# antonilo/unsupervised_detection

Measured on AMD Instinct MI355X. Metric: frame-pairs/sec per adversarial step, DAVIS 480p batch4, 1/2/4/8 GPU, higher is better.
Workload: dtype f32

## Files before the change

include/udet.h:

```cpp
#ifndef UDET_H
#define UDET_H
#include <stddef.h>
#ifdef __cplusplus
extern "C" {
#endif

#define UDET_OK 0
#define UDET_ERR_SHAPE (-1)
#define UDET_ERR_ALIGN (-2)
#define UDET_ERR_HIP (-3)
#define UDET_ERR_UNSUPPORTED (-4)
#define UDET_ERR_ARG (-5)
#define UDET_ERR_OVERFLOW (-6)

#define UDET_ACT_NONE 0
#define UDET_ACT_LEAKY 1
#define UDET_ACT_ELU 2

int udet_version(void);
const char* udet_last_error(void);


int udet_warp(const float* image, const float* flow, float flow_scale, float* out, int n, int h, int w, int c,
              void* stream);
// ... 58 lines not shown
typedef struct {
  int batch;
  int in_h, in_w;
  int img_h, img_w;
  float flow_normalizer;
  float cbn;
  float epsilon;
  float lr, beta1, beta2, adam_eps;
  float clip;
  unsigned long long noise_seed;
  int conv_fp16;
} udet_config;

int udet_plan_create(const udet_config* cfg, udet_plan** out);
void udet_plan_destroy(udet_plan* plan);
size_t udet_workspace_bytes(const udet_plan* plan);
int udet_plan_init(udet_plan* plan, void* workspace, void* stream);

int udet_param_count(int net);
size_t udet_param_total(int net);
int udet_param_info(int net, int index, const char** name, int* rank, int* shape4, size_t* offset_floats);
int udet_buffer_count(const udet_plan* plan);
int udet_buffer_info(const udet_plan* plan, int index, const char** name, size_t* offset_bytes, int* dims_nhw_ld);

int udet_pack_pwc(udet_plan* plan, const float* w_pwc, void* workspace, void* stream);
int udet_pack_trainable(udet_plan* plan, const float* w_gen, const float* w_rec, void* workspace, void* stream);

int udet_pwc_forward(udet_plan* plan, const float* img1, const float* img2, void* workspace, void* stream);
int udet_forward(udet_plan* plan, const float* img1, const float* img2, int ncalls, void* workspace, void* stream);
int udet_prefetch_flow(udet_plan* plan, const float* img1, const float* img2, void* workspace, void* stream);
int udet_forward_prefetched(udet_plan* plan, int ncalls, void* workspace, void* stream);
int udet_prefetch_consume(udet_plan* plan, void* workspace, void* stream);
int udet_forward_from_flow(udet_plan* plan, int ncalls, void* workspace, void* stream);
int udet_generator_forward(udet_plan* plan, void* workspace, void* stream);
int udet_generator_layers(udet_plan* plan, void* workspace, void* stream);
int udet_recover_forward(udet_plan* plan, int n, void* workspace, void* stream);
int udet_backward(udet_plan* plan, int which, const float* w_gen, const float* w_rec, float* g_gen, float* g_rec,
                  void* workspace, void* stream);
int udet_stream_wait_grads(udet_plan* plan, int net, void* stream);
int udet_generator_backward(udet_plan* plan, const float* w_gen, float* g_gen, void* workspace, void* stream);
int udet_recover_backward(udet_plan* plan, const float* w_rec, float* g_rec, void* workspace, void* stream);
int udet_grad_absmean(udet_plan* plan, int net, const float* g, float* out2, void* workspace, void* stream);
int udet_apply(udet_plan* plan, int net, float* w, float* g, float* m, float* v, void* workspace, void* stream);
long udet_fp16_overflow_count(udet_plan* plan);
long udet_get_adam_step(const udet_plan* plan);
void udet_set_adam_step(udet_plan* plan, long t);
int udet_train_step(udet_plan* plan, int which, const float* img1, const float* img2, float* w_gen, float* w_rec,
                    float* g_gen, float* g_rec, float* m_gen, float* v_gen, float* m_rec, float* v_rec, void* workspace,
                    void* stream);

int udet_autotune(udet_plan* plan, const float* w_gen, const float* w_rec, float* g_gen, float* g_rec, void* workspace,
                  void* stream);
int udet_tuned_shapes(void);
int udet_tune_save(const char* path);
int udet_tune_load(const char* path);
int udet_tune_rejected(void);
int udet_profile_begin(udet_plan* plan);
int udet_profile_end(udet_plan* plan, double* out, int ncat, void* stream);

int udet_plan_set_concurrent(udet_plan* plan, int on);

int udet_plan_lane_queues(udet_plan* plan, void* stream, int* queue);
int udet_plan_pin_lanes(udet_plan* plan, void* stream, void* const* side_streams, int n);

#ifdef __cplusplus
}
// ... 3 lines not shown
```

include/udet_debug.h:

```cpp
#ifndef UDET_DEBUG_H
#define UDET_DEBUG_H
#ifdef __cplusplus
extern "C" {
#endif
void udet_debug_force_conv(int bm, int bn, int ks);
void udet_debug_conv_fp16(int on);
void udet_debug_force_wgrad(int nsplit, int dma);
int udet_debug_last_wgrad(void);
void udet_debug_upb_min_pixels(long v);
void udet_debug_set_tuning(int on);
void udet_debug_force_pair(int on);
int udet_debug_last_pair(void);
#include <stddef.h>
int udet_debug_conv2d_pair(const float* xa, const float* xb, const float* wa, const float* wb, const float* ba, const float* bb, float* ya, float* yb,
                           int na, int nb, int h, int w, int cin, int cout, int k, int stride, int dilation, int act, float alpha, void* workspace,
                           size_t workspace_bytes, void* stream);
int udet_debug_last_conv(void);
#ifdef __cplusplus
}
#endif
#endif
```

unsupervised_detection_amd/_devel.py:

```python
from __future__ import annotations

import ctypes
import os

from ._ffi import lib as _lib

_PATH = os.path.join(os.path.dirname(os.path.abspath(__file__)), "libudet_debug.so")
if not os.path.exists(_PATH):
    raise RuntimeError(f"{_PATH} is missing: build it with `make -C unsupervised_detection_amd/csrc`")
dbg = ctypes.CDLL(_PATH, mode=ctypes.RTLD_GLOBAL)
dbg.udet_debug_force_conv.restype = None
dbg.udet_debug_force_conv.argtypes = [ctypes.c_int, ctypes.c_int, ctypes.c_int]
dbg.udet_debug_last_conv.restype = ctypes.c_int
dbg.udet_debug_last_conv.argtypes = []
dbg.udet_debug_conv_fp16.restype = None
dbg.udet_debug_conv_fp16.argtypes = [ctypes.c_int]
dbg.udet_debug_force_wgrad.restype = None
dbg.udet_debug_force_wgrad.argtypes = [ctypes.c_int, ctypes.c_int]
dbg.udet_debug_upb_min_pixels.restype = None
dbg.udet_debug_upb_min_pixels.argtypes = [ctypes.c_long]
dbg.udet_debug_set_tuning.restype = None
dbg.udet_debug_set_tuning.argtypes = [ctypes.c_int]
dbg.udet_debug_last_wgrad.restype = ctypes.c_int
dbg.udet_debug_last_wgrad.argtypes = []
dbg.udet_debug_force_pair.restype = None
dbg.udet_debug_force_pair.argtypes = [ctypes.c_int]
dbg.udet_debug_last_pair.restype = ctypes.c_int
dbg.udet_debug_last_pair.argtypes = []
dbg.udet_debug_conv2d_pair.restype = ctypes.c_int
dbg.udet_debug_conv2d_pair.argtypes = [ctypes.c_void_p] * 8 + [ctypes.c_int] * 10 + [ctypes.c_float, ctypes.c_void_p, ctypes.c_size_t, ctypes.c_void_p]
```

unsupervised_detection_amd/csrc/api_plan.hip:

```cpp
#include <stdlib.h>
#include <string.h>

#include "conv_host.h"
#include "elementwise.h"
#include "plan.h"

using namespace udet;

struct udet_plan {
  Plan* p;
};

extern "C" {

int udet_plan_create(const udet_config* c, udet_plan** out) {
  if (!c || !out) { set_error("plan_create: null argument"); return UDET_ERR_ARG; }
  Config k;
  k.batch = c->batch; k.in_h = c->in_h; k.in_w = c->in_w; k.img_h = c->img_h; k.img_w = c->img_w;
  k.flow_normalizer = c->flow_normalizer; k.cbn = c->cbn; k.epsilon = c->epsilon;
  k.lr = c->lr; k.beta1 = c->beta1; k.beta2 = c->beta2; k.adam_eps = c->adam_eps; k.clip = c->clip;
  k.noise_seed = c->noise_seed;
  k.conv_fp16 = c->conv_fp16 ? 1 : 0;
  Plan* P = plan_build(k);
  if (!P) return UDET_ERR_SHAPE;
// ... 35 lines not shown
  return plan_lane_queues(h->p, (hipStream_t)stream, queue);
}
int udet_plan_pin_lanes(udet_plan* h, void* stream, void* const* side_streams, int n) {
  if (!h || (n > 0 && !side_streams)) { set_error("plan_pin_lanes: null argument"); return UDET_ERR_ARG; }
  return plan_pin_lanes(h->p, (hipStream_t)stream, reinterpret_cast<hipStream_t const*>(side_streams), n);
}
long udet_fp16_overflow_count(udet_plan* h) {
  if (!h) return 0;
  (void)plan_check_overflow(h->p, true);
  return h->p->ovf_skipped;
}
long udet_get_adam_step(const udet_plan* h) {
  plan_settle_adam_step(h->p);
  return h->p->adam_t;
}
void udet_set_adam_step(udet_plan* h, long t) {
  plan_settle_adam_step(h->p);
  h->p->adam_t = t;
}

int udet_pack_pwc(udet_plan* h, const float* w_pwc, void* ws, void* stream) {
  return plan_pack_pwc(h->p, w_pwc, (float*)ws, (hipStream_t)stream);
}
int udet_pack_trainable(udet_plan* h, const float* w_gen, const float* w_rec, void* ws, void* stream) {
  return plan_pack_trainable(h->p, w_gen, w_rec, (float*)ws, (hipStream_t)stream);
}
int udet_pwc_forward(udet_plan* h, const float* img1, const float* img2, void* ws, void* stream) {
  return plan_pwc_forward(h->p, img1, img2, (float*)ws, (hipStream_t)stream);
}
int udet_forward_from_flow(udet_plan* h, int ncalls, void* ws, void* stream) {
  UDET_TRY(plan_check_overflow(h->p, false));
  if (ncalls < 0 || ncalls > 3) { set_error("forward: ncalls must be 0..3"); return UDET_ERR_ARG; }
  return plan_forward(h->p, nullptr, nullptr, ncalls, (float*)ws, (hipStream_t)stream);
}
int udet_generator_forward(udet_plan* h, void* ws, void* stream) {
  UDET_TRY(plan_generator_forward(h->p, (float*)ws, (hipStream_t)stream));
  return plan_recover_forward(h->p, 0, (float*)ws, (hipStream_t)stream);
}
int udet_generator_layers(udet_plan* h, void* ws, void* stream) {
  h->p->ev_next = 0;
  UDET_TRY(plan_generator_layers(h->p, (float*)ws, (hipStream_t)stream));
  return plan_recover_forward(h->p, 0, (float*)ws, (hipStream_t)stream);
}
int udet_recover_forward(udet_plan* h, int n, void* ws, void* stream) {
  if (n < 1 || n > 3) { set_error("recover_forward: n must be 1..3 (multiples of the plan batch)"); return UDET_ERR_ARG; }
  return plan_recover_forward(h->p, n, (float*)ws, (hipStream_t)stream, true);
}
int udet_forward(udet_plan* h, const float* img1, const float* img2, int ncalls, void* ws, void* stream) {
  UDET_TRY(plan_check_overflow(h->p, false));
  if (ncalls < 0 || ncalls > 3) { set_error("forward: ncalls must be 0..3"); return UDET_ERR_ARG; }
  if (!img1 || !img2) { set_error("forward: null image pointer"); return UDET_ERR_ARG; }
  return plan_forward(h->p, img1, img2, ncalls, (float*)ws, (hipStream_t)stream);
}
int udet_prefetch_flow(udet_plan* h, const float* img1, const float* img2, void* ws, void* stream) {
  if (!img1 || !img2) { set_error("prefetch_flow: null image pointer"); return UDET_ERR_ARG; }
  return plan_prefetch(h->p, img1, img2, (float*)ws, (hipStream_t)stream);
}
int udet_prefetch_consume(udet_plan* h, void* ws, void* stream) {
  return plan_prefetch_consume(h->p, (float*)ws, (hipStream_t)stream);
}
int udet_forward_prefetched(udet_plan* h, int ncalls, void* ws, void* stream) {
  UDET_TRY(plan_check_overflow(h->p, false));
  if (ncalls < 0 || ncalls > 3) { set_error("forward: ncalls must be 0..3"); return UDET_ERR_ARG; }
  return plan_forward(h->p, nullptr, nullptr, ncalls, (float*)ws, (hipStream_t)stream, true);
}
int udet_backward(udet_plan* h, int which, const float* w_gen, const float* w_rec, float* g_gen, float* g_rec, void* ws,
// ... 149 lines not shown
```

unsupervised_detection_amd/csrc/common.h:

```cpp
#pragma once
#include <hip/hip_runtime.h>
#include <hip/hip_ext.h>
#include <stdint.h>
#include <stdio.h>
#include <string>

#include "../../include/udet.h"

namespace udet {

void set_error(const char* fmt, ...);
int hip_fail(hipError_t e, const char* what);
#define UDET_HIP(x)                                   \
  do {                                                \
    hipError_t _e = (x);                              \
    if (_e != hipSuccess) return udet::hip_fail(_e, #x); \
  } while (0)
#define UDET_TRY(x)            \
  do {                         \
    int _s = (x);              \
    if (_s != 0) return _s;    \
  } while (0)

struct LaunchSink {
// ... 93 lines not shown
  const float* res;
  int ldres, res_coff;
  float* y2;
  int ldy2, y2_coff;
  int accumulate;
  float* uo;
  int ldu, u_coff;
  const float* ua;
  int ldua, ua_coff, uact;
  float ualpha;
  int u_c0, u_c1;
  int ksplit;
  float* partial;
  size_t partial_cap;
  int ldp;
  int fold;
  int* tickets;
  int tail_full, tail_ks, tail_prow0;
  int f16;
  float f16_xscale;
  const float* wino_u;
  int wino_np;
  int kreal;
};
#define UDET_MAX_TICKETS 4096

int launch_conv(ConvParams& p, hipStream_t stream);
int launch_conv_pair(ConvParams& a, ConvParams& b, hipStream_t stream);
int launch_tap_gather(const ConvParams& g, const float* z, int ldz, hipStream_t stream);

struct PackJob {
  long src_off, dst_off, gamma_off, beta_off;
  long total;
  int T, R, C, Kc, ldw, k_split, k_gap, mode;
};

struct WgradParams {
  const float* x;
  int ldx, x_coff;
  int N, H, W, up_shift;
  int Cin;
  const float* dy;
  const float* ya;
  int ldy, y_coff, Cout;
  int yact;
  float yalpha;
  int OH, OW, isy, isx;
  int ycls, OHf, OWf;
  int ntaps;
  ConvTap taps[UDET_MAX_TAPS];
  float* dw;
  float* db;
  float* partial;
  size_t partial_floats;
  const float* zero16;
  int swapped, oCin, oCout, bias_m;
  int Cin4, Mpad;
  float* pbias;
  FastDiv fd_ohw, fd_ow;
  const float* w;
  const float* b;
  const float* gamma;
  float* dgamma;
  float* dbeta;
  float bn_c;
  int f16;
  float f16_yscale;
};
int launch_wgrad_T(WgradParams& p, int T, hipStream_t stream);
int launch_bn_finalize(float* dw, int T, int Cin, int Cout, const float* w, const float* b, const float* gamma, float bn_c, float* pd,
                       float* db, float* dgamma, float* dbeta, hipStream_t stream);
int launch_wgrad_up_combine(const float* deff, float* dw, int Cin, int Cout, hipStream_t stream);
size_t wgrad_partial_floats_needed(int T, int Cin, int Cout);

}
```

unsupervised_detection_amd/csrc/conv_host.h:

```cpp
#pragma once
#include "common.h"
namespace udet {
void same_pad(int in, int k, int s, int d, int* before, int* out);
void conv_setup_fwd(ConvParams& p, int N, int H, int W, int kh, int kw, int s, int d);
int conv_dgrad_classes(int s, int H, int W);
void conv_force_config(int bm, int bn, int ks);
bool conv_thin_n_ok(const ConvParams& p);
bool conv_thin_k_ok(const ConvParams& p);
int launch_conv_thin_n(const ConvParams& p, hipStream_t stream);
int launch_conv_thin_k(const ConvParams& p, hipStream_t stream);
bool conv_wino_geometry(const ConvParams& p, int* dil, int widx_at[9]);
bool conv_wino_ok(const ConvParams& p);
bool conv_wino_variant_ok(const ConvParams& p, int variant);
int conv_wino_np(int cout);
size_t conv_wino_floats(int Kc, int cout);
long conv_wino_workgroups(const ConvParams& p, int variant);
int conv_wino_max_ksplit(const ConvParams& p, int variant);
int launch_conv_wino(ConvParams& p, int variant, int ks, hipStream_t stream);
int launch_splitk_second_pass(const ConvParams& p, hipStream_t stream);
int launch_wino_pack(const float* src, float* dst, int R, int C, int Kc, int np, int k_split, int k_gap, int transposed, hipStream_t stream);
int launch_wino_from_packed(const ConvParams& p, float* dst, int np, hipStream_t stream);
void conv_debug_f16(int on);
int conv_debug_f16_on();
int conv_last_config();
void conv_set_tuning(int on);
int conv_tuned_shapes();
void conv_clear_tuning();
int conv_tune_rejected();
void conv_tune_note_reject();
float* tune_scratch(size_t floats, int which);
bool tune_compare(const float* a, const float* b, size_t n, hipStream_t stream, float* diff_out, float* scale_out);
void wgrad_set_tuning(int on);
bool wgrad_wino_ok(const WgradParams& p);
int wgrad_wino_slices(const WgradParams& p, int wanted);
int launch_wgrad_wino(const WgradParams& q, int slices, int ldn, hipStream_t stream);
int wgrad_last_config();
void wgrad_force(int nsplit, int dma);
int wgrad_tuned_shapes();
void conv_tune_dump(FILE* f);
void conv_tune_put(unsigned long long key, int bm, int bn, int ks, int ws, int fold, int tail);
void wgrad_tune_dump(FILE* f);
void conv_pair_tune_dump(FILE* f);
void conv_pair_tune_put(unsigned long long key, int bm, int bn, int ks, int ws);
int conv_pair_tuned_shapes();
void conv_pair_clear_tuning();
void conv_force_pair(int on);
int conv_last_pair();
#define UDET_TUNE_ABI 6
void wgrad_tune_put(unsigned long long key, int cfg);
bool conv_setup_dgrad(ConvParams& p, int cls, int N, int H, int W, int kh, int kw, int s, int d);
int launch_pack_weights(const float* src, float* dst, int T, int R, int C, int Kc, int ldw, int k_split, int k_gap,
                        int mode, const float* scale, hipStream_t stream);
int launch_pack_taps_into_n(const float* src, float* dst, int T, int R, int C, int Kc, int ldz, int k_split, int k_gap,
                            int transposed, hipStream_t stream);
int launch_pack_jobs(const PackJob* jobs_dev, int njobs, const float* wsrc, float* ws, float bn_c, hipStream_t stream);
int launch_fold_bn(const float* b, const float* gamma, const float* beta, float c, float* scale, float* bias_f, int n,
                   hipStream_t stream);
int launch_copy_channels(const float* src, int lds, int s_coff, float* dst, int ldd, int d_coff, long P, int C, float mul,
                         float add, hipStream_t stream);
int launch_warp(const float* img, const float* flow, int ldf, int f_coff, float flow_scale, float* out, int N, int H,
                int W, int C, int* dbg_idx, float* dbg_alpha, hipStream_t stream);
int launch_cost_volume(const float* c1, const float* wr, float* out, int ldo, int o_coff, int N, int H, int W, int C,
                       hipStream_t stream);
int launch_warp_cost_volume(const float* c1, const float* c2, const float* flow, int ldf, int f_coff, float flow_scale, float* out,
                            int ldo, int corr_coff, int c1_coff, float* warped_dbg, int N, int H, int W, int C, hipStream_t stream);
inline int round_up(int v, int m) { return (v + m - 1) / m * m; }
}
```

unsupervised_detection_amd/csrc/conv_host.hip:

```cpp
#include <string.h>

#include <stdint.h>

#include "common.h"
#include "conv_host.h"
#include "wino_pack.h"

namespace udet {

void same_pad(int in, int k, int s, int d, int* before, int* out) {
  const int o = (in + s - 1) / s;
  int total = (o - 1) * s + (k - 1) * d + 1 - in;
  if (total < 0) total = 0;
  *before = total / 2;
  *out = o;
}

static inline int floordiv2(int v) { return v >= 0 ? v / 2 : -((-v + 1) / 2); }

static void push_tap(ConvParams& p, int dy, int dx, int widx) {
  const int ymax = (p.OHq - 1) * p.isy + dy, xmax = (p.OWq - 1) * p.isx + dx;
  if (dy >= p.H || ymax < 0 || dx >= p.W || xmax < 0) return;
  p.taps[p.ntaps].dy = dy;
  p.taps[p.ntaps].dx = dx;
// ... 72 lines not shown
    const int k = (int)((e / ldw) % Kc);
    const int t = (int)(e / ((long)ldw * Kc));
    float v = 0.f;
    int ks = k;
    if (k >= k_split) ks = (k < k_split + k_gap) ? -1 : k - k_gap;
    const int r = mode == 0 ? ks : n, c = mode == 0 ? n : ks;
    if (r >= 0 && r < R && c >= 0 && c < C) {
      v = src[((long)t * R + r) * C + c];
      if (scale) v *= scale[c];
    }
    dst[e] = v;
  }
}

int launch_pack_weights(const float* src, float* dst, int T, int R, int C, int Kc, int ldw, int k_split, int k_gap,
                        int mode, const float* scale, hipStream_t stream) {
  const long total = (long)T * Kc * ldw;
  int nb = (int)((total + 255) / 256);
  if (nb > 2048) nb = 2048;
  UDET_LAUNCH(pack_weights_kernel, dim3(nb), dim3(256), 0, stream, src, dst, T, R, C, Kc, ldw, k_split, k_gap,
                     mode, scale);
  UDET_HIP(hipGetLastError());
  return UDET_OK;
}

__constant__ float UPB_MERGE[2][3][3][4] = {
    {{{.5f, 0.f, 0.f, 0.f}, {.5f, 1.f, .5f, 0.f}, {0.f, 0.f, .5f, 1.f}},
     {{.5f, 0.f, 0.f, 0.f}, {.5f, 1.f, 1.f, 0.f}, {0.f, 0.f, 0.f, 0.f}},
     {{0.f, 0.f, 0.f, 0.f}, {0.f, 0.f, .5f, 0.f}, {0.f, 0.f, -.5f, -1.f}}},
    {{{1.f, .5f, 0.f, 0.f}, {0.f, .5f, 1.f, .5f}, {0.f, 0.f, 0.f, .5f}},
     {{1.f, 1.f, 0.f, 0.f}, {0.f, 0.f, 0.f, 0.f}, {0.f, 0.f, 0.f, 0.f}},
     {{0.f, .5f, 0.f, 0.f}, {0.f, -.5f, -1.f, -.5f}, {0.f, 0.f, 0.f, -.5f}}}};

__global__ __launch_bounds__(256) void pack_jobs_kernel(const PackJob* __restrict__ jobs, const float* __restrict__ wsrc,
                                                        float* __restrict__ ws, float bn_c) {
  const PackJob j = jobs[blockIdx.y];
  const float* src = wsrc + j.src_off;
  float* dst = ws + j.dst_off;
  const float* gamma = j.gamma_off >= 0 ? wsrc + j.gamma_off : nullptr;
  if (j.mode == 2) {
    for (long e = (long)blockIdx.x * 256 + threadIdx.x; e < j.total; e += (long)gridDim.x * 256)
      dst[e] = gamma ? src[e] * (gamma[e] * bn_c) + wsrc[j.beta_off + e] : src[e];
    return;
  }
  if (j.mode == 9 || j.mode == 10) {
    const int rv = (int)(j.beta_off / 3), cv = (int)(j.beta_off % 3);
    for (long e = (long)blockIdx.x * 256 + threadIdx.x; e < j.total; e += (long)gridDim.x * 256) {
      const int n = (int)(e % j.ldw), k = (int)(e / j.ldw);
      int ks = k;
      if (k >= j.k_split) ks = (k < j.k_split + j.k_gap) ? -1 : k - j.k_gap;
      const int ci = j.mode == 9 ? ks : n, co = j.mode == 9 ? n : ks;
      const bool real = ci >= 0 && ci < j.R && co >= 0 && co < j.C;
      float w[4][4];
#pragma unroll
      for (int kk = 0; kk < 4; ++kk)
#pragma unroll
        for (int ll = 0; ll < 4; ++ll) w[kk][ll] = real ? src[((long)(kk * 4 + ll) * j.R + ci) * j.C + co] : 0.f;
      const long plane = (long)j.Kc * j.ldw;
#pragma unroll
      for (int py = 0; py < 2; ++py) {
        float t1[3][4];
#pragma unroll
        for (int a = 0; a < 3; ++a)
#pragma unroll
          for (int ll = 0; ll < 4; ++ll) {
            float v = 0.f;
#pragma unroll
            for (int kk = 0; kk < 4; ++kk) v += UPB_MERGE[py][rv][a][kk] * w[kk][ll];
            t1[a][ll] = v;
          }
#pragma unroll
        for (int px = 0; px < 2; ++px)
#pragma unroll
          for (int a = 0; a < 3; ++a)
#pragma unroll
            for (int bb = 0; bb < 3; ++bb) {
              float v = 0.f;
#pragma unroll
              for (int ll = 0; ll < 4; ++ll) v += UPB_MERGE[px][cv][bb][ll] * t1[a][ll];
              dst[(long)((py * 2 + px) * 9 + a * 3 + bb) * plane + e] = v;
            }
      }
    }
    return;
  }
  if (j.mode == 7 || j.mode == 8) {
    for (long e = (long)blockIdx.x * 256 + threadIdx.x; e < j.total; e += (long)gridDim.x * 256) wino_pack_item(j, src, gamma, bn_c, dst, e);
    return;
  }
  for (long e = (long)blockIdx.x * 256 + threadIdx.x; e < j.total; e += (long)gridDim.x * 256) {
    const int n = (int)(e % j.ldw);
    const int k = (int)((e / j.ldw) % j.Kc);
    int t = (int)(e / ((long)j.ldw * j.Kc));
    float v = 0.f;
    int ks = k;
    if (k >= j.k_split) ks = (k < j.k_split + j.k_gap) ? -1 : k - j.k_gap;
    int r = j.mode == 0 ? ks : n, c = j.mode == 0 ? n : ks;
    if (j.mode == 3 || j.mode == 4) {
      t = n / j.C;
      c = n - t * j.C;
      r = ks;
      if (t >= j.T) r = -1;
    }
    if (j.mode >= 5) {
      const int cls = t >> 2, ty = (t >> 1) & 1, tx = t & 1, py = cls >> 1, px = cls & 1;
      const int y0 = py == 0 ? (ty == 0 ? 0 : 1) : (ty == 0 ? 0 : 2), y1 = py == 0 ? (ty == 0 ? 0 : 2) : (ty == 0 ? 1 : 2);
      const int x0 = px == 0 ? (tx == 0 ? 0 : 1) : (tx == 0 ? 0 : 2), x1 = px == 0 ? (tx == 0 ? 0 : 2) : (tx == 0 ? 1 : 2);
      const int ci = j.mode == 5 ? ks : n, co = j.mode == 5 ? n : ks;
      if (ci >= 0 && ci < j.R && co >= 0 && co < j.C) {
        for (int ky = y0; ky <= y1; ++ky)
          for (int kx = x0; kx <= x1; ++kx) v += src[((long)(ky * 3 + kx) * j.R + ci) * j.C + co];
        if (gamma) v *= gamma[co] * bn_c;
      }
      dst[e] = v;
      continue;
    }
    if (r >= 0 && r < j.R && c >= 0 && c < j.C) {
      v = j.mode == 4 ? src[((long)t * j.C + c) * j.R + r] : src[((long)t * j.R + r) * j.C + c];
      if (gamma) v *= gamma[c] * bn_c;
    }
    dst[e] = v;
  }
}
int launch_pack_jobs(const PackJob* jobs_dev, int njobs, const float* wsrc, float* ws, float bn_c, hipStream_t stream) {
  if (njobs < 1) return UDET_OK;
  UDET_LAUNCH(pack_jobs_kernel, dim3(48, njobs), dim3(256), 0, stream, jobs_dev, wsrc, ws, bn_c);
  UDET_HIP(hipGetLastError());
  return UDET_OK;
}

__global__ __launch_bounds__(256) void pack_job_kernel(const PackJob j, const float* __restrict__ wsrc, float* __restrict__ ws) {
  const float* src = wsrc + j.src_off;
  float* dst = ws + j.dst_off;
  for (long e = (long)blockIdx.x * 256 + threadIdx.x; e < j.total; e += (long)gridDim.x * 256) {
    const int n = (int)(e % j.ldw);
    const int k = (int)((e / j.ldw) % j.Kc);
    int ks = k;
    if (k >= j.k_split) ks = (k < j.k_split + j.k_gap) ? -1 : k - j.k_gap;
    const int t = n / j.C, c = n - t * j.C;
    float v = 0.f;
    if (ks >= 0 && ks < j.R && t < j.T) v = j.mode == 4 ? src[((long)t * j.C + c) * j.R + ks] : src[((long)t * j.R + ks) * j.C + c];
    dst[e] = v;
  }
}
int launch_pack_taps_into_n(const float* src, float* dst, int T, int R, int C, int Kc, int ldz, int k_split, int k_gap,
                            int transposed, hipStream_t stream) {
  PackJob j;
  memset(&j, 0, sizeof(j));
  j.T = T; j.R = R; j.C = C; j.Kc = Kc; j.ldw = ldz; j.k_split = k_split; j.k_gap = k_gap;
  j.mode = transposed ? 4 : 3; j.total = (long)Kc * ldz; j.gamma_off = -1;
  int nb = (int)((j.total + 255) / 256);
  if (nb > 1024) nb = 1024;
  UDET_LAUNCH(pack_job_kernel, dim3(nb), dim3(256), 0, stream, j, src, dst);
  UDET_HIP(hipGetLastError());
  return UDET_OK;
}

__global__ __launch_bounds__(256) void tap_gather_kernel(const ConvParams g, const float* __restrict__ z, int ldz) {
  const long total = (long)g.N * g.OH * g.OW * g.Cout;
// ... 117 lines not shown
```

unsupervised_detection_amd/csrc/conv_wgrad.hip:

```cpp
#include <stdlib.h>

#include <mutex>
#include <unordered_map>

#include "common.h"
#include <algorithm>
#include <vector>
#include "conv_host.h"
#include "plan.h"

namespace udet {

typedef float floatx16 __attribute__((ext_vector_type(16)));
typedef _Float16 halfx4 __attribute__((ext_vector_type(4)));

template <int BM, int BN, int WAVES_M, int WAVES_N>
__global__ __launch_bounds__(256) void conv_wgrad_kernel(const WgradParams p, int co_tiles, int nsplit) {
  constexpr int BKP = 32;
  constexpr int WTM = BM / WAVES_M, WTN = BN / WAVES_N;
  constexpr int TM = WTM / 32, TN = WTN / 32;
  static_assert(WAVES_M * WAVES_N == 4 && TM * 32 == WTM && TN * 32 == WTN, "tile");
  constexpr int A_F4_ROW = BM / 4, B_F4_ROW = BN / 4;
  constexpr int A_PIX = 256 / A_F4_ROW, B_PIX = 256 / B_F4_ROW;
  constexpr int A_LD = BKP / A_PIX, B_LD = BKP / B_PIX;
// ... 439 lines not shown
      for (; k + 7 * SL < nsplit; k += 8 * SL) {
        float a[8];
#pragma unroll
        for (int u = 0; u < 8; ++u) a[u] = src[(size_t)(k + u * SL) * slab];
#pragma unroll
        for (int u = 0; u < 8; ++u) s += a[u];
      }
      for (; k < nsplit; k += SL) s += src[(size_t)k * slab];
    }
    if (SL > 1) {
      part[t] = s;
      __syncthreads();
      if (sl == 0) {
#pragma unroll
        for (int u = 1; u < SL; ++u) s += part[t + u * CW];
      }
      __syncthreads();
    }
    if (on && sl == 0) {
      const size_t e = ((size_t)p.taps[tap].widx * p.Cin + ci) * p.Cout + co;
      dot = fmaf(p.w[e], s, dot);
      p.dw[e] = s * gs;
    }
  }
  red[t] = dot;
  __syncthreads();
  if (rg == 0 && co < p.Cout) {
    float d = red[co];
#pragma unroll
    for (int g = 1; g < RG; ++g) d += red[g * CW + co];
    pd[(size_t)blockIdx.x * p.Cout + co] = d;
  }
}
__global__ __launch_bounds__(256) void wgrad_bn_finish2_kernel(const WgradParams p, int ldn, int nsplit, int nb, const float* __restrict__ pd) {
  __shared__ float red[256];
  __shared__ float redS[256];
  const int t = threadIdx.x, cl = t & 31, rg = t >> 5, co = blockIdx.x * 32 + cl;
  const int per = (nb + 7) / 8, b0 = rg * per, b1 = b0 + per < nb ? b0 + per : nb;
  const int pers = (nsplit + 7) / 8, k0 = rg * pers, k1 = k0 + pers < nsplit ? k0 + pers : nsplit;
  float d = 0.f, S = 0.f;
  if (co < p.Cout) {
    int b = b0;
    for (; b + 11 < b1; b += 12) {
      float a[12];
#pragma unroll
      for (int u = 0; u < 12; ++u) a[u] = pd[(size_t)(b + u) * p.Cout + co];
#pragma unroll
      for (int u = 0; u < 12; ++u) d += a[u];
    }
    for (; b < b1; ++b) d += pd[(size_t)b * p.Cout + co];
    int k = k0;
    for (; k + 7 < k1; k += 8) {
      float a[8];
#pragma unroll
      for (int u = 0; u < 8; ++u) a[u] = p.pbias[(size_t)(k + u) * ldn + co];
#pragma unroll
      for (int u = 0; u < 8; ++u) S += a[u];
    }
    for (; k < k1; ++k) S += p.pbias[(size_t)k * ldn + co];
  }
  red[t] = d;
  redS[t] = S;
  __syncthreads();
  if (rg == 0 && co < p.Cout) {
    float dsum = red[cl], Ssum = redS[cl];
#pragma unroll
    for (int g = 1; g < 8; ++g) { dsum += red[g * 32 + cl]; Ssum += redS[g * 32 + cl]; }
    p.dgamma[co] = p.bn_c * (dsum + p.b[co] * Ssum);
    p.dbeta[co] = Ssum;
    p.db[co] = p.gamma[co] * p.bn_c * Ssum;
  }
}
__global__ __launch_bounds__(256) void bn_dot_kernel(const float* __restrict__ w, const float* __restrict__ g, int R, int C,
                                                     float* __restrict__ pd) {
  __shared__ float red[256];
  const int t = threadIdx.x, cx = t & 63, ry = t >> 6;
  const int c = blockIdx.x * 64 + cx;
  const int r_begin = (int)((long)R * blockIdx.y / BND_SPLIT), r_end = (int)((long)R * (blockIdx.y + 1) / BND_SPLIT);
  float s = 0.f;
  if (c < C)
    for (int r = r_begin + ry; r < r_end; r += 4) s = fmaf(w[(size_t)r * C + c], g[(size_t)r * C + c], s);
  red[t] = s;
  __syncthreads();
  if (ry == 0 && c < C) pd[(size_t)blockIdx.y * C + c] = red[cx] + red[64 + cx] + red[128 + cx] + red[192 + cx];
}
__global__ __launch_bounds__(256) void bn_finish_kernel(float* __restrict__ dw, long n, int C, const float* __restrict__ gamma,
                                                        const float* __restrict__ b, float bn_c, const float* __restrict__ pd,
                                                        float* __restrict__ db, float* __restrict__ dgamma,
                                                        float* __restrict__ dbeta) {
  for (long e = (long)blockIdx.x * 256 + threadIdx.x; e < n; e += (long)gridDim.x * 256) {
    const int c = (int)(e % C);
    dw[e] *= gamma[c] * bn_c;
  }
  if (blockIdx.x == 0) {
    for (int c = threadIdx.x; c < C; c += 256) {
      float dot = 0.f;
      for (int j = 0; j < BND_SPLIT; ++j) dot += pd[(size_t)j * C + c];
      const float S = db[c];
      dgamma[c] = bn_c * (dot + b[c] * S);
      dbeta[c] = S;
      db[c] = gamma[c] * bn_c * S;
    }
  }
}
// ... 29 lines not shown
}
size_t wgrad_partial_floats_needed(int T, int Cin, int Cout) {
  const size_t cin4 = (size_t)((Cin + 3) & ~3), mpad = (T * cin4 + 127) / 128 * 128, ldn = (size_t)(Cout + 127) / 128 * 128;
  return (size_t)BNR_MAXBLK * Cout + ldn + mpad * ldn + 64;
}

static int g_force_wsplit = 0, g_force_wdma = -1;
static int g_wlast = 0;
int wgrad_last_config() { return g_wlast; }
void wgrad_force(int nsplit, int dma) { g_force_wsplit = nsplit > 0 ? nsplit : 0; g_force_wdma = dma; }
static std::unordered_map<uint64_t, int> g_wcache;
static std::mutex g_wcache_mu;
static int g_wtuning = 0;
void wgrad_set_tuning(int on) { g_wtuning = on; }
int wgrad_tuned_shapes() { std::lock_guard<std::mutex> l(g_wcache_mu); return (int)g_wcache.size(); }
void wgrad_tune_dump(FILE* f) {
  std::lock_guard<std::mutex> l(g_wcache_mu);
  for (auto& kv : g_wcache) fprintf(f, "w %llu %d\n", (unsigned long long)kv.first, kv.second);
}
void wgrad_tune_put(unsigned long long key, int cfg) {
  std::lock_guard<std::mutex> l(g_wcache_mu);
  g_wcache[(uint64_t)key] = cfg;
}

template <int BM, int BN, int WM_, int WN_>
static void wgrad_launch(const WgradParams& p, int m_tiles, int co_tiles, int nsplit, int dma, hipStream_t stream) {
  dim3 grid(m_tiles * co_tiles, nsplit);
  if (dma && p.f16) UDET_LAUNCH((conv_wgrad_dma_kernel<BM, BN, WM_, WN_, 2, true>), grid, dim3(512), 0, stream, p, co_tiles, nsplit);
  else if (dma == 2) UDET_LAUNCH((conv_wgrad_dma_kernel<BM, BN, WM_, WN_, 3>), grid, dim3(512), 0, stream, p, co_tiles, nsplit);
  else if (dma) UDET_LAUNCH((conv_wgrad_dma_kernel<BM, BN, WM_, WN_, 2>), grid, dim3(512), 0, stream, p, co_tiles, nsplit);
  else UDET_LAUNCH((conv_wgrad_kernel<BM, BN, WM_, WN_>), grid, dim3(256), 0, stream, p, co_tiles, nsplit);
}

int launch_wgrad_T(WgradParams& p, int T, hipStream_t stream) {
  if (conv_debug_f16_on()) p.f16 = 1;
  if (p.f16 && !(p.f16_yscale > 0.f)) p.f16_yscale = 1.f;
  if (p.f16 && g_wtuning) p.f16_yscale = 1.f;
  if (p.ldx % 4 || p.x_coff % 4 || p.ldy % 4 || p.y_coff % 4) {
    set_error("wgrad: ldx=%d x_coff=%d ldy=%d y_coff=%d must be multiples of 4", p.ldx, p.x_coff, p.ldy, p.y_coff);
    return UDET_ERR_ALIGN;
  }
  WgradParams g = p;
  g.swapped = 0; g.bias_m = -1; g.oCin = p.Cin; g.oCout = p.Cout;
  {
    int centre = -1;
    for (int t = 0; t < p.ntaps; ++t)
      if (p.taps[t].dy == 0 && p.taps[t].dx == 0) centre = t;
    auto tile_cost = [](long rows, int cols) {
      const int bn_ = cols > 64 ? 128 : (cols > 32 ? 64 : 32);
      return ((rows + 127) / 128 * 128) * (long)((cols + bn_ - 1) / bn_ * bn_);
    };
    const int co4 = (p.Cout + 3) & ~3, ci4 = (p.Cin + 3) & ~3;
    const bool cheaper = tile_cost((long)p.ntaps * co4, p.Cin) < tile_cost((long)p.ntaps * ci4, p.Cout);
    const bool narrow = p.Cout <= 4 ? p.Cin >= 16 : (p.Cout <= 16 && 128 % co4 == 0 && cheaper);
    const bool swap = narrow && p.isy == 1 && p.isx == 1 && p.up_shift == 0 && p.H == p.OH && p.W == p.OW &&
                      p.ya == nullptr && centre >= 0;
    if (swap) {
      g.x = p.dy; g.ldx = p.ldy; g.x_coff = p.y_coff; g.Cin = p.Cout;
      g.dy = p.x; g.ldy = p.ldx; g.y_coff = p.x_coff; g.Cout = p.Cin;
      for (int t = 0; t < p.ntaps; ++t) { g.taps[t].dy = -p.taps[t].dy; g.taps[t].dx = -p.taps[t].dx; }
      g.swapped = 1;
      g.bias_m = centre * co4;
    }
  }
  const int BM = 128;
  const int bn = g.Cout > 64 ? 128 : (g.Cout > 32 ? 64 : 32);
  g.Cin4 = (g.Cin + 3) & ~3;
// ... 10 lines not shown
  g.fd_ohw = make_fastdiv((unsigned)(g.OH * g.OW));
  g.fd_ow = make_fastdiv((unsigned)g.OW);
  float* pd = p.partial;
  float* base = pd + (size_t)BNR_MAXBLK * p.Cout;
  base += (16 - ((uintptr_t)base / sizeof(float)) % 16) % 16;
  const size_t fixed = (size_t)(base - p.partial);
  const size_t bgroups = p.ycls ? 4 : 1;
  const size_t per_split = bgroups * (size_t)ldn + (size_t)g.Mpad * ldn;
  if (p.partial_floats < fixed + per_split) {
    set_error("wgrad: workspace too small (%zu < %zu floats)", p.partial_floats, fixed + per_split);
    return UDET_ERR_ARG;
  }
  const long tiles = (long)m_tiles * co_tiles;
  const size_t maxs = (p.partial_floats - fixed) / per_split;
  int cap = nchunks / 2 > 0 ? nchunks / 2 : 1;
  if ((size_t)cap > maxs) cap = (int)maxs;
  int nsplit = (int)((768 + tiles - 1) / tiles);
  if (nsplit > cap) nsplit = cap;
  if (nsplit < 1) nsplit = 1;
  if (p.f16 && p.ya == nullptr && p.zero16 != nullptr && !(reinterpret_cast<uintptr_t>(p.zero16) & 15)) nsplit |= 1 << 20;
  const size_t wsz = (size_t)T * p.Cin * p.Cout;
  if (p.ntaps < T) UDET_HIP(hipMemsetAsync(p.dw, 0, wsz * sizeof(float), stream));
  const long total = (long)(Mreal + 1) * g.Cout;
  const bool dma_ok = p.ya == nullptr && p.zero16 != nullptr && !(reinterpret_cast<uintptr_t>(p.zero16) & 15);
  const bool fused_bn = p.gamma && !g.swapped && !p.ycls && p.ntaps == T && p.Cout <= 128 && p.db && p.dgamma && p.dbeta && p.w && p.b;
  const bool wino_ok = !g.swapped && !p.ycls && !plan_knob(UDET_KNOB_NO_WGRAD_WINO) && wgrad_wino_ok(g);
  auto run = [&](int cfg) -> int {
    int ns = cfg & 0xfffff;
    int dma = cfg >> 20;
    if (dma == 3 && !wino_ok) dma = 1;
    if (dma != 3 && !dma_ok) dma = 0;
    if (dma == 3) ns = wgrad_wino_slices(g, ns > (int)maxs ? (int)maxs : ns);
    WgradParams q = g;
    q.pbias = base;
    q.partial = base + (size_t)ns * bgroups * ldn;
    if (dma == 3 && launch_wgrad_wino(q, ns, ldn, stream) != UDET_OK) {
      dma = dma_ok ? 1 : 0;
      ns = nsplit & 0xfffff;
      if (ns > cap) ns = cap;
      if (ns < 1) ns = 1;
      q.partial = base + (size_t)ns * bgroups * ldn;
    }
    if (dma == 3) {}
    else if (bn == 128) wgrad_launch<128, 128, 2, 2>(q, m_tiles, co_tiles, ns, dma, stream);
    else if (bn == 64) wgrad_launch<128, 64, 2, 2>(q, m_tiles, co_tiles, ns, dma, stream);
    else wgrad_launch<128, 32, 4, 1>(q, m_tiles, co_tiles, ns, dma, stream);
    if (fused_bn) {
      const int cw = g.Cout > 64 ? 128 : (g.Cout > 32 ? 64 : (g.Cout > 16 ? 32 : 16));
      const int rg = 256 / cw;
      int sl = ns >= 64 ? 8 : (ns >= 32 ? 4 : (ns >= 12 ? 2 : 1));
      if (sl > rg) sl = rg;
      while (sl > 1 && (long)((Mreal + rg - 1) / rg) * sl > 512) sl >>= 1;
      int rb = rg / sl;
      while ((Mreal + rb - 1) / rb > BNR_MAXBLK) rb *= 2;
      const int nb = (Mreal + rb - 1) / rb;
#define UDET_RBN(CW_, SL_) UDET_LAUNCH((wgrad_reduce_bn_kernel<CW_, SL_>), dim3(nb), dim3(256), 0, stream, q, ldn, ns, rb, pd)
      if (cw == 128) { if (sl == 2) UDET_RBN(128, 2); else UDET_RBN(128, 1); }
      else if (cw == 64) { if (sl == 4) UDET_RBN(64, 4); else if (sl == 2) UDET_RBN(64, 2); else UDET_RBN(64, 1); }
      else if (cw == 32) { if (sl == 8) UDET_RBN(32, 8); else if (sl == 4) UDET_RBN(32, 4); else if (sl == 2) UDET_RBN(32, 2); else UDET_RBN(32, 1); }
      else { if (sl == 8) UDET_RBN(16, 8); else if (sl == 4) UDET_RBN(16, 4); else if (sl == 2) UDET_RBN(16, 2); else UDET_RBN(16, 1); }
#undef UDET_RBN
      UDET_LAUNCH(wgrad_bn_finish2_kernel, dim3((g.Cout + 31) / 32), dim3(256), 0, stream, q, ldn, ns, nb, pd);
      return UDET_OK;
    }
    const int sl = (ns >= 64 && total * 64 <= 262144) ? 64 : ((ns >= 8 && total * 8 <= 262144) ? 8 : 1);
    const long nbl = (total * sl + 255) / 256;
    const int nb = (int)(nbl > 4096 ? 4096 : nbl);
    if (sl == 64) UDET_LAUNCH(wgrad_reduce_kernel<64>, dim3(nb), dim3(256), 0, stream, q, ldn, ns);
    else if (sl == 8) UDET_LAUNCH(wgrad_reduce_kernel<8>, dim3(nb), dim3(256), 0, stream, q, ldn, ns);
    else UDET_LAUNCH(wgrad_reduce_kernel<1>, dim3(nb), dim3(256), 0, stream, q, ldn, ns);
    return UDET_OK;
  };
  {
    const int f[] = {p.N, p.H, p.W, p.up_shift, p.Cin, p.Cout, p.ntaps, p.OH, p.OW, p.isy, p.ya ? 1 : 0, p.ldx, p.ldy, cap, dma_ok ? 1 : 0, g.swapped, p.ycls, p.f16 ? 1 : 0,
                     p.ntaps > 0 ? p.taps[0].dy : 0, p.ntaps > 0 ? p.taps[0].dx : 0};
    uint64_t key = 1469598103934665603ull;
    for (int v : f) { key ^= (uint64_t)(uint32_t)v; key *= 1099511628211ull; }
    bool have = false;
    {
      std::lock_guard<std::mutex> l(g_wcache_mu);
      auto it = g_wcache.find(key);
      if (it != g_wcache.end()) {
        const int hv = nsplit, v = it->second >> 20, ns = it->second & 0xfffff;
        if (v < 0 || v > 3 || ns < 1) nsplit = hv;
        else nsplit = (v != 3 && ns > cap ? cap : ns) | (v << 20);
        have = true;
      }
    }
    if (!have && g_wtuning) {
      static hipEvent_t e0 = nullptr, e1 = nullptr;
      if (!e0) { (void)hipEventCreate(&e0); (void)hipEventCreate(&e1); }
      const int h = nsplit;
      float best_ms = 1e30f;
      int best = h;
      const int hc = h & 0xfffff;
// ... 41 lines not shown
        float diff = 0.f, scale = 0.f;
        if (r0) {
          run(h);
          (void)hipMemcpyAsync(r0, p.dw, wsz * sizeof(float), hipMemcpyDeviceToDevice, stream);
          if (p.db) (void)hipMemcpyAsync(r0 + wsz, p.db, (size_t)p.Cout * sizeof(float), hipMemcpyDeviceToDevice, stream);
          run(best);
          ok = tune_compare(r0, p.dw, wsz, stream, &diff, &scale);
          if (ok && p.db) ok = tune_compare(r0 + wsz, p.db, (size_t)p.Cout, stream, &diff, &scale);
        }
        if (!ok) {
          fprintf(stderr, "[udet tune] REJECTED wgrad N=%d %dx%d Cin=%d Cout=%d taps=%d: nsplit=%d dma=%d differs from the heuristic "
                  "configuration (max|diff| %.3e, scale %.3e)\n", p.N, p.OH, p.OW, p.Cin, p.Cout, p.ntaps, best & 0xfffff, best >> 20, diff, scale);
          conv_tune_note_reject();
          nsplit = h;
        }
      }
      if (getenv("UDET_TUNE_LOG"))
        fprintf(stderr, "[udet tune] wgrad N=%d %dx%d Cin=%d Cout=%d taps=%d -> nsplit=%d dma=%d (heuristic %d) %.1f us\n", p.N, p.OH,
                p.OW, p.Cin, p.Cout, p.ntaps, nsplit & 0xfffff, nsplit >> 20, h & 0xfffff, best_ms / 3 * 1e3f);
      std::lock_guard<std::mutex> l(g_wcache_mu);
      g_wcache[key] = nsplit;
    }
  }
  if (g_force_wsplit > 0) {
    const int ns = g_force_wsplit > cap ? cap : g_force_wsplit;
    int v = g_force_wdma >= 0 ? g_force_wdma : (nsplit >> 20);
    if (v == 3 && !wino_ok) v = dma_ok ? 1 : 0;
    if (v != 3 && !dma_ok) v = 0;
    nsplit = ns | (v << 20);
  }
  if ((nsplit >> 20) == 3 && !wino_ok) nsplit = (nsplit & 0xfffff) | ((dma_ok ? 1 : 0) << 20);
  if ((nsplit >> 20) == 3) nsplit = wgrad_wino_slices(g, (nsplit & 0xfffff) > (int)maxs ? (int)maxs : (nsplit & 0xfffff)) | (3 << 20);
  g_wlast = nsplit;
  UDET_TRY(run(nsplit));
  UDET_HIP(hipGetLastError());
  int nbw = (int)((wsz + 255) / 256);
  if (nbw > 2048) nbw = 2048;
  if (p.gamma && !fused_bn) {
    if (!p.db || !p.dgamma || !p.dbeta || !p.w || !p.b) {
      set_error("wgrad: BN finalisation needs db, dgamma, dbeta, w and b");
      return UDET_ERR_ARG;
    }
    UDET_LAUNCH(bn_dot_kernel, dim3((p.Cout + 63) / 64, BND_SPLIT), dim3(256), 0, stream, p.w, p.dw, T * p.Cin,
                       p.Cout, pd);
    UDET_LAUNCH(bn_finish_kernel, dim3(nbw), dim3(256), 0, stream, p.dw, (long)wsz, p.Cout, p.gamma, p.b, p.bn_c, pd,
                       p.db, p.dgamma, p.dbeta);
    UDET_HIP(hipGetLastError());
  }
  return UDET_OK;
}

}
```

unsupervised_detection_amd/csrc/devel/api_debug.hip:

```cpp
#include <string.h>

#include "../../../include/udet_debug.h"
#include "../conv_host.h"
#include "../plan.h"

using namespace udet;

extern "C" {
int udet_debug_last_conv(void) { return conv_last_config(); }
void udet_debug_force_conv(int bm, int bn, int ks) { conv_force_config(bm, bn, ks); }
void udet_debug_conv_fp16(int on) { conv_debug_f16(on); }
void udet_debug_force_wgrad(int nsplit, int dma) { wgrad_force(nsplit, dma); }
int udet_debug_last_wgrad(void) { return wgrad_last_config(); }
void udet_debug_upb_min_pixels(long v) { plan_debug_upb_min_pixels(v); }
void udet_debug_force_pair(int on) { conv_force_pair(on); }
int udet_debug_last_pair(void) { return conv_last_pair(); }
int udet_debug_conv2d_pair(const float* xa, const float* xb, const float* wa, const float* wb, const float* ba, const float* bb, float* ya, float* yb,
                           int na, int nb, int h, int w, int cin, int cout, int k, int stride, int dilation, int act, float alpha, void* workspace,
                           size_t workspace_bytes, void* stream_) {
  hipStream_t stream = (hipStream_t)stream_;
  if (cin % 8 != 0 || k * k > UDET_MAX_TAPS) { set_error("debug_conv2d_pair: cin must be a multiple of 8"); return UDET_ERR_SHAPE; }
  const int kc = cin, ldw = round_up(cout, 4);
  const size_t wfl = ((size_t)k * k * kc * ldw + 63) & ~(size_t)63, part_fl = (size_t)4 << 20, zero_fl = 64 + UDET_MAX_TICKETS;
  if (workspace_bytes < (2 * wfl + part_fl + zero_fl) * sizeof(float)) { set_error("debug_conv2d_pair: workspace too small"); return UDET_ERR_ARG; }
  float* wpa = reinterpret_cast<float*>(workspace);
  float* wpb = wpa + wfl;
  float* part = wpb + wfl;
  float* zero = part + part_fl;
  UDET_HIP(hipMemsetAsync(zero, 0, zero_fl * sizeof(float), stream));
  UDET_TRY(launch_pack_weights(wa, wpa, k * k, cin, cout, kc, ldw, kc, 0, 0, nullptr, stream));
  UDET_TRY(launch_pack_weights(wb, wpb, k * k, cin, cout, kc, ldw, kc, 0, 0, nullptr, stream));
  ConvParams p[2];
  for (int i = 0; i < 2; ++i) {
    memset(&p[i], 0, sizeof(ConvParams));
    conv_setup_fwd(p[i], i ? nb : na, h, w, k, k, stride, dilation);
    p[i].x = i ? xb : xa; p[i].ldx = cin; p[i].wp = i ? wpb : wpa; p[i].Kc = kc; p[i].ldw = ldw; p[i].bias = i ? bb : ba;
    p[i].y = i ? yb : ya; p[i].ldy = cout; p[i].Cout = cout; p[i].act = act; p[i].alpha = alpha;
    p[i].partial = part; p[i].partial_cap = part_fl; p[i].zero16 = zero; p[i].tickets = reinterpret_cast<int*>(zero + 64);
  }
  return launch_conv_pair(p[0], p[1], stream);
}
void udet_debug_set_tuning(int on) {
  conv_set_tuning(on);
  wgrad_set_tuning(on);
}
}
```

unsupervised_detection_amd/csrc/elementwise.h:

```cpp
#pragma once
#include "common.h"
namespace udet {
int launch_resize_bilinear_fwd(const float* x, int ldx, int x_coff, int N, int H, int W, float* y, int ldy, int y_coff,
                               int OH, int OW, int C, float mul, float div, hipStream_t s);
int launch_resize_bilinear_bwd(const float* dy, int ldy, int y_coff, int N, int OH, int OW, float* dx, int ldx, int x_coff,
                               int H, int W, int C, int accumulate, hipStream_t s);
int launch_upb_ring(const float* x, int ld, int N, int H, int W, float* xh, hipStream_t s);
int launch_upb_ring_fold(const float* dxh, int ld, int N, int H, int W, float* dx, hipStream_t s);
int launch_share_samples(float* buf, long P, int ld, int coff, int C, int copies, hipStream_t s);
int launch_fold_samples(float* buf, long P, int ld, int coff, int C, int copies, hipStream_t s);
int launch_emit_du(const float* d, const float* a, float* u, long P, int ld, int coff, int C, int act, float alpha, hipStream_t s);
int launch_pool2x2_sum(const float* du, float* dx, int N, int H, int W, int C, hipStream_t s);
int launch_pack_pwc_input(const float* i1, const float* i2, float* x8, long P, hipStream_t s);
int launch_gen_input(const float* img, const float* f, double* part, float* gin, int B, long HW, hipStream_t s);
size_t flow_stats_doubles(int B);
int launch_mask_rec_inputs(const float* logits, const float* f, float* mask, float* fin, long P, int ncalls, hipStream_t s);
int launch_pack_imgin(const float* img, float* imgin, long P, int ncalls, hipStream_t s);
int launch_losses(const float* f, const float* mask, const float* pred, long HW, int B, float cbn, float eps,
                  float num_pixels, float* part, float* losses, float* coef, float* sums, hipStream_t s);
size_t loss_part_floats(int B);
int launch_rec_loss_bwd(const float* f, const float* mask, const float* pred, float* dpred, long BHW, float cbn,
                        float inv_np, hipStream_t s);
int launch_gen_loss_bwd(const float* f, const float* mask, const float* pred, const float* coef, float* dpred,
                        float* dmask, long HW, int B, float cbn, hipStream_t s);
int launch_mask_bwd(const float* dmask, const float* dfin, const float* f, const float* mask, float* dlogits, long P,
                    hipStream_t s);
int launch_grad_absmean(const float* g, const long* seg_off, const long* seg_len, int nvars, float* vmean, float thresh,
                        float* out, hipStream_t s);
int launch_adam(float* w, float* g, float* m, float* v, long n, float lr_t, float b1, float b2, float eps, float clip,
                const float* flag, uint64_t seed, uint64_t step, hipStream_t s, int mode = 0, const int* skip = nullptr);
int launch_nonfinite_count(const float* g, long n, int* out, hipStream_t s);
int launch_flow_normalize(const float* f, double* part, float* out, int B, long HW, hipStream_t s);
int launch_charbonnier(const float* gt, const float* pred, const float* mask, int mc, int B, long HW, float cbn, float* part,
                       float* out, hipStream_t s);
int launch_crop_flip_resize(const void* src, int src_u8, int nearest, int N, int H, int W, int C, const int* prm, float* dst, int OH,
                            int OW, float div, float add, hipStream_t s);
int launch_crop_flip_resize_ragged(const void* src, int src_u8, int nearest, int N, int C, const long long* offsets, const int* hw,
                                   const int* prm, float* dst, int OH, int OW, float div, float add, hipStream_t s);
int launch_mask_stats(const float* pred, const float* gt, int N, int H, int W, float threshold, float gt_threshold, double* out,
                      hipStream_t s);
int launch_fill_uniform(float* x, long n, uint64_t seed, float lo, float hi, hipStream_t s);
int launch_axpy(const float* x, float* y, long n, float a, int accumulate, hipStream_t s);
}
```

unsupervised_detection_amd/csrc/elementwise.hip:

```cpp
#include "common.h"
#include "elementwise.h"

namespace udet {

static inline int grid_for(long total, int cap = 4096) {
  long nb = (total + 255) / 256;
  if (nb > cap) nb = cap;
  if (nb < 1) nb = 1;
  return (int)nb;
}

template <typename T>
__device__ __forceinline__ T wave_sum(T v) {
#pragma unroll
  for (int o = 32; o > 0; o >>= 1) v += __shfl_down(v, o, 64);
  return v;
}
template <typename T>
__device__ __forceinline__ T block_sum(T v, T* sm ) {
  v = wave_sum(v);
  __syncthreads();
  if ((threadIdx.x & 63) == 0) sm[threadIdx.x >> 6] = v;
  __syncthreads();
  return sm[0] + sm[1] + sm[2] + sm[3];
// ... 314 lines not shown
        float4* q = reinterpret_cast<float4*>(buf + o + (long)k * P * ld);
        if (FOLD) {
          const float4 w = *q;
          v.x += w.x; v.y += w.y; v.z += w.z; v.w += w.w;
        } else {
          *q = v;
        }
      }
      if (FOLD) *reinterpret_cast<float4*>(buf + o) = v;
    } else {
      float v = buf[o];
      for (int k = 1; k < copies; ++k) {
        if (FOLD) v += buf[o + (long)k * P * ld];
        else buf[o + (long)k * P * ld] = v;
      }
      if (FOLD) buf[o] = v;
    }
  }
}
static int launch_share_fold(float* buf, long P, int ld, int coff, int C, int copies, bool fold, hipStream_t s) {
  if (copies < 2 || C < 1) return UDET_OK;
  const bool v4 = (ld % 4 == 0) && (coff % 4 == 0) && (C % 4 == 0);
  const long n = P * (v4 ? C / 4 : C);
  if (v4) {
    if (fold) hipLaunchKernelGGL((share_fold_kernel<4, true>), dim3(grid_for(n)), dim3(256), 0, s, buf, P, ld, coff, C, copies);
    else hipLaunchKernelGGL((share_fold_kernel<4, false>), dim3(grid_for(n)), dim3(256), 0, s, buf, P, ld, coff, C, copies);
  } else {
    if (fold) hipLaunchKernelGGL((share_fold_kernel<1, true>), dim3(grid_for(n)), dim3(256), 0, s, buf, P, ld, coff, C, copies);
    else hipLaunchKernelGGL((share_fold_kernel<1, false>), dim3(grid_for(n)), dim3(256), 0, s, buf, P, ld, coff, C, copies);
  }
  UDET_HIP(hipGetLastError());
  return UDET_OK;
}
int launch_share_samples(float* buf, long P, int ld, int coff, int C, int copies, hipStream_t s) {
  return launch_share_fold(buf, P, ld, coff, C, copies, false, s);
}
int launch_fold_samples(float* buf, long P, int ld, int coff, int C, int copies, hipStream_t s) {
  return launch_share_fold(buf, P, ld, coff, C, copies, true, s);
}

__global__ __launch_bounds__(256) void pack_pwc_input_kernel(const float* __restrict__ i1, const float* __restrict__ i2,
                                                             float* __restrict__ x8, long P) {
  for (long e = (long)blockIdx.x * 256 + threadIdx.x; e < 2 * P; e += (long)gridDim.x * 256) {
    const float* s = e < P ? i1 + e * 3 : i2 + (e - P) * 3;
    float4 a = make_float4(s[0] + 0.5f, s[1] + 0.5f, s[2] + 0.5f, 0.f);
    *reinterpret_cast<float4*>(x8 + e * 4) = a;
  }
}
int launch_pack_pwc_input(const float* i1, const float* i2, float* x8, long P, hipStream_t s) {
  hipLaunchKernelGGL(pack_pwc_input_kernel, dim3(grid_for(2 * P)), dim3(256), 0, s, i1, i2, x8, P);
  UDET_HIP(hipGetLastError());
  return UDET_OK;
}

#define FS_BLOCKS 32
__global__ __launch_bounds__(256) void flow_stats_kernel(const float* __restrict__ f, long HW, double* __restrict__ part) {
  __shared__ double sm[4];
  const int n = blockIdx.y;
  double s0 = 0, s1 = 0, q0 = 0, q1 = 0;
  for (long p = (long)blockIdx.x * 256 + threadIdx.x; p < HW; p += (long)gridDim.x * 256) {
    const float2 v = *reinterpret_cast<const float2*>(f + ((long)n * HW + p) * 2);
    s0 += v.x; s1 += v.y;
    q0 += (double)v.x * v.x; q1 += (double)v.y * v.y;
  }
  s0 = block_sum(s0, sm); s1 = block_sum(s1, sm); q0 = block_sum(q0, sm); q1 = block_sum(q1, sm);
  if (threadIdx.x == 0) {
// ... 2 lines not shown
  }
}
__global__ __launch_bounds__(256) void pack_gen_input_kernel(const float* __restrict__ img, const float* __restrict__ f,
                                                             const double* __restrict__ part, float* __restrict__ gin,
                                                             long HW) {
  __shared__ float st[4];
  const int n = blockIdx.y;
  if (threadIdx.x < 2) {
    double s = 0, q = 0;
    for (int b = 0; b < FS_BLOCKS; ++b) {
      s += part[((long)n * FS_BLOCKS + b) * 4 + threadIdx.x];
      q += part[((long)n * FS_BLOCKS + b) * 4 + 2 + threadIdx.x];
    }
    const double mean = s / (double)HW, var = q / (double)HW - mean * mean;
    st[threadIdx.x] = (float)mean;
    st[2 + threadIdx.x] = sqrtf((float)var);
  }
  __syncthreads();
  const float m0 = st[0], m1 = st[1], d0 = st[2], d1 = st[3];
  for (long p = (long)blockIdx.x * 256 + threadIdx.x; p < HW; p += (long)gridDim.x * 256) {
    const long q = (long)n * HW + p;
    const float2 v = *reinterpret_cast<const float2*>(f + q * 2);
    *reinterpret_cast<float4*>(gin + q * 8) = make_float4(img[q * 3], img[q * 3 + 1], img[q * 3 + 2], (v.x - m0) / d0);
    *reinterpret_cast<float4*>(gin + q * 8 + 4) = make_float4((v.y - m1) / d1, 0.f, 0.f, 0.f);
  }
}
int launch_gen_input(const float* img, const float* f, double* part, float* gin, int B, long HW, hipStream_t s) {
  hipLaunchKernelGGL(flow_stats_kernel, dim3(FS_BLOCKS, B), dim3(256), 0, s, f, HW, part);
  hipLaunchKernelGGL(pack_gen_input_kernel, dim3(grid_for(HW, 256), B), dim3(256), 0, s, img, f, part, gin, HW);
  UDET_HIP(hipGetLastError());
  return UDET_OK;
}
size_t flow_stats_doubles(int B) { return (size_t)B * FS_BLOCKS * 4; }
__global__ __launch_bounds__(256) void flow_normalize_kernel(const float* __restrict__ f, const double* __restrict__ part,
                                                             float* __restrict__ out, long HW) {
  __shared__ float st[4];
  const int n = blockIdx.y;
  if (threadIdx.x < 2) {
    double s = 0, q = 0;
    for (int b = 0; b < FS_BLOCKS; ++b) {
      s += part[((long)n * FS_BLOCKS + b) * 4 + threadIdx.x];
      q += part[((long)n * FS_BLOCKS + b) * 4 + 2 + threadIdx.x];
    }
    const double mean = s / (double)HW, var = q / (double)HW - mean * mean;
    st[threadIdx.x] = (float)mean;
    st[2 + threadIdx.x] = sqrtf((float)var);
  }
  __syncthreads();
  const float m0 = st[0], m1 = st[1], d0 = st[2], d1 = st[3];
  for (long p = (long)blockIdx.x * 256 + threadIdx.x; p < HW; p += (long)gridDim.x * 256) {
    const long q = (long)n * HW + p;
    const float2 v = *reinterpret_cast<const float2*>(f + q * 2);
    *reinterpret_cast<float2*>(out + q * 2) = make_float2((v.x - m0) / d0, (v.y - m1) / d1);
  }
}
int launch_flow_normalize(const float* f, double* part, float* out, int B, long HW, hipStream_t s) {
  hipLaunchKernelGGL(flow_stats_kernel, dim3(FS_BLOCKS, B), dim3(256), 0, s, f, HW, part);
  hipLaunchKernelGGL(flow_normalize_kernel, dim3(grid_for(HW, 256), B), dim3(256), 0, s, f, part, out, HW);
  UDET_HIP(hipGetLastError());
  return UDET_OK;
}

__global__ __launch_bounds__(256) void mask_rec_inputs_kernel(const float* __restrict__ logits ,
                                                              const float* __restrict__ f, float* __restrict__ mask,
                                                              float* __restrict__ fin, long P, int ncalls) {
  for (long q = (long)blockIdx.x * 256 + threadIdx.x; q < P; q += (long)gridDim.x * 256) {
// ... 37 lines not shown
__device__ __forceinline__ float charb(float e, float cbn) {
  const float s = e * e + 0.001f * 0.001f;
  return cbn == 0.5f ? sqrtf(s) : powf(s, cbn);
}
__device__ __forceinline__ float charb_d(float e, float cbn) {
  const float s = e * e + 0.001f * 0.001f;
  return cbn == 0.5f ? e / sqrtf(s) : cbn * powf(s, cbn - 1.f) * 2.f * e;
}
#define LS_BLOCKS 64
__global__ __launch_bounds__(256) void loss_sums_kernel(const float* __restrict__ f, const float* __restrict__ mask,
                                                        const float* __restrict__ pred , long HW, int B,
                                                        float cbn, float* __restrict__ part ) {
  __shared__ float sm[4];
  const int n = blockIdx.y;
  float R = 0, Rc = 0, Pp = 0, Dr = 0, Dc = 0;
  for (long p = (long)blockIdx.x * 256 + threadIdx.x; p < HW; p += (long)gridDim.x * 256) {
    const long q = (long)n * HW + p;
    const float2 fl = *reinterpret_cast<const float2*>(f + q * 2);
    const float2 a = *reinterpret_cast<const float2*>(pred + q * 2);
    const float2 b = *reinterpret_cast<const float2*>(pred + ((long)B * HW + q) * 2);
    const float2 c = *reinterpret_cast<const float2*>(pred + ((long)2 * B * HW + q) * 2);
    const float m = mask[q], cm = 1.f - m;
    const float pa = charb(fl.x - a.x, cbn) + charb(fl.y - a.y, cbn);
    const float pb = charb(fl.x - b.x, cbn) + charb(fl.y - b.y, cbn);
    const float pc = charb(fl.x - c.x, cbn) + charb(fl.y - c.y, cbn);
    R += pa * m; Rc += pb * cm; Pp += pc; Dr += pc * m; Dc += pc * cm;
  }
  R = block_sum(R, sm); Rc = block_sum(Rc, sm); Pp = block_sum(Pp, sm); Dr = block_sum(Dr, sm); Dc = block_sum(Dc, sm);
  if (threadIdx.x == 0) {
    float* o = part + ((long)n * LS_BLOCKS + blockIdx.x) * 5;
    o[0] = R; o[1] = Rc; o[2] = Pp; o[3] = Dr; o[4] = Dc;
  }
}
__global__ void loss_finish_kernel(const float* __restrict__ part, int B, float eps, float num_pixels,
                                   float* __restrict__ losses, float* __restrict__ coef, float* __restrict__ sums) {
  if (threadIdx.x != 0 || blockIdx.x != 0) return;
  float red = 0.f, redc = 0.f, rs = 0.f;
  for (int b = 0; b < B; ++b) {
    float v[5] = {0, 0, 0, 0, 0};
    for (int k = 0; k < LS_BLOCKS; ++k)
      for (int j = 0; j < 5; ++j) v[j] += part[((long)b * LS_BLOCKS + k) * 5 + j];
    const float D = v[3] + eps, Dc = v[4] + eps;
    red += 1.f - v[0] / D;
    redc += 1.f - v[1] / Dc;
    rs += v[0] + v[1] + v[2];
    coef[b * 4 + 0] = -1.f / (B * D);
    coef[b * 4 + 1] = v[0] / (B * D * D);
    coef[b * 4 + 2] = -1.f / (B * Dc);
    coef[b * 4 + 3] = v[1] / (B * Dc * Dc);
    for (int j = 0; j < 5; ++j) sums[b * 5 + j] = v[j];
    if (b == 0) { losses[4] = v[0]; losses[5] = v[1]; losses[6] = D; losses[7] = Dc; }
  }
  red /= B; redc /= B;
  losses[0] = red + redc;
  losses[1] = rs / num_pixels;
  losses[2] = red;
  losses[3] = redc;
}
int launch_losses(const float* f, const float* mask, const float* pred, long HW, int B, float cbn, float eps,
                  float num_pixels, float* part, float* losses, float* coef, float* sums, hipStream_t s) {
  hipLaunchKernelGGL(loss_sums_kernel, dim3(LS_BLOCKS, B), dim3(256), 0, s, f, mask, pred, HW, B, cbn, part);
  hipLaunchKernelGGL(loss_finish_kernel, dim3(1), dim3(64), 0, s, part, B, eps, num_pixels, losses, coef, sums);
  UDET_HIP(hipGetLastError());
  return UDET_OK;
}
size_t loss_part_floats(int B) { return (size_t)B * LS_BLOCKS * 5; }

__global__ __launch_bounds__(256) void charbonnier_sum_kernel(const float* __restrict__ gt, const float* __restrict__ pred,
                                                              const float* __restrict__ mask, int mc, long HW, float cbn,
                                                              float* __restrict__ part ) {
  __shared__ float sm[4];
  const int n = blockIdx.y;
  float acc = 0.f;
  for (long p = (long)blockIdx.x * 256 + threadIdx.x; p < HW; p += (long)gridDim.x * 256) {
    const long q = (long)n * HW + p;
    const float2 a = *reinterpret_cast<const float2*>(gt + q * 2);
    const float2 b = *reinterpret_cast<const float2*>(pred + q * 2);
    const float m0 = mask ? mask[q * mc] : 1.f, m1 = mask ? mask[q * mc + (mc - 1)] : 1.f;
    acc += charb(a.x - b.x, cbn) * m0 + charb(a.y - b.y, cbn) * m1;
  }
  acc = block_sum(acc, sm);
  if (threadIdx.x == 0) part[(long)n * LS_BLOCKS + blockIdx.x] = acc;
}
__global__ void charbonnier_finish_kernel(const float* __restrict__ part, int B, float* __restrict__ out) {
  const int b = blockIdx.x * blockDim.x + threadIdx.x;
  if (b >= B) return;
  float v = 0.f;
  for (int k = 0; k < LS_BLOCKS; ++k) v += part[(long)b * LS_BLOCKS + k];
  out[b] = v;
}
int launch_charbonnier(const float* gt, const float* pred, const float* mask, int mc, int B, long HW, float cbn, float* part,
                       float* out, hipStream_t s) {
  hipLaunchKernelGGL(charbonnier_sum_kernel, dim3(LS_BLOCKS, B), dim3(256), 0, s, gt, pred, mask, mc, HW, cbn, part);
  hipLaunchKernelGGL(charbonnier_finish_kernel, dim3((B + 63) / 64), dim3(64), 0, s, part, B, out);
  UDET_HIP(hipGetLastError());
// ... 61 lines not shown
    dm -= g0.x * fl.x + g0.y * fl.y + g0.w;
    dm += g1.x * fl.x + g1.y * fl.y + g1.w;
    const float m = mask[q];
    const float d0 = dm * m * (1.f - m) / 10.f;
    dlogits[q * 8] = d0;
    dlogits[q * 8 + 1] = -d0;
  }
}
int launch_mask_bwd(const float* dmask, const float* dfin, const float* f, const float* mask, float* dlogits, long P,
                    hipStream_t s) {
  hipLaunchKernelGGL(mask_bwd_kernel, dim3(grid_for(P)), dim3(256), 0, s, dmask, dfin, f, mask, dlogits, P);
  UDET_HIP(hipGetLastError());
  return UDET_OK;
}

#define GA_SPLIT 8
__global__ __launch_bounds__(256) void grad_absmean_kernel(const float* __restrict__ g, const long* __restrict__ seg_off,
                                                           const long* __restrict__ seg_len, float* __restrict__ vpart) {
  __shared__ float sm[4];
  const long off = seg_off[blockIdx.x], len = seg_len[blockIdx.x];
  const long b = len * blockIdx.y / GA_SPLIT, e = len * (blockIdx.y + 1) / GA_SPLIT;
  float s0 = 0.f, s1 = 0.f, s2 = 0.f, s3 = 0.f;
  long i = b + threadIdx.x;
  for (; i + 768 < e; i += 1024) {
    s0 += fabsf(g[off + i]);
    s1 += fabsf(g[off + i + 256]);
    s2 += fabsf(g[off + i + 512]);
    s3 += fabsf(g[off + i + 768]);
  }
  for (; i < e; i += 256) s0 += fabsf(g[off + i]);
  const float s = block_sum((s0 + s1) + (s2 + s3), sm);
  if (threadIdx.x == 0) vpart[blockIdx.x * GA_SPLIT + blockIdx.y] = s;
}
__global__ void grad_flag_kernel(const float* __restrict__ vpart, const long* __restrict__ seg_len, int nvars, float thresh,
                                 float* __restrict__ out ) {
  if (threadIdx.x == 0 && blockIdx.x == 0) {
    float s = 0.f;
    for (int i = 0; i < nvars; ++i) {
      float v = 0.f;
      for (int j = 0; j < GA_SPLIT; ++j) v += vpart[i * GA_SPLIT + j];
      s += v / (float)seg_len[i];
    }
    s /= (float)nvars;
    out[0] = s;
    out[1] = s < thresh ? 1.f : 0.f;
  }
}
int launch_grad_absmean(const float* g, const long* seg_off, const long* seg_len, int nvars, float* vmean, float thresh,
                        float* out, hipStream_t s) {
  hipLaunchKernelGGL(grad_absmean_kernel, dim3(nvars, GA_SPLIT), dim3(256), 0, s, g, seg_off, seg_len, vmean);
  hipLaunchKernelGGL(grad_flag_kernel, dim3(1), dim3(64), 0, s, vmean, seg_len, nvars, thresh, out);
  UDET_HIP(hipGetLastError());
  return UDET_OK;
}

__device__ __host__ __forceinline__ float udet_uniform01(uint64_t seed, uint64_t step, uint64_t idx) {
  uint64_t z = seed * 0x9E3779B97F4A7C15ull + step * 0xBF58476D1CE4E5B9ull + idx + 0x94D049BB133111EBull;
  z = (z ^ (z >> 30)) * 0xBF58476D1CE4E5B9ull;
  z = (z ^ (z >> 27)) * 0x94D049BB133111EBull;
  z = z ^ (z >> 31);
  return (float)(z >> 40) * (1.0f / 16777216.0f);
}

__global__ __launch_bounds__(256) void adam_kernel(float* __restrict__ w, float* __restrict__ g, float* __restrict__ m,
                                                   float* __restrict__ v, long n, float lr_t, float b1, float b2, float eps,
                                                   float clip, const float* __restrict__ flag, uint64_t seed,
                                                   uint64_t step, int mode, const int* __restrict__ skip) {
  if (skip && *skip != 0) return;
  const bool noise = flag && flag[1] != 0.f;
  for (long i = (long)blockIdx.x * 256 + threadIdx.x; i < n; i += (long)gridDim.x * 256) {
    float gi = g[i];
    if (mode != 2) {
      if (noise) gi = fabsf((udet_uniform01(seed, step, (uint64_t)i) * 2.f - 1.f) * clip);
      else gi = fminf(fmaxf(gi, -clip), clip);
      g[i] = gi;
      if (mode == 1) continue;
    }
    const float mi = m[i] + (gi - m[i]) * (1.f - b1);
    const float vi = v[i] + (gi * gi - v[i]) * (1.f - b2);
    m[i] = mi;
    v[i] = vi;
    w[i] = w[i] - lr_t * mi / (sqrtf(vi) + eps);
  }
}
// ... 136 lines not shown
```

unsupervised_detection_amd/csrc/plan.h:

```cpp
#pragma once
#include <map>
#include <string>
#include <vector>

#include "common.h"

namespace udet {

struct ParamDesc {
  std::string name;
  int rank;
  int shape[4];
  size_t offset, count;
};
struct NetParams {
  std::vector<ParamDesc> p;
  size_t total = 0;
  int add(const std::string& name, int a, int b = 0, int c = 0, int d = 0);
  int find(const std::string& name) const;
};
enum { NET_PWC = 0, NET_GEN = 1, NET_REC = 2 };
const NetParams& net_params(int net);

struct Buf {
  std::string name;
  size_t off;
  int n, h, w, ld;
  size_t floats() const { return (size_t)n * h * w * ld; }
};

struct Layer {
  std::string name;
  int net;
  int kh, kw, cin, cout, stride, dil;
  bool transposed = false;
  bool up = false;
  int act = ACT_NONE;
  float alpha = 0.f;
  int w_idx = -1, b_idx = -1, g_idx = -1, be_idx = -1;
  int Kc = 0, ldw = 0, k_split = 0, k_gap = 0;
  size_t wp_off = 0;
  int KcT = 0, ldwT = 0;
  size_t wpT_off = 0;
  size_t bias_f_off = 0, scale_off = 0;
  size_t wu_off = 0, wuT_off = 0;
  size_t wino_off = 0, winoT_off = 0;
  int wino_np = 0, winoT_np = 0;
  bool upb = false;
  bool upb_bwd = false;
  bool upb_split = false;
  int xhat = -1, src = -1;
  size_t wupb_off = 0, wupbT_off = 0;
  struct SegLaunch {
    int nseg = 0;
    ConvSeg seg[UDET_MAX_SEGS];
    int seg_tap[UDET_MAX_SEGS + 1];
    std::vector<ConvTap> taps;
    size_t tab_off = 0;
  } upb_f, upb_b;
  int x = -1, x_coff = 0, y = -1, y_coff = 0;
  int res = -1, res_coff = 0, y2 = -1;
  int H = 0, W = 0;
  bool col2im = false;
  int ldz = 0, zbuf = -1;
  size_t wz_off = 0;
};

struct Config {
  int batch, in_h, in_w, img_h, img_w;
  float flow_normalizer, cbn, epsilon;
  float lr, beta1, beta2, adam_eps, clip;
  unsigned long long noise_seed;
  int conv_fp16 = 0;
};

struct Plan {
  Config cfg;
  std::vector<Buf> bufs;
  std::map<std::string, int> buf_by_name;
  std::vector<Layer> pwc, gen, rec;
  size_t packed_floats = 0;
  size_t arena_floats = 0;
  enum { NLANE = 6, NCAND = 8, MAXCAND = 32 };
  std::vector<hipStream_t> cand;
  struct Placement {
    hipStream_t main = nullptr;
    hipStream_t lane[NLANE] = {};
    int queue[NLANE] = {};
    int nqueues = 1;
  };
  std::vector<Placement> placements;
  int placed = -1;
  hipEvent_t prefetch_ev = nullptr;
  hipEvent_t grad_ev[3] = {nullptr, nullptr, nullptr};
  bool prefetch_pending = false;
  std::vector<hipEvent_t> ev_pool, ev_pool_prefetch;
  size_t ev_next = 0, ev_next_prefetch = 0;
  bool in_prefetch = false;
  bool concurrent = true;
  bool enc_a_shared = false;
  size_t scratch_off[NLANE] = {}, scratch_floats = 0;
  size_t wgrad_off[NLANE] = {}, wgrad_floats = 0;
  ~Plan();
  size_t small_off = 0;
  size_t ticket_off = 0;
  size_t seg_off[3] = {0, 0, 0};
  size_t jobs_off[3] = {0, 0, 0};
  int njobs[3] = {0, 0, 0};
  struct ProfRec {
    int cat; double flops, bytes; hipEvent_t a, b; std::string name;
    double mfma_scale = 1.0;
    enum { MAXK = 16 };
    hipEvent_t kev[2 * MAXK];
    LaunchSink sink;
  };
  bool profiling = false;
  std::vector<ProfRec*> prof;
  long adam_t = 0;
  int* ovf_host = nullptr;
  hipEvent_t ovf_ev[3] = {nullptr, nullptr, nullptr};
  bool ovf_pending[3] = {false, false, false};
  long ovf_skipped = 0;
  int ovf_report_values = 0, ovf_report_nets = 0;
  bool pwc_packed = false;
  int add_buf(const std::string& name, int n, int h, int w, int ld);
  const Buf& buf(int id) const { return bufs[id]; }
  int bid(const std::string& name) const;
};

#define UDET_PACKJOB_CAP(layers) (8 * (layers) + 32)
#define UDET_SMALL_NOISE 256
#define UDET_SMALL_OVF 300
#define UDET_SMALL_SUMS 1024
Plan* plan_build(const Config& cfg);
void plan_debug_upb_min_pixels(long v);
enum { UDET_KNOB_ENC_A_LANE = 0, UDET_KNOB_REC_DEC_WGRAD_LANE = 1, UDET_KNOB_REC_ENC_WGRAD_LANE = 2, UDET_KNOB_GEN_WGRAD_LATE = 3, UDET_KNOB_NO_WGRAD_WINO = 6, UDET_KNOB_SKIP = 7, UDET_KNOB_NO_PAIRS = 8, UDET_KNOB_COUNT = 12 };
#ifdef UDET_EXPERIMENT
void plan_debug_knob(int id, long v);
long plan_knob(int id);
#else
constexpr long plan_knob(int) { return 0; }
#endif

int plan_init_workspace(Plan* P, float* ws, hipStream_t s);
int plan_pack_pwc(Plan* P, const float* w_pwc, float* ws, hipStream_t s);
int plan_pack_trainable(Plan* P, const float* w_gen, const float* w_rec, float* ws, hipStream_t s);
int plan_pwc_forward(Plan* P, const float* img1, const float* img2, float* ws, hipStream_t s);
int plan_forward(Plan* P, const float* img1, const float* img2, int ncalls, float* ws, hipStream_t s, bool prefetched = false);
int plan_prefetch(Plan* P, const float* img1, const float* img2, float* ws, hipStream_t s);
int plan_prefetch_consume(Plan* P, float* ws, hipStream_t s);
int plan_generator_forward(Plan* P, float* ws, hipStream_t s);
int plan_generator_layers(Plan* P, float* ws, hipStream_t s);
int plan_recover_forward(Plan* P, int ncalls, float* ws, hipStream_t s, bool inputs_prepacked = false, bool skip_enc_a = false, bool enc_a_input_packed = false);
int plan_losses(Plan* P, float* ws, hipStream_t s);
int plan_backward(Plan* P, int which, const float* w_gen, const float* w_rec, float* g_gen, float* g_rec, float* ws, hipStream_t s);
int plan_apply(Plan* P, int net, float* w, float* g, float* m, float* v, float* ws, hipStream_t s);
int plan_check_overflow(Plan* P, bool wait);
void plan_settle_adam_step(Plan* P);
int plan_lane_queues(Plan* P, hipStream_t s, int* queue);
int plan_pin_lanes(Plan* P, hipStream_t main, hipStream_t const* streams, int n);
enum { PROF_CONV_FWD = 0, PROF_CONV_DGRAD = 1, PROF_CONV_WGRAD = 2, PROF_WARP = 3, PROF_CORR = 4, PROF_NCAT = 5 };
void prof_begin(Plan* P, int cat, double flops, double bytes, hipStream_t s, const char* name = "");
void prof_end(Plan* P, hipStream_t s);

}
```

unsupervised_detection_amd/csrc/plan_build.hip:

```cpp
#include <stdarg.h>
#include <stdlib.h>
#include <string.h>

#include "conv_host.h"
#include "elementwise.h"
#include "plan.h"

namespace udet {

int NetParams::add(const std::string& name, int a, int b, int c, int d) {
  ParamDesc q;
  q.name = name;
  q.shape[0] = a; q.shape[1] = b; q.shape[2] = c; q.shape[3] = d;
  q.rank = d ? 4 : (c ? 3 : (b ? 2 : 1));
  q.count = (size_t)a * (b ? b : 1) * (c ? c : 1) * (d ? d : 1);
  q.offset = total;
  total += q.count;
  p.push_back(q);
  return (int)p.size() - 1;
}
int NetParams::find(const std::string& name) const {
  for (size_t i = 0; i < p.size(); ++i)
    if (p[i].name == name) return (int)i;
  return -1;
// ... 121 lines not shown
                      int cout, int stride, int dil, int act, float alpha) {
  Layer L;
  L.name = name; L.net = net;
  L.kh = L.kw = k; L.cin = cin; L.cout = cout; L.stride = stride; L.dil = dil;
  L.act = act; L.alpha = alpha;
  const NetParams& np = net_params(net);
  L.w_idx = np.find(wname);
  L.b_idx = np.find(bname);
  L.Kc = round_up(cin, cin <= 4 ? 4 : 8);
  L.ldw = round_up(cout, 4);
  L.k_split = L.Kc;
  L.k_gap = 0;
  return L;
}

static size_t align64(size_t v) { return (v + 63) & ~(size_t)63; }

Plan::~Plan() {
  for (auto& st : cand)
    if (st) (void)hipStreamDestroy(st);
  for (auto& e : ev_pool) (void)hipEventDestroy(e);
  for (auto& e : ev_pool_prefetch) (void)hipEventDestroy(e);
  if (prefetch_ev) (void)hipEventDestroy(prefetch_ev);
  for (auto* r : prof) delete r;
  for (auto& ev : grad_ev)
    if (ev) (void)hipEventDestroy(ev);
  for (auto& ev : ovf_ev)
    if (ev) (void)hipEventDestroy(ev);
  if (ovf_host) (void)hipHostFree(ovf_host);
}

static long g_upb_bwd_min = 8192;
void plan_debug_upb_min_pixels(long v) { g_upb_bwd_min = v < 0 ? 8192 : v; }
#ifdef UDET_EXPERIMENT
static long g_knob[UDET_KNOB_COUNT] = {};
void plan_debug_knob(int id, long v) { if (id >= 0 && id < UDET_KNOB_COUNT) g_knob[id] = v; }
long plan_knob(int id) { return id >= 0 && id < UDET_KNOB_COUNT ? g_knob[id] : 0; }
extern "C" void udet_exp_knob(int id, long v) { plan_debug_knob(id, v); }
#endif

static inline bool upb_used(int parity, int last, int a) { return !last || (parity == 0 ? a < 2 : a < 1); }
static void build_upb_launches(Layer& L, int h, int w) {
  Layer::SegLaunch& F = L.upb_f;
  F.nseg = 0; F.taps.clear();
  for (int r = 0; r < 4; ++r) {
    const int rv = r & 1, cv = r >> 1;
    const int r0 = rv ? h - 1 : 0, c0 = cv ? w - 1 : 0, nr = rv ? 1 : h - 1, nc = cv ? 1 : w - 1;
    for (int c = 0; c < 4; ++c) {
      const int py = c >> 1, px = c & 1;
      ConvSeg& g = F.seg[F.nseg];
      memset(&g, 0, sizeof(g));
      g.oy = 2 * r0 + py; g.ox = 2 * c0 + px; g.h = nr; g.w = nc;
      F.seg_tap[F.nseg++] = (int)F.taps.size();
      for (int a = 0; a < 3; ++a)
        for (int b = 0; b < 3; ++b) {
          if (!upb_used(py, rv, a) || !upb_used(px, cv, b)) continue;
          F.taps.push_back(ConvTap{r0 + a + py, c0 + b + px, r * 36 + 9 * c + 3 * a + b});
        }
    }
  }
  F.seg_tap[F.nseg] = (int)F.taps.size();
  Layer::SegLaunch& B = L.upb_b;
  B.nseg = 0; B.taps.clear();
  struct Combo { int p, a, last; };
  auto combos = [](int grp, std::vector<Combo>& out) {
    out.clear();
// ... 312 lines not shown
    if (L.upb) {
      L.wupb_off = off; off = align64(off + (size_t)4 * 36 * L.Kc * L.ldw);
      L.upb_f.tab_off = off; off = align64(off + L.upb_f.taps.size() * (sizeof(ConvTap) / sizeof(float)));
      if (L.upb_bwd) {
        L.wupbT_off = off; off = align64(off + (size_t)4 * 36 * L.KcT * L.ldwT);
        L.upb_b.tab_off = off; off = align64(off + L.upb_b.taps.size() * (sizeof(ConvTap) / sizeof(float)));
      }
    }
    if (!cfg.conv_fp16 && L.kh == 3 && L.kw == 3 && L.stride == 1 && !L.up && !L.transposed && !L.col2im && L.cout >= 16 && L.H * L.W >= 512) {
      if (L.Kc % 8 == 0) {
        L.wino_np = conv_wino_np(L.cout);
        L.wino_off = off; off = align64(off + conv_wino_floats(L.Kc, L.cout));
      }
      if (trainable && L.KcT % 8 == 0 && L.cin >= 16) {
        L.winoT_np = conv_wino_np(L.cin);
        L.winoT_off = off; off = align64(off + conv_wino_floats(L.KcT, L.cin));
      }
    }
  };
  for (auto& L : P->pwc) place(L, false);
  for (auto& L : P->gen) place(L, true);
  for (auto& L : P->rec) place(L, true);
  P->packed_floats = off;

  for (auto& b : P->bufs) { b.off = off; off = align64(off + b.floats()); }
  P->scratch_floats = (size_t)24 << 20;
  P->wgrad_floats = (size_t)48 << 20;
  for (int l = 0; l < Plan::NLANE; ++l) {
    P->scratch_off[l] = off;
    off = align64(off + P->scratch_floats);
    P->wgrad_off[l] = off;
    if (l < 4) off = align64(off + P->wgrad_floats);
  }
  P->small_off = off;
  off = align64(off + 65536);
  P->ticket_off = off;
  off = align64(off + (size_t)Plan::NLANE * UDET_MAX_TICKETS);
  for (int net = 1; net <= 2; ++net) {
    P->seg_off[net] = off;
    off = align64(off + 4 * net_params(net).p.size() + 64);
  }
  for (int net = 1; net <= 2; ++net) {
    const size_t nl = net == NET_GEN ? P->gen.size() : P->rec.size();
    P->jobs_off[net] = off;
    off = align64(off + UDET_PACKJOB_CAP(nl) * (sizeof(PackJob) / sizeof(float)) + 64);
  }
  P->arena_floats = off;
  if (const char* e = getenv("UDET_SERIAL")) P->concurrent = atoi(e) == 0;
  for (int i = 0; i < Plan::NCAND; ++i) {
    hipStream_t c = nullptr;
    if (hipStreamCreateWithFlags(&c, hipStreamNonBlocking) == hipSuccess) P->cand.push_back(c);
  }
  if (P->cand.empty()) P->concurrent = false;
  struct { const char* n; int a, d; size_t o; } views[5] = {{"losses", 1, 8, 0}, {"loss_coef", B, 4, 16}, {"noise_flag", 1, 2, UDET_SMALL_NOISE},
                                                            {"fp16_overflow", 2, 2, UDET_SMALL_OVF}, {"loss_sums", B, 5, UDET_SMALL_SUMS}};
  for (auto& v : views) {
    const int id = P->add_buf(v.n, v.a, 1, 1, v.d);
    P->bufs[id].off = P->small_off + v.o;
  }
  return P;
}

}
```

unsupervised_detection_amd/csrc/plan_exec.hip:

```cpp
#include <math.h>
#include <stdlib.h>
#include <string.h>

#include "conv_host.h"
#include "elementwise.h"
#include "lanes.h"
#include "plan.h"

namespace udet {

static const float BN_C = 0.99950037468777316f;

static const Layer* find_layer(const std::vector<Layer>& v, const std::string& name) {
  for (const auto& L : v)
    if (L.name == name) return &L;
  return nullptr;
}
static std::string S(const char* fmt, int a, int b = 0) {
  char buf[128];
  snprintf(buf, sizeof(buf), fmt, a, b);
  return buf;
}

void prof_begin(Plan* P, int cat, double flops, double bytes, hipStream_t s, const char* name) {
// ... 314 lines not shown
    set_error("dgrad(%s): gradient/activation layout mismatch (%d vs %d)", L.name.c_str(), bdy.ld, ba.ld);
    return UDET_ERR_SHAPE;
  }
  const int up = L.up ? 1 : 0;
  prof_begin(P, PROF_CONV_DGRAD, layer_flops(L, N) * ((L.up && L.wuT_off) ? 4.0 / 9.0 : 1.0), layer_bytes(L, N), s, L.name.c_str());
  const bool upeff = L.up && L.wuT_off;
  for (int cls = 0; cls < (upeff ? 1 : conv_dgrad_classes(L.stride, L.H << up, L.W << up)); ++cls) {
    ConvParams p;
    memset(&p, 0, sizeof(p));
    if (upeff) setup_up_dgrad(p, N, L.H, L.W);
    else if (!conv_setup_dgrad(p, cls, N, L.H << up, L.W << up, L.kh, L.kw, L.stride, L.dil)) continue;
    p.x = ws + bdy.off; p.ldx = bdy.ld; p.x_coff = L.y_coff;
    if (L.act != ACT_NONE && !dy_is_du) { p.xa = ws + ba.off; p.xact = L.act; p.xalpha = L.alpha; }
    p.wp = ws + (upeff ? L.wuT_off : L.wpT_off); p.Kc = L.KcT; p.ldw = L.ldwT; p.kreal = L.cout;
    p.y = ws + bdx.off; p.ldy = bdx.ld; p.y_coff = dx_coff; p.Cout = L.cin;
    p.accumulate = accumulate;
    if (res >= 0) { p.res = ws + P->buf(res).off; p.ldres = P->buf(res).ld; p.res_coff = 0; }
    if (em.ubuf >= 0) {
      const Buf &bu = P->buf(em.ubuf), &bua = P->buf(em.abuf);
      p.uo = ws + bu.off; p.ldu = bu.ld; p.u_coff = dx_coff;
      p.ua = ws + bua.off; p.ldua = bua.ld; p.ua_coff = dx_coff;
      p.uact = em.act; p.ualpha = em.alpha; p.u_c0 = em.c0; p.u_c1 = em.c1;
    }
    if (L.winoT_off && !upeff) { p.wino_u = ws + L.winoT_off; p.wino_np = L.winoT_np; }
    fill_common(P, p, ws, ln.slot);
    p.f16_xscale = UDET_F16_GRAD_SCALE;
    UDET_TRY(launch_conv(p, s));
    if (P->profiling && (conv_last_config() & 0xff) == 9) P->prof.back()->mfma_scale = 4.0 / 9.0;
  }
  prof_end(P, s);
  return UDET_OK;
}

static int run_wgrad(Plan* P, const Layer& L, int N, int dy, bool dy_is_du, const float* w_flat, float* g_flat, float* ws, const Lane& ln) {
  hipStream_t s = ln.s;
  if (skip_launch(2, L.net)) return UDET_OK;
  const NetParams& np = net_params(L.net);
  const int act_buf = L.y2 >= 0 ? L.y2 : L.y;
  const Buf &bx = P->buf(L.x), &bdy = P->buf(dy), &ba = P->buf(act_buf);
  const int up = L.up ? 1 : 0;
  ConvParams g;
  memset(&g, 0, sizeof(g));
  conv_setup_fwd(g, N, L.H << up, L.W << up, L.kh, L.kw, L.stride, L.dil);
  WgradParams q;
  memset(&q, 0, sizeof(q));
  q.x = ws + bx.off; q.ldx = bx.ld; q.x_coff = L.x_coff;
  q.N = N; q.H = L.H << up; q.W = L.W << up; q.up_shift = up; q.Cin = L.cin;
  q.dy = ws + bdy.off; q.ldy = bdy.ld; q.y_coff = L.y_coff; q.Cout = L.cout;
  if (L.act != ACT_NONE && !dy_is_du) { q.ya = ws + ba.off; q.yact = L.act; q.yalpha = L.alpha; }
  q.OH = g.OH; q.OW = g.OW; q.isy = q.isx = L.stride;
  q.ntaps = g.ntaps;
  memcpy(q.taps, g.taps, sizeof(g.taps));
  q.dw = g_flat + np.p[L.w_idx].offset;
  q.db = g_flat + np.p[L.b_idx].offset;
  q.partial = ws + P->wgrad_off[ln.slot];
  q.zero16 = ws + P->small_off + 60000;
  q.partial_floats = P->wgrad_floats;
  q.f16 = P->cfg.conv_fp16;
  q.f16_yscale = UDET_F16_GRAD_SCALE;
  if (L.g_idx >= 0) {
    q.w = w_flat + np.p[L.w_idx].offset;
    q.b = w_flat + np.p[L.b_idx].offset;
    q.gamma = w_flat + np.p[L.g_idx].offset;
    q.dgamma = g_flat + np.p[L.g_idx].offset;
    q.dbeta = g_flat + np.p[L.be_idx].offset;
    q.bn_c = BN_C;
  }
  if (L.up && L.wu_off && L.g_idx >= 0 && dy_is_du) {
    ConvParams u;
    memset(&u, 0, sizeof(u));
    setup_up_fwd(u, N, L.H, L.W);
    q.H = L.H; q.W = L.W; q.up_shift = 0;
    q.OH = L.H; q.OW = L.W; q.isy = q.isx = 1;
    q.ycls = 1; q.OHf = 2 * L.H; q.OWf = 2 * L.W;
    q.ntaps = 16;
    memcpy(q.taps, u.taps, sizeof(u.taps));
    const size_t reserve = (size_t)16 * L.cin * L.cout + 64 * (size_t)L.cout + 1024;
    float* deff = ws + P->wgrad_off[ln.slot] + (P->wgrad_floats - reserve);
    float* pd = deff + (size_t)16 * L.cin * L.cout;
    q.partial_floats = P->wgrad_floats - reserve;
    float* dw = q.dw;
    float* db = q.db;
    q.dw = deff;
    const float *w_ = q.w, *b_ = q.b, *gamma_ = q.gamma;
    float *dgamma_ = q.dgamma, *dbeta_ = q.dbeta;
    q.w = q.b = q.gamma = nullptr; q.dgamma = q.dbeta = nullptr;
    prof_begin(P, PROF_CONV_WGRAD, layer_flops(L, N) * 4.0 / 9.0, layer_bytes(L, N), s, L.name.c_str());
    int rc = launch_wgrad_T(q, 16, s);
    if (rc == UDET_OK) rc = launch_wgrad_up_combine(deff, dw, L.cin, L.cout, s);
    if (rc == UDET_OK) rc = launch_bn_finalize(dw, 9, L.cin, L.cout, w_, b_, gamma_, BN_C, pd, db, dgamma_, dbeta_, s);
    prof_end(P, s);
    return rc;
  }
  prof_begin(P, PROF_CONV_WGRAD, layer_flops(L, N), layer_bytes(L, N), s, L.name.c_str());
  const int rc = launch_wgrad_T(q, L.kh * L.kw, s);
  if (P->profiling && (wgrad_last_config() >> 20) == 3) P->prof.back()->mfma_scale = 4.0 / 9.0;
  prof_end(P, s);
  return rc;
}

static bool pairs_on(const Plan* P, int dir = 0) { return !P->cfg.conv_fp16 && !((plan_knob(UDET_KNOB_NO_PAIRS) >> dir) & 1); }
static void fwd_params(Plan* P, const Layer& L, int N, float* ws, int slot, ConvParams& p) {
  const Buf &bx = P->buf(L.x), &by = P->buf(L.y);
  memset(&p, 0, sizeof(p));
  conv_setup_fwd(p, N, L.H, L.W, L.kh, L.kw, L.stride, L.dil);
  p.x = ws + bx.off; p.ldx = bx.ld; p.x_coff = L.x_coff;
  p.wp = ws + L.wp_off; p.Kc = L.Kc; p.ldw = L.ldw; p.bias = ws + L.bias_f_off;
  p.y = ws + by.off; p.ldy = by.ld; p.y_coff = L.y_coff; p.Cout = L.cout;
  p.act = L.act; p.alpha = L.alpha;
  if (L.res >= 0) { p.res = ws + P->buf(L.res).off; p.ldres = P->buf(L.res).ld; p.res_coff = L.res_coff; }
  if (L.y2 >= 0) { p.y2 = ws + P->buf(L.y2).off; p.ldy2 = P->buf(L.y2).ld; p.y2_coff = 0; }
  fill_common(P, p, ws, slot);
}
static bool plain_fwd_layer(const Layer& L) { return !L.transposed && !L.up && !L.upb && !L.col2im; }
static int run_fwd_pair(Plan* P, const Layer& La, int Na, const Layer& Lb, int Nb, float* ws, const Lane& ln) {
  if (!pairs_on(P) || !plain_fwd_layer(La) || !plain_fwd_layer(Lb)) {
    UDET_TRY(run_fwd(P, La, Na, ws, ln));
    return run_fwd(P, Lb, Nb, ws, ln);
  }
  if (skip_launch(0, La.net)) return UDET_OK;
  ConvParams a, b;
  fwd_params(P, La, Na, ws, ln.slot, a);
  fwd_params(P, Lb, Nb, ws, ln.slot, b);
  prof_begin(P, PROF_CONV_FWD, layer_flops(La, Na) + layer_flops(Lb, Nb), layer_bytes(La, Na) + layer_bytes(Lb, Nb), ln.s, (La.name + "+" + Lb.name).c_str());
  const int rc = launch_conv_pair(a, b, ln.s);
  prof_end(P, ln.s);
  return rc;
}
// ... 83 lines not shown
        j.T = T;
      }
      if (L.upb)
        for (int r = 0; r < 4; ++r) {
          j.T = 36; j.gamma_off = -1;
          j.dst_off = (long)(L.wupb_off + (size_t)r * 36 * L.Kc * L.ldw); j.R = L.cin; j.C = L.cout; j.Kc = L.Kc; j.ldw = L.ldw; j.k_split = L.k_split; j.k_gap = L.k_gap;
          j.mode = 9; j.beta_off = (long)((r & 1) * 3 + (r >> 1)); j.total = (long)L.Kc * L.ldw;
          jobs.push_back(j);
          if (L.upb_bwd) {
            j.dst_off = (long)(L.wupbT_off + (size_t)r * 36 * L.KcT * L.ldwT); j.Kc = L.KcT; j.ldw = L.ldwT; j.k_split = L.KcT; j.k_gap = 0;
            j.mode = 10; j.total = (long)L.KcT * L.ldwT;
            jobs.push_back(j);
          }
          j.T = T; j.beta_off = beoff;
        }
      if (L.wino_off) {
        j.dst_off = (long)L.wino_off; j.R = L.cin; j.C = L.cout; j.Kc = L.Kc; j.ldw = L.wino_np; j.k_split = L.k_split; j.k_gap = L.k_gap;
        j.mode = 7; j.total = (long)(L.Kc / 8) * 2 * L.wino_np;
        jobs.push_back(j);
      }
      if (L.winoT_off) {
        j.dst_off = (long)L.winoT_off; j.R = L.cin; j.C = L.cout; j.Kc = L.KcT; j.ldw = L.winoT_np; j.k_split = L.KcT; j.k_gap = 0;
        j.mode = 8; j.total = (long)(L.KcT / 8) * 2 * L.winoT_np;
        jobs.push_back(j);
      }
      j.src_off = (long)np.p[L.b_idx].offset; j.dst_off = (long)L.bias_f_off; j.mode = 2; j.total = L.cout;
      jobs.push_back(j);
    }
    if (jobs.size() > UDET_PACKJOB_CAP(layers.size())) {
      set_error("plan_init: %zu weight re-layout jobs for %zu layers exceed the table's %zu entries", jobs.size(), layers.size(),
                (size_t)UDET_PACKJOB_CAP(layers.size()));
      return UDET_ERR_ARG;
    }
    P->njobs[net] = (int)jobs.size();
    UDET_HIP(hipMemcpyAsync(ws + P->jobs_off[net], jobs.data(), jobs.size() * sizeof(PackJob), hipMemcpyHostToDevice, s));
    UDET_HIP(hipStreamSynchronize(s));
  }
  for (const auto& L : P->rec)
    if (L.upb)
      for (const Layer::SegLaunch* g : {&L.upb_f, &L.upb_b})
        if (g == &L.upb_f || L.upb_bwd)
          UDET_HIP(hipMemcpyAsync(ws + g->tab_off, g->taps.data(), g->taps.size() * sizeof(ConvTap), hipMemcpyHostToDevice, s));
  UDET_HIP(hipStreamSynchronize(s));
  P->pwc_packed = false;
  return UDET_OK;
}

static int pack_layer(const Layer& L, const float* w_flat, float* ws, const float* scale, bool trainable, hipStream_t s) {
  const NetParams& np = net_params(L.net);
  const float* w = w_flat + np.p[L.w_idx].offset;
  const int T = L.kh * L.kw;
  if (L.transposed)
    UDET_TRY(launch_pack_weights(w, ws + L.wp_off, T, L.cout, L.cin, L.Kc, L.ldw, L.k_split, L.k_gap, 1, nullptr, s));
  else
    UDET_TRY(launch_pack_weights(w, ws + L.wp_off, T, L.cin, L.cout, L.Kc, L.ldw, L.k_split, L.k_gap, 0, scale, s));
  if (trainable)
    UDET_TRY(launch_pack_weights(w, ws + L.wpT_off, T, L.cin, L.cout, L.KcT, L.ldwT, L.KcT, 0, 1, scale, s));
  if (L.col2im)
    UDET_TRY(launch_pack_taps_into_n(w, ws + L.wz_off, T, L.cin, L.cout, L.Kc, L.ldz, L.k_split, L.k_gap, L.transposed ? 1 : 0, s));
  if (L.wino_off && !trainable)
    UDET_TRY(launch_wino_pack(w, ws + L.wino_off, L.cin, L.cout, L.Kc, L.wino_np, L.k_split, L.k_gap, 0, s));
  return UDET_OK;
}

int plan_pack_pwc(Plan* P, const float* w, float* ws, hipStream_t s) {
  const NetParams& np = net_params(NET_PWC);
  for (const auto& L : P->pwc) {
    UDET_TRY(pack_layer(L, w, ws, nullptr, false, s));
    UDET_TRY(launch_copy_channels(w + np.p[L.b_idx].offset, L.cout, 0, ws + L.bias_f_off, L.cout, 0, 1, L.cout, 1.f, 0.f, s));
  }
  P->pwc_packed = true;
  return UDET_OK;
}

int plan_pack_trainable(Plan* P, const float* w_gen, const float* w_rec, float* ws, hipStream_t s) {
  if (w_gen)
    UDET_TRY(launch_pack_jobs(reinterpret_cast<const PackJob*>(ws + P->jobs_off[NET_GEN]), P->njobs[NET_GEN], w_gen, ws, BN_C, s));
  if (w_rec)
    UDET_TRY(launch_pack_jobs(reinterpret_cast<const PackJob*>(ws + P->jobs_off[NET_REC]), P->njobs[NET_REC], w_rec, ws, BN_C, s));
  return UDET_OK;
}

static const int PWC_CH[7] = {0, 16, 32, 64, 96, 128, 196};

static int pwc_forward_on(Plan* P, const float* img1, const float* img2, float* ws, const Lane& L0, const Lane& LH) {
  if (!P->pwc_packed) {
    set_error("pwc_forward: call udet_pack_pwc first");
    return UDET_ERR_ARG;
  }
  const Config& c = P->cfg;
  const int B = c.batch;
  hipStream_t s = L0.s;
  UDET_TRY(launch_pack_pwc_input(img1, img2, ws + P->buf(P->bid("pwc.x8")).off, (long)B * c.in_h * c.in_w, s));
  for (int l = 1; l <= 6; ++l)
    for (const char* suf : {"a", "aa", "b"}) {
      char nm[64];
      snprintf(nm, sizeof(nm), "pwcnet/featpyr/conv%d%s", l, suf);
      UDET_TRY(run_fwd(P, *find_layer(P->pwc, nm), 2 * B, ws, L0));
    }
  for (int l = 6; l >= 2; --l) {
    const int h = c.in_h >> l, w = c.in_w >> l, C = PWC_CH[l];
    const Buf& cb = P->buf(P->bid(S("pwc.c%d", l)));
    const Buf& slab = P->buf(P->bid(S("pwc.slab%d", l)));
    const float* c1 = ws + cb.off;
    const float* c2 = ws + cb.off + (size_t)B * h * w * C;
    const bool warped = l != 6;
    const double px = (double)B * h * w;
    prof_begin(P, PROF_CORR, 2.0 * px * 81.0 * C, px * ((warped ? 3.0 * C + 2.0 : 2.0 * C) + 81.0) * 4.0, s, S("warp_costvol%d", l).c_str());
    UDET_TRY(launch_warp_cost_volume(c1, c2, warped ? ws + slab.off : nullptr, slab.ld, 532 + C, 20.0f / (float)(1 << l), ws + slab.off,
                                     slab.ld, 448, warped ? 532 : -1, nullptr, B, h, w, C, s));
    prof_end(P, s);
    for (int i = 0; i < 5; ++i) UDET_TRY(run_fwd(P, *find_layer(P->pwc, S("pwcnet/predict_flow/conv%d_%d", l, i)), B, ws, L0));
    order_after(P, L0, LH);
    UDET_TRY(run_fwd(P, *find_layer(P->pwc, S("pwcnet/predict_flow/flow%d", l)), B, ws, LH));
    if (l != 2) UDET_TRY(run_fwd(P, *find_layer(P->pwc, S("pwcnet/upsample/up_feat%d", l)), B, ws, LH));
    for (int i = 1; i <= 6; ++i) UDET_TRY(run_fwd(P, *find_layer(P->pwc, S("pwcnet/ctxt/dc_conv%d%d", l, i)), B, ws, L0));
    order_after(P, LH, L0);
    UDET_TRY(run_fwd(P, *find_layer(P->pwc, S("pwcnet/ctxt/dc_conv%d%d", l, 7)), B, ws, L0));
    if (l != 2) UDET_TRY(run_fwd(P, *find_layer(P->pwc, S("pwcnet/upsample/up_flow%d", l)), B, ws, L0));
  }
  const Buf& fr = P->buf(P->bid("pwc.rflow2"));
  const Buf& ff = P->buf(P->bid("flow_full"));
  return launch_resize_bilinear_fwd(ws + fr.off, fr.ld, 0, B, fr.h, fr.w, ws + ff.off, 2, 0, c.in_h, c.in_w, 2, 4.0f, 1.f, s);
}

int plan_pwc_forward(Plan* P, const float* img1, const float* img2, float* ws, hipStream_t s) {
  P->ev_next = 0;
  if (P->prefetch_pending) (void)hipStreamWaitEvent(s, P->prefetch_ev, 0);
  return pwc_forward_on(P, img1, img2, ws, lane_of(P, s, 0), lane_of(P, s, 2));
}

static int plan_prepare_image(Plan* P, const float* img1, const char* dst, float* ws, hipStream_t s) {
  const Config& c = P->cfg;
  return launch_resize_bilinear_fwd(img1, 3, 0, c.batch, c.in_h, c.in_w, ws + P->buf(P->bid(dst)).off, 3, 0, c.img_h, c.img_w,
                                    3, 1.f, 1.f, s);
}
static int plan_prepare_flow(Plan* P, const char* dst, float* ws, hipStream_t s) {
  const Config& c = P->cfg;
  const Buf& ff = P->buf(P->bid("flow_full"));
  return launch_resize_bilinear_fwd(ws + ff.off, 2, 0, c.batch, c.in_h, c.in_w, ws + P->buf(P->bid(dst)).off, 2, 0, c.img_h,
                                    c.img_w, 2, 1.f, c.flow_normalizer, s);
}

int plan_prefetch(Plan* P, const float* img1, const float* img2, float* ws, hipStream_t s) {
  const Lane L0 = lane_of(P, s, 0), LC = lane_of(P, s, 4), LH = lane_of(P, s, 5);
  P->in_prefetch = true;
  P->ev_next_prefetch = 0;
  order_after(P, L0, LC);
  int rc = pwc_forward_on(P, img1, img2, ws, LC, LH);
  P->in_prefetch = false;
  UDET_TRY(rc);
  UDET_TRY(plan_prepare_flow(P, "flow.next", ws, LC.s));
  UDET_TRY(plan_prepare_image(P, img1, "image.next", ws, LC.s));
  if (!P->prefetch_ev) (void)hipEventCreateWithFlags(&P->prefetch_ev, hipEventDisableTiming);
  (void)hipEventRecord(P->prefetch_ev, LC.s);
  P->prefetch_pending = true;
  return UDET_OK;
}

int plan_generator_forward(Plan* P, float* ws, hipStream_t s) {
  const Config& c = P->cfg;
  const long HW = (long)c.img_h * c.img_w;
  const Lane L0 = lane_of(P, s, 0);
  double* part = reinterpret_cast<double*>(ws + P->small_off + 4096);
  UDET_TRY(launch_gen_input(ws + P->buf(P->bid("image")).off, ws + P->buf(P->bid("flow")).off, part,
                            ws + P->buf(P->bid("gen.in")).off, c.batch, HW, s));
  for (const auto& L : P->gen) UDET_TRY(run_fwd(P, L, c.batch, ws, L0));
  return UDET_OK;
}
int plan_generator_layers(Plan* P, float* ws, hipStream_t s) {
  const Lane L0 = lane_of(P, s, 0);
  for (const auto& L : P->gen) UDET_TRY(run_fwd(P, L, P->cfg.batch, ws, L0));
  return UDET_OK;
}

static int rec_resize(Plan* P, const char* src, const char* dst, int N, float* ws, hipStream_t s) {
  const Buf &a = P->buf(P->bid(src)), &b = P->buf(P->bid(dst));
  return launch_resize_bilinear_fwd(ws + a.off, a.ld, 0, N, a.h, a.w, ws + b.off, b.ld, 0, b.h, b.w, a.ld, 1.f, 1.f, s);
}

static const char* ENC_NAMES[9] = {"conv1", "conv2", "conv3", "conv31", "conv4", "conv41", "conv5", "conv51", "conv6"};

static int share_enc_a_output(Plan* P, const Layer& L, int ncalls, float* ws, hipStream_t s) {
  const Buf& y = P->buf(L.y);
  if (ncalls > 1 && (y.name.find("concat") != std::string::npos || y.name == "rec.conv6"))
    return launch_share_samples(ws + y.off, (long)P->cfg.batch * y.h * y.w, y.ld, L.y_coff, L.cout, ncalls, s);
  return UDET_OK;
}
static int plan_rec_image_branch(Plan* P, int ncalls, float* ws, const Lane& ln, bool with_layers = true) {
  const Config& c = P->cfg;
  if (ncalls < 1) return UDET_OK;
  const long Ppix = (long)c.batch * c.img_h * c.img_w;
  UDET_TRY(launch_pack_imgin(ws + P->buf(P->bid("image")).off, ws + P->buf(P->bid("rec.imgin")).off, Ppix, 1, ln.s));
  if (!with_layers) return UDET_OK;
  for (int i = 0; i < 9; ++i) {
    const Layer& L = *find_layer(P->rec, std::string("a") + ENC_NAMES[i]);
    UDET_TRY(run_fwd(P, L, c.batch, ws, ln));
    UDET_TRY(share_enc_a_output(P, L, ncalls, ws, ln.s));
  }
  P->enc_a_shared = true;
  return UDET_OK;
}

int plan_recover_forward(Plan* P, int ncalls, float* ws, hipStream_t s, bool inputs_prepacked, bool skip_enc_a, bool enc_a_input_packed) {
  const Config& c = P->cfg;
  const int B = c.batch, N = ncalls * B;
  const long Ppix = (long)B * c.img_h * c.img_w;
  const Lane L0 = lane_of(P, s, 0);
  if (!inputs_prepacked)
    UDET_TRY(launch_mask_rec_inputs(ws + P->buf(P->bid("gen.a17")).off, ws + P->buf(P->bid("flow")).off,
                                    ws + P->buf(P->bid("mask")).off, ws + P->buf(P->bid("rec.fin")).off, Ppix, ncalls, s));
  if (ncalls < 1) return UDET_OK;
  if (!skip_enc_a && pairs_on(P)) {
    if (!inputs_prepacked && !enc_a_input_packed) UDET_TRY(plan_rec_image_branch(P, ncalls, ws, L0, false));
    for (int i = 0; i < 9; ++i) {
      const Layer& La = *find_layer(P->rec, std::string("a") + ENC_NAMES[i]);
      UDET_TRY(run_fwd_pair(P, La, inputs_prepacked ? N : B, *find_layer(P->rec, std::string("b") + ENC_NAMES[i]), N, ws, L0));
      if (!inputs_prepacked) UDET_TRY(share_enc_a_output(P, La, ncalls, ws, s));
    }
    P->enc_a_shared = !inputs_prepacked;
  } else {
    if (!skip_enc_a) {
      if (inputs_prepacked) {
        for (int i = 0; i < 9; ++i) UDET_TRY(run_fwd(P, *find_layer(P->rec, std::string("a") + ENC_NAMES[i]), N, ws, L0));
        P->enc_a_shared = false;
      } else {
        UDET_TRY(plan_rec_image_branch(P, ncalls, ws, L0));
      }
    }
    for (int i = 0; i < 9; ++i) UDET_TRY(run_fwd(P, *find_layer(P->rec, std::string("b") + ENC_NAMES[i]), N, ws, L0));
  }
  for (int k = 5; k >= 1; --k) {
    const Layer& dcl = *find_layer(P->rec, S("deconv%d", k));
    if (!dcl.upb) UDET_TRY(rec_resize(P, k == 5 ? "rec.conv6" : S("rec.concat%d", k + 1).c_str(), S("rec.r%d", k + 1).c_str(), N, ws, s));
    UDET_TRY(run_fwd(P, dcl, N, ws, L0));
    if (k < 5) {
      UDET_TRY(rec_resize(P, S("rec.flow%d", k + 1).c_str(), S("rec.rf%d", k + 1).c_str(), N, ws, s));
      UDET_TRY(run_fwd(P, *find_layer(P->rec, S("upflow%d", k)), N, ws, L0));
    }
    UDET_TRY(run_fwd(P, *find_layer(P->rec, S("flow%d", k)), N, ws, L0));
  }
  const Buf& f1 = P->buf(P->bid("rec.flow1"));
  return launch_resize_bilinear_fwd(ws + f1.off, f1.ld, 0, N, f1.h, f1.w, ws + P->buf(P->bid("pred")).off, 2, 0, c.img_h,
                                    c.img_w, 2, 1.f, 1.f, s);
}

int plan_losses(Plan* P, float* ws, hipStream_t s) {
  const Config& c = P->cfg;
  float* sm = ws + P->small_off;
  const long HW = (long)c.img_h * c.img_w;
  return launch_losses(ws + P->buf(P->bid("flow")).off, ws + P->buf(P->bid("mask")).off, ws + P->buf(P->bid("pred")).off, HW,
                       c.batch, c.cbn, c.epsilon, (float)(c.img_w * c.img_h * c.batch), sm + 8192, sm, sm + 16, sm + UDET_SMALL_SUMS, s);
}

int plan_prefetch_consume(Plan* P, float* ws, hipStream_t s) {
  if (!P->prefetch_pending) {
    set_error("forward_prefetched: no udet_prefetch_flow is pending");
    return UDET_ERR_ARG;
  }
  (void)hipStreamWaitEvent(s, P->prefetch_ev, 0);
  P->prefetch_pending = false;
  const Buf &fn = P->buf(P->bid("flow.next")), &in = P->buf(P->bid("image.next"));
  UDET_HIP(hipMemcpyAsync(ws + P->buf(P->bid("flow")).off, ws + fn.off, fn.floats() * sizeof(float), hipMemcpyDeviceToDevice, s));
  UDET_HIP(hipMemcpyAsync(ws + P->buf(P->bid("image")).off, ws + in.off, in.floats() * sizeof(float), hipMemcpyDeviceToDevice, s));
  return UDET_OK;
}

int plan_forward(Plan* P, const float* img1, const float* img2, int ncalls, float* ws, hipStream_t s, bool prefetched) {
  P->ev_next = 0;
  const Lane L0 = lane_of(P, s, 0), LI = lane_of(P, s, 1);
  if (prefetched) {
    UDET_TRY(plan_prefetch_consume(P, ws, s));
    img1 = img2 = nullptr;
  } else if (img1 && P->prefetch_pending) {
    (void)hipStreamWaitEvent(s, P->prefetch_ev, 0);
  }
  order_after(P, L0, LI);
  if (img1) UDET_TRY(plan_prepare_image(P, img1, "image", ws, LI.s));
  hipEvent_t e_img = nullptr;
  if (LI.s != L0.s) {
    e_img = next_event(P);
    (void)hipEventRecord(e_img, LI.s);
  }
  const bool paired = pairs_on(P);
  UDET_TRY(plan_rec_image_branch(P, ncalls, ws, LI, !paired));
  if (img1) {
    UDET_TRY(pwc_forward_on(P, img1, img2, ws, L0, lane_of(P, s, 2)));
    UDET_TRY(plan_prepare_flow(P, "flow", ws, s));
  }
  if (e_img) (void)hipStreamWaitEvent(s, e_img, 0);
  UDET_TRY(plan_generator_forward(P, ws, s));
  order_after(P, LI, L0);
  UDET_TRY(plan_recover_forward(P, ncalls, ws, s, false, !paired, paired));
  if (ncalls == 3) UDET_TRY(plan_losses(P, ws, s));
  return UDET_OK;
}

static int rec_backward(Plan* P, int N, const char* dp, bool with_wgrad, bool need_dfin, const float* w_rec, float* g_rec, float* ws,
                        const Lane& LD, const Lane& LW, const Lane* LAp = nullptr, const Lane* LWdecp = nullptr) {
  const Config& c = P->cfg;
  hipStream_t s = LD.s;
  const std::string pre = std::string("rec.") + dp + ".", upre = std::string("rec.u") + dp + ".";
  auto B_ = [&](const std::string& n) { return P->bid(n); };
  auto D_ = [&](const std::string& n) { return P->bid(pre + n); };
  auto U_ = [&](const std::string& n) { return P->bid(upre + n); };
  auto Lr = [&](const std::string& n) { return find_layer(P->rec, n); };
  const Lane LWdec = LWdecp ? *LWdecp : LW;
  auto wgrad_on = [&](const Lane& lw, const Layer& L, int dy, bool is_du, int n) -> int {
    order_after(P, LD, lw);
    return run_wgrad(P, L, n < 0 ? N : n, dy, is_du, w_rec, g_rec, ws, lw);
  };
  auto wgrad = [&](const Layer& L, int dy, bool is_du, int n = -1) -> int { return wgrad_on(LW, L, dy, is_du, n); };
  auto wgrad_dec = [&](const Layer& L, int dy, bool is_du) -> int { return wgrad_on(LWdec, L, dy, is_du, -1); };
  const Lane LA = LAp ? *LAp : LD;
  const bool a_own_lane = LA.s != LD.s;
  const int ncopies = N / c.batch;
  const bool a_shared = P->enc_a_shared && ncopies > 1;
  const Emit none;
  const float LEAK = 0.2f;
  {
    const Buf& df1 = P->buf(D_("flow1"));
    UDET_TRY(launch_resize_bilinear_bwd(ws + P->buf(B_(std::string(dp) + ".pred")).off, 2, 0, N, c.img_h, c.img_w, ws + df1.off,
                                        df1.ld, 0, df1.h, df1.w, 2, 0, s));
  }
// ... 7 lines not shown
    UDET_TRY(run_dgrad(P, *fl, N, D_(S("flow%d", k)), false, dconcat, 0, k == 1 ? 0 : 1, -1, em, ws, LD));
    if (with_wgrad) UDET_TRY(wgrad_dec(*fl, D_(S("flow%d", k)), false));
    if (k < 5) {
      const Layer* uf = Lr(S("upflow%d", k));
      if (with_wgrad) UDET_TRY(wgrad_dec(*uf, dconcat, false));
      UDET_TRY(run_dgrad(P, *uf, N, dconcat, false, D_(S("rf%d", k + 1)), 0, 0, -1, none, ws, LD));
      const Buf &drf = P->buf(D_(S("rf%d", k + 1))), &dfn = P->buf(D_(S("flow%d", k + 1)));
      UDET_TRY(launch_resize_bilinear_bwd(ws + drf.off, drf.ld, 0, N, drf.h, drf.w, ws + dfn.off, dfn.ld, 0, dfn.h, dfn.w, drf.ld, 0, s));
    }
    if (with_wgrad) {
      if (dc->upb) {
        order_after(P, LD, LWdec);
        UDET_TRY(rec_resize(P, k == 5 ? "rec.conv6" : S("rec.concat%d", k + 1).c_str(), S("rec.r%d", k + 1).c_str(), N, ws, LWdec.s));
      }
      UDET_TRY(wgrad_dec(*dc, uconcat, true));
    }
    if (dc->upb_bwd) {
      UDET_TRY(run_dgrad_upb(P, *dc, N, uconcat, D_(S("p%d", k + 1)), D_(S("concat%d", k + 1)), ws, LD));
      continue;
    }
    const int dr = D_(S("r%d", k + 1));
    UDET_TRY(run_dgrad(P, *dc, N, uconcat, true, dr, 0, 0, -1, none, ws, LD));
    const Buf& bdr = P->buf(dr);
    const Buf& dsrc = P->buf(k == 5 ? D_("conv6") : D_(S("concat%d", k + 1)));
    UDET_TRY(launch_resize_bilinear_bwd(ws + bdr.off, bdr.ld, 0, N, bdr.h, bdr.w, ws + dsrc.off, dsrc.ld, 0, dsrc.h, dsrc.w,
                                        bdr.ld, 0, s));
  }
  {
    const Buf &d6 = P->buf(D_("conv6")), &a6 = P->buf(B_("rec.conv6")), &u6 = P->buf(U_("conv6"));
    UDET_TRY(launch_emit_du(ws + d6.off, ws + a6.off, ws + u6.off, (long)N * d6.h * d6.w, d6.ld, 0, d6.ld, ACT_LEAKY, LEAK, s));
  }
  if (a_own_lane) order_after(P, LD, LA);
  const bool pair_enc = pairs_on(P, 1) && with_wgrad && !a_own_lane;
  for (int i = 8; i >= 0; --i) {
    DgradJob job[2];
    int njob = 0;
    for (const char* e : {"a", "b"}) {
      if (e[0] == 'a' && !with_wgrad) continue;
      const Layer* L = Lr(std::string(e) + ENC_NAMES[i]);
      const int du = U_(P->buf(L->y).name.substr(4));
      const bool shared = e[0] == 'a' && a_shared;
      const int Ne = shared ? c.batch : N;
      const bool own = e[0] == 'a' && a_own_lane;
      const Lane& LE = own ? LA : LD;
      hipStream_t se = LE.s;
      if (shared && i == 8) {
        const Buf& u = P->buf(du);
        UDET_TRY(launch_fold_samples(ws + u.off, (long)c.batch * u.h * u.w, u.ld, L->y_coff, L->cout, ncopies, se));
      }
      if (with_wgrad) {
        if (own) UDET_TRY(run_wgrad(P, *L, Ne, du, true, w_rec, g_rec, ws, LA));
        else UDET_TRY(wgrad(*L, du, true, Ne));
      }
      if (i == 0) {
        if (e[0] == 'b' && need_dfin) UDET_TRY(run_dgrad(P, *L, N, du, true, D_("fin"), 0, 0, -1, none, ws, LD));
        continue;
      }
      const std::string xname = P->buf(L->x).name;
      const int dx = D_(xname.substr(4));
      const bool slab_in = xname.find("concat") != std::string::npos;
      Emit em;
      em.ubuf = U_(xname.substr(4)); em.abuf = L->x; em.c0 = 0; em.c1 = L->cin; em.act = ACT_LEAKY; em.alpha = LEAK;
      if (shared && slab_in) {
        const Buf& d = P->buf(dx);
        UDET_TRY(launch_fold_samples(ws + d.off, (long)c.batch * d.h * d.w, d.ld, L->x_coff, L->cin, ncopies, se));
      }
      if (pair_enc) {
        job[njob].L = L; job[njob].N = Ne; job[njob].dy = du; job[njob].dx = dx; job[njob].dx_coff = L->x_coff;
        job[njob].accumulate = slab_in ? 1 : 0; job[njob].em = em;
        ++njob;
        continue;
      }
      UDET_TRY(run_dgrad(P, *L, Ne, du, true, dx, L->x_coff, slab_in ? 1 : 0, -1, em, ws, LE));
    }
    if (njob == 2) UDET_TRY(run_dgrad_pair(P, job[0], job[1], ws, LD));
    else if (njob == 1) UDET_TRY(run_dgrad(P, *job[0].L, job[0].N, job[0].dy, true, job[0].dx, job[0].dx_coff, job[0].accumulate, -1, job[0].em, ws, LD));
  }
  if (a_own_lane) order_after(P, LA, LD);
  if (with_wgrad && LWdec.s != LW.s) order_after(P, LWdec, LD);
  return UDET_OK;
}

static int backward_recover(Plan* P, const float* w_rec, float* g_rec, float* ws, const Lane& LD, const Lane& LW, const Lane* LA = nullptr,
                            const Lane* LWdec = nullptr) {
  const Config& c = P->cfg;
  const long BHW = (long)c.batch * c.img_h * c.img_w;
  UDET_TRY(launch_rec_loss_bwd(ws + P->buf(P->bid("flow")).off, ws + P->buf(P->bid("mask")).off, ws + P->buf(P->bid("pred")).off,
                               ws + P->buf(P->bid("d.pred")).off, BHW, c.cbn, 1.0f / (float)(c.img_w * c.img_h * c.batch), LD.s));
  return rec_backward(P, 3 * c.batch, "d", true, false, w_rec, g_rec, ws, LD, LW, LA, LWdec);
}

static int backward_generator(Plan* P, const float* w_gen, float* g_gen, float* ws, const Lane& LD, const Lane& LW, const Lane* LWlate = nullptr,
                              int nlate = 0) {
  const Config& c = P->cfg;
  const int B = c.batch;
  const long HW = (long)c.img_h * c.img_w;
  hipStream_t s = LD.s;
  float* sm = ws + P->small_off;
  auto B_ = [&](const std::string& n) { return P->bid(n); };
  UDET_TRY(launch_gen_loss_bwd(ws + P->buf(B_("flow")).off, ws + P->buf(B_("mask")).off, ws + P->buf(B_("pred")).off, sm + 16,
                               ws + P->buf(B_("e.pred")).off, ws + P->buf(B_("d.mask")).off, HW, B, c.cbn, s));
  UDET_TRY(rec_backward(P, 2 * B, "e", false, true, nullptr, nullptr, ws, LD, LD));
  UDET_TRY(launch_mask_bwd(ws + P->buf(B_("d.mask")).off, ws + P->buf(B_("rec.e.fin")).off, ws + P->buf(B_("flow")).off,
                           ws + P->buf(B_("mask")).off, ws + P->buf(B_("gen.d17")).off, B * HW, s));
  for (int i = 16; i >= 0; --i) {
    const Layer& L = P->gen[i];
    const bool has_act = L.act != ACT_NONE;
    const int dy = has_act ? B_(S("gen.u%d", i + 1)) : B_(S("gen.d%d", i + 1));
    const Lane& LWi = (LWlate && i < nlate) ? *LWlate : LW;
    order_after(P, LD, LWi);
    UDET_TRY(run_wgrad(P, L, B, dy, has_act, w_gen, g_gen, ws, LWi));
    if (i == 0) break;
    int res = -1;
    if (i == 6) res = B_("gen.d11");
    if (i == 3) res = B_("gen.d14");
    if (i == 1) res = B_("gen.d15");
    const int dx = B_(S("gen.d%d", i));
    const Layer& Lp = P->gen[i - 1];
    const int ap = Lp.y2 >= 0 ? Lp.y2 : Lp.y;
    {
      Emit em;
      if (Lp.act != ACT_NONE) { em.ubuf = B_(S("gen.u%d", i)); em.abuf = ap; em.c0 = 0; em.c1 = L.cin; em.act = Lp.act; em.alpha = Lp.alpha; }
      UDET_TRY(run_dgrad(P, L, B, dy, has_act, dx, 0, 0, res, em, ws, LD));
    }
  }
  return UDET_OK;
}

int plan_backward(Plan* P, int which, const float* w_gen, const float* w_rec, float* g_gen, float* g_rec, float* ws, hipStream_t s) {
  P->ev_next = 0;
  const Lane L0 = lane_of(P, s, 0), L1 = lane_of(P, s, 1), L2 = lane_of(P, s, 2), L3 = lane_of(P, s, 3);
  auto mark = [&](int net) {
    if (!P->grad_ev[net]) (void)hipEventCreateWithFlags(&P->grad_ev[net], hipEventDisableTiming);
    (void)hipEventRecord(P->grad_ev[net], s);
  };
  if (which == 3) {
    order_after(P, L0, L1);
    const int la = (int)plan_knob(UDET_KNOB_ENC_A_LANE);
    const Lane LA = lane_of(P, s, la > 0 && la < Plan::NLANE ? la : 0);
    const int lw = (int)plan_knob(UDET_KNOB_REC_DEC_WGRAD_LANE), le = (int)plan_knob(UDET_KNOB_REC_ENC_WGRAD_LANE);
    const Lane LWD = lane_of(P, s, lw > 0 && lw < Plan::NLANE ? lw : 3);
    const Lane LWE = lane_of(P, s, le > 0 && le < Plan::NLANE ? le : 2);
    UDET_TRY(backward_recover(P, w_rec, g_rec, ws, L0, LWE, la > 0 ? &LA : nullptr, &LWD));
    if (LWE.s != L2.s) order_after(P, LWE, L0);
// ... 90 lines not shown
```

unsupervised_detection_amd/engine.py:

```python
from __future__ import annotations

import ctypes
from dataclasses import dataclass

import torch

from ._ffi import c_f, c_i, c_p, c_sz, check, lib
from .weights import NET_GEN, NET_REC


class _Cfg(ctypes.Structure):
    _fields_ = [("batch", c_i), ("in_h", c_i), ("in_w", c_i), ("img_h", c_i), ("img_w", c_i), ("flow_normalizer", c_f),
                ("cbn", c_f), ("epsilon", c_f), ("lr", c_f), ("beta1", c_f), ("beta2", c_f), ("adam_eps", c_f), ("clip", c_f),
                ("noise_seed", ctypes.c_ulonglong), ("conv_fp16", c_i)]


lib.udet_plan_create.restype = c_i
lib.udet_plan_create.argtypes = [ctypes.POINTER(_Cfg), ctypes.POINTER(c_p)]
lib.udet_plan_destroy.restype = None
lib.udet_plan_destroy.argtypes = [c_p]
lib.udet_workspace_bytes.restype = c_sz
lib.udet_workspace_bytes.argtypes = [c_p]
lib.udet_plan_init.restype = c_i
lib.udet_plan_init.argtypes = [c_p, c_p, c_p]
lib.udet_buffer_count.restype = c_i
lib.udet_buffer_count.argtypes = [c_p]
lib.udet_buffer_info.restype = c_i
lib.udet_buffer_info.argtypes = [c_p, c_i, ctypes.POINTER(ctypes.c_char_p), ctypes.POINTER(c_sz), ctypes.POINTER(c_i)]
lib.udet_plan_set_concurrent.restype = c_i
lib.udet_plan_set_concurrent.argtypes = [c_p, c_i]
lib.udet_plan_lane_queues.restype = c_i
lib.udet_plan_lane_queues.argtypes = [c_p, c_p, ctypes.POINTER(c_i)]
lib.udet_plan_pin_lanes.restype = c_i
lib.udet_plan_pin_lanes.argtypes = [c_p, c_p, ctypes.POINTER(c_p), c_i]
lib.udet_fp16_overflow_count.restype = ctypes.c_long
lib.udet_fp16_overflow_count.argtypes = [c_p]
lib.udet_get_adam_step.restype = ctypes.c_long
lib.udet_get_adam_step.argtypes = [c_p]
lib.udet_set_adam_step.restype = None
lib.udet_set_adam_step.argtypes = [c_p, ctypes.c_long]
for _n, _a in (("udet_pack_pwc", [c_p, c_p, c_p, c_p]), ("udet_pack_trainable", [c_p, c_p, c_p, c_p, c_p]),
               ("udet_pwc_forward", [c_p, c_p, c_p, c_p, c_p]), ("udet_forward", [c_p, c_p, c_p, c_i, c_p, c_p]),
               ("udet_forward_from_flow", [c_p, c_i, c_p, c_p]), ("udet_generator_forward", [c_p, c_p, c_p]),
               ("udet_recover_forward", [c_p, c_i, c_p, c_p]),
               ("udet_prefetch_flow", [c_p, c_p, c_p, c_p, c_p]), ("udet_forward_prefetched", [c_p, c_i, c_p, c_p]),
               ("udet_prefetch_consume", [c_p, c_p, c_p]),
               ("udet_backward", [c_p, c_i, c_p, c_p, c_p, c_p, c_p, c_p]),
               ("udet_apply", [c_p, c_i, c_p, c_p, c_p, c_p, c_p, c_p]),
               ("udet_train_step", [c_p, c_i] + [c_p] * 12)):
    getattr(lib, _n).restype = c_i
    getattr(lib, _n).argtypes = _a

lib.udet_autotune.restype = c_i
lib.udet_autotune.argtypes = [c_p] * 7
lib.udet_tuned_shapes.restype = c_i
lib.udet_tuned_shapes.argtypes = []
lib.udet_profile_begin.restype = c_i
lib.udet_profile_begin.argtypes = [c_p]
lib.udet_profile_end.restype = c_i
lib.udet_profile_end.argtypes = [c_p, ctypes.POINTER(ctypes.c_double), c_i, c_p]

GEN, REC, BOTH = 1, 2, 3
LOSS_KEYS = ("generator", "recover", "red_rate", "red_rate_compl", "reconstruction_loss", "reconstruction_compl_loss",
             "denominator_red_rate", "denominator_red_rate_compl")


@dataclass
class EngineConfig:
    batch_size: int = 4
    in_height: int = 384
    in_width: int = 640
    img_height: int = 192
    img_width: int = 384
    flow_normalizer: float = 80.0
    cbn: float = 0.5
    epsilon: float = 75.0
    beta1: float = 0.9
    lr: float = 1e-4
    beta2: float = 0.999
    adam_eps: float = 1e-8
    clip: float = 0.2
    noise_seed: int = 8964
    conv_fp16: bool = False

# ... 48 lines not shown

    def pack_pwc(self, w_pwc):
        check(lib.udet_pack_pwc(self._h, _ptr(w_pwc), self.ws.data_ptr(), self._stream()))

    def pack_trainable(self, w_gen=None, w_rec=None):
        check(lib.udet_pack_trainable(self._h, _ptr(w_gen), _ptr(w_rec), self.ws.data_ptr(), self._stream()))

    def _check_pair(self, img1, img2):
        c = self.cfg
        want = (c.batch_size, c.in_height, c.in_width, 3)
        for name, t in (("img1", img1), ("img2", img2)):
            if tuple(t.shape) != want:
                raise ValueError("%s has shape %s, this plan takes %s (pad the last batch of a one-pass reader: "
                                 "learner.pad_batch)" % (name, tuple(t.shape), want))

    def pwc_forward(self, img1, img2):
        self._check_pair(img1, img2)
        check(lib.udet_pwc_forward(self._h, _ptr(img1), _ptr(img2), self.ws.data_ptr(), self._stream()))
        return self.buffer("flow_full")

    def forward(self, img1, img2, ncalls=3):
        self._check_pair(img1, img2)
        check(lib.udet_forward(self._h, _ptr(img1), _ptr(img2), ncalls, self.ws.data_ptr(), self._stream()))

    def prefetch_flow(self, img1, img2):
        self._check_pair(img1, img2)
        self._prefetch_keep = (img1, img2)
        check(lib.udet_prefetch_flow(self._h, _ptr(img1), _ptr(img2), self.ws.data_ptr(), self._stream()))

    def prefetch_consume(self):
        check(lib.udet_prefetch_consume(self._h, self.ws.data_ptr(), self._stream()))
        self._prefetch_keep = None

    def forward_in_place(self, ncalls=3):
        check(lib.udet_forward_from_flow(self._h, ncalls, self.ws.data_ptr(), self._stream()))

    def forward_prefetched(self, ncalls=3):
        check(lib.udet_forward_prefetched(self._h, ncalls, self.ws.data_ptr(), self._stream()))
        self._prefetch_keep = None

    def forward_from_flow(self, image, flow, ncalls=3):
        if tuple(image.shape) != tuple(self.buffer("image").shape) or tuple(flow.shape) != tuple(self.buffer("flow").shape):
            raise ValueError("image / flow must be %s / %s" % (tuple(self.buffer("image").shape), tuple(self.buffer("flow").shape)))
        self.buffer("image").copy_(image)
        self.buffer("flow").copy_(flow)
        check(lib.udet_forward_from_flow(self._h, ncalls, self.ws.data_ptr(), self._stream()))

    def losses(self):
        v = self.buffer("losses").view(-1).cpu().tolist()
        return dict(zip(LOSS_KEYS, v))

    def backward(self, which, w_gen, w_rec, g_gen, g_rec):
        check(lib.udet_backward(self._h, which, _ptr(w_gen), _ptr(w_rec), _ptr(g_gen), _ptr(g_rec), self.ws.data_ptr(),
                                self._stream()))

    def apply(self, net, w, g, m, v):
        check(lib.udet_apply(self._h, net, _ptr(w), _ptr(g), _ptr(m), _ptr(v), self.ws.data_ptr(), self._stream()))

    def train_step(self, which, img1, img2, w_gen, w_rec, g_gen, g_rec, m_gen, v_gen, m_rec, v_rec):
        self._check_pair(img1, img2)
        check(lib.udet_train_step(self._h, which, _ptr(img1), _ptr(img2), _ptr(w_gen), _ptr(w_rec), _ptr(g_gen), _ptr(g_rec),
                                  _ptr(m_gen), _ptr(v_gen), _ptr(m_rec), _ptr(v_rec), self.ws.data_ptr(), self._stream()))

    def autotune(self, w_gen, w_rec, g_gen, g_rec):
        check(lib.udet_autotune(self._h, _ptr(w_gen), _ptr(w_rec), _ptr(g_gen), _ptr(g_rec), self.ws.data_ptr(), self._stream()))
        return int(lib.udet_tuned_shapes())

    def profile(self, fn):
# ... 37 lines not shown
```

unsupervised_detection_amd/trainer.py:

```python
from __future__ import annotations

import torch

from . import weights as W
from .engine import BOTH, GEN, REC, Engine


class TrainState:

    def __init__(self, engine: Engine, seed: int = 8964, w_pwc=None, w_gen=None, w_rec=None, autotune: bool = False):
        dev = engine.device
        self.engine = engine
        self.w_pwc = (w_pwc if w_pwc is not None else W.init_flat(W.NET_PWC, seed)).to(dev)
        self.w_gen = (w_gen if w_gen is not None else W.init_flat(W.NET_GEN, seed)).to(dev)
        self.w_rec = (w_rec if w_rec is not None else W.init_flat(W.NET_REC, seed)).to(dev)
        n_gen, n_rec = self.w_gen.numel(), self.w_rec.numel()
        off_rec = (n_gen + 63) // 64 * 64
        self.g_all = torch.zeros(off_rec + n_rec, dtype=torch.float32, device=dev)
        self.g_gen, self.g_rec = self.g_all[:n_gen], self.g_all[off_rec:off_rec + n_rec]
        self.m_gen, self.v_gen = torch.zeros_like(self.w_gen), torch.zeros_like(self.w_gen)
        self.m_rec, self.v_rec = torch.zeros_like(self.w_rec), torch.zeros_like(self.w_rec)
        engine.pack_pwc(self.w_pwc)
        engine.pack_trainable(self.w_gen, self.w_rec)
        self._dirty = 0
# ... 88 lines not shown
    with torch.cuda.stream(comm):
        allreduce_mean_(st.g_rec, group)
        done = comm.record_event()
    allreduce_mean_(st.g_gen, group)
    main.wait_event(done)


def train_step(st: TrainState, img1, img2, which: int = BOTH, group=None, next_pair=None):
    e = st.engine
    flush_weights(st)

    def call(fn, *a):
        if not getattr(e.cfg, "conv_fp16", False):
            return fn(*a)
        from ._ffi import UdetOverflow
        for _ in range(4):
            try:
                return fn(*a)
            except UdetOverflow as ex:
                st.overflow_skipped = getattr(st, "overflow_skipped", 0) + 1
                import sys
                print("[udet] fp16 overflow: an optimizer update was dropped (%d so far): %s" % (st.overflow_skipped, ex), file=sys.stderr)
        return fn(*a)

    if getattr(st, "_prefetched", None) is not None:
        p1, p2 = st._prefetched
        if p1.data_ptr() != img1.data_ptr() or p2.data_ptr() != img2.data_ptr():
            raise ValueError("train_step: this step's pair is not the one prefetched by the previous call")
        e.prefetch_consume()
        st._prefetched = None
        if next_pair is not None:
            e.prefetch_flow(next_pair[0], next_pair[1])
            st._prefetched = (next_pair[0], next_pair[1])
        call(e.forward_in_place, 3)
    else:
        call(e.forward, img1, img2, 3)
        if next_pair is not None:
            e.prefetch_flow(next_pair[0], next_pair[1])
            st._prefetched = (next_pair[0], next_pair[1])
    call(e.backward, which, st.w_gen, st.w_rec, st.g_gen, st.g_rec)
    _exchange_gradients(st, which, group)
    if which & GEN:
        e.apply(W.NET_GEN, st.w_gen, st.g_gen, st.m_gen, st.v_gen)
    if which & REC:
        e.apply(W.NET_REC, st.w_rec, st.g_rec, st.m_rec, st.v_rec)
    st._dirty = which & (GEN | REC)
```

Baseline: 501.2.

## Batch small kernels: deferred BN finish, packed weight jobs, fused prefetch consume and share-fold

Result: no change. 500.7 (-0.1%).

```diff
diff --git a/include/udet.h b/include/udet.h
--- a/include/udet.h
+++ b/include/udet.h
@@ -114,6 +114,7 @@
 int udet_forward_prefetched(udet_plan* plan, int ncalls, void* workspace, void* stream);
 int udet_prefetch_consume(udet_plan* plan, void* workspace, void* stream);
 int udet_forward_from_flow(udet_plan* plan, int ncalls, void* workspace, void* stream);
+int udet_forward_consumed(udet_plan* plan, int ncalls, void* workspace, void* stream);
 int udet_generator_forward(udet_plan* plan, void* workspace, void* stream);
 int udet_generator_layers(udet_plan* plan, void* workspace, void* stream);
 int udet_recover_forward(udet_plan* plan, int n, void* workspace, void* stream);
diff --git a/include/udet_debug.h b/include/udet_debug.h
--- a/include/udet_debug.h
+++ b/include/udet_debug.h
@@ -8,6 +8,9 @@
 void udet_debug_force_wgrad(int nsplit, int dma);
 int udet_debug_last_wgrad(void);
 void udet_debug_upb_min_pixels(long v);
+void udet_debug_chain_old_mask(unsigned mask);
+int udet_debug_grad_absmean(const float* g, const long* seg_off, const long* seg_len, int nvars, float* vpart, float thresh, float* out2,
+                            void* stream);
 void udet_debug_set_tuning(int on);
 void udet_debug_force_pair(int on);
 int udet_debug_last_pair(void);
diff --git a/unsupervised_detection_amd/_devel.py b/unsupervised_detection_amd/_devel.py
--- a/unsupervised_detection_amd/_devel.py
+++ b/unsupervised_detection_amd/_devel.py
@@ -19,6 +19,10 @@
 dbg.udet_debug_force_wgrad.argtypes = [ctypes.c_int, ctypes.c_int]
 dbg.udet_debug_upb_min_pixels.restype = None
 dbg.udet_debug_upb_min_pixels.argtypes = [ctypes.c_long]
+dbg.udet_debug_chain_old_mask.restype = None
+dbg.udet_debug_chain_old_mask.argtypes = [ctypes.c_uint]
+dbg.udet_debug_grad_absmean.restype = ctypes.c_int
+dbg.udet_debug_grad_absmean.argtypes = [ctypes.c_void_p] * 3 + [ctypes.c_int, ctypes.c_void_p, ctypes.c_float, ctypes.c_void_p, ctypes.c_void_p]
 dbg.udet_debug_set_tuning.restype = None
 dbg.udet_debug_set_tuning.argtypes = [ctypes.c_int]
 dbg.udet_debug_last_wgrad.restype = ctypes.c_int
diff --git a/unsupervised_detection_amd/csrc/api_plan.hip b/unsupervised_detection_amd/csrc/api_plan.hip
--- a/unsupervised_detection_amd/csrc/api_plan.hip
+++ b/unsupervised_detection_amd/csrc/api_plan.hip
@@ -91,6 +91,11 @@
   UDET_TRY(plan_check_overflow(h->p, false));
   if (ncalls < 0 || ncalls > 3) { set_error("forward: ncalls must be 0..3"); return UDET_ERR_ARG; }
   return plan_forward(h->p, nullptr, nullptr, ncalls, (float*)ws, (hipStream_t)stream);
+}
+int udet_forward_consumed(udet_plan* h, int ncalls, void* ws, void* stream) {
+  UDET_TRY(plan_check_overflow(h->p, false));
+  if (ncalls < 0 || ncalls > 3) { set_error("forward: ncalls must be 0..3"); return UDET_ERR_ARG; }
+  return plan_forward(h->p, nullptr, nullptr, ncalls, (float*)ws, (hipStream_t)stream, false, true);
 }
 int udet_generator_forward(udet_plan* h, void* ws, void* stream) {
   UDET_TRY(plan_generator_forward(h->p, (float*)ws, (hipStream_t)stream));
diff --git a/unsupervised_detection_amd/csrc/common.h b/unsupervised_detection_amd/csrc/common.h
--- a/unsupervised_detection_amd/csrc/common.h
+++ b/unsupervised_detection_amd/csrc/common.h
@@ -149,6 +149,7 @@
 struct PackJob {
   long src_off, dst_off, gamma_off, beta_off;
   long total;
+  int blk0, nblk;
   int T, R, C, Kc, ldw, k_split, k_gap, mode;
 };
 
@@ -184,7 +185,26 @@
   int f16;
   float f16_yscale;
 };
-int launch_wgrad_T(WgradParams& p, int T, hipStream_t stream);
+struct BnFinishJob {
+  const float *pd, *pbias, *b, *gamma;
+  float *dgamma, *dbeta, *db;
+  float bn_c;
+  int Cout, ldn, nsplit, nb;
+};
+#define UDET_BN_JOBS 16
+struct BnFinishJobs {
+  int n = 0;
+  int blk0[UDET_BN_JOBS + 1] = {0};
+  BnFinishJob j[UDET_BN_JOBS];
+};
+struct WgradBnDefer {
+  float* pd;
+  float* pbias;
+  size_t pbias_floats;
+  BnFinishJobs* table;
+};
+int launch_wgrad_T(WgradParams& p, int T, hipStream_t stream, WgradBnDefer* defer = nullptr);
+int launch_bn_finish_jobs(const BnFinishJobs& t, hipStream_t stream);
 int launch_bn_finalize(float* dw, int T, int Cin, int Cout, const float* w, const float* b, const float* gamma, float bn_c, float* pd,
                        float* db, float* dgamma, float* dbeta, hipStream_t stream);
 int launch_wgrad_up_combine(const float* deff, float* dw, int Cin, int Cout, hipStream_t stream);
diff --git a/unsupervised_detection_amd/csrc/conv_host.h b/unsupervised_detection_amd/csrc/conv_host.h
--- a/unsupervised_detection_amd/csrc/conv_host.h
+++ b/unsupervised_detection_amd/csrc/conv_host.h
@@ -53,7 +53,8 @@
                         int mode, const float* scale, hipStream_t stream);
 int launch_pack_taps_into_n(const float* src, float* dst, int T, int R, int C, int Kc, int ldz, int k_split, int k_gap,
                             int transposed, hipStream_t stream);
-int launch_pack_jobs(const PackJob* jobs_dev, int njobs, const float* wsrc, float* ws, float bn_c, hipStream_t stream);
+int launch_pack_jobs(const PackJob* jobs_dev, int njobs, const int* blkmap_dev, int nblocks, const float* wsrc, float* ws, float bn_c,
+                     hipStream_t stream);
 int launch_fold_bn(const float* b, const float* gamma, const float* beta, float c, float* scale, float* bias_f, int n,
                    hipStream_t stream);
 int launch_copy_channels(const float* src, int lds, int s_coff, float* dst, int ldd, int d_coff, long P, int C, float mul,
diff --git a/unsupervised_detection_amd/csrc/conv_host.hip b/unsupervised_detection_amd/csrc/conv_host.hip
--- a/unsupervised_detection_amd/csrc/conv_host.hip
+++ b/unsupervised_detection_amd/csrc/conv_host.hip
@@ -128,20 +128,21 @@
      {{1.f, 1.f, 0.f, 0.f}, {0.f, 0.f, 0.f, 0.f}, {0.f, 0.f, 0.f, 0.f}},
      {{0.f, .5f, 0.f, 0.f}, {0.f, -.5f, -1.f, -.5f}, {0.f, 0.f, 0.f, -.5f}}}};
 
-__global__ __launch_bounds__(256) void pack_jobs_kernel(const PackJob* __restrict__ jobs, const float* __restrict__ wsrc,
-                                                        float* __restrict__ ws, float bn_c) {
-  const PackJob j = jobs[blockIdx.y];
+__global__ __launch_bounds__(256) void pack_jobs_kernel(const PackJob* __restrict__ jobs, const int* __restrict__ blkmap,
+                                                        const float* __restrict__ wsrc, float* __restrict__ ws, float bn_c) {
+  const PackJob j = jobs[blkmap ? blkmap[blockIdx.x] : blockIdx.y];
+  const int lb = blkmap ? (int)blockIdx.x - j.blk0 : (int)blockIdx.x, nb = blkmap ? j.nblk : (int)gridDim.x;
   const float* src = wsrc + j.src_off;
   float* dst = ws + j.dst_off;
   const float* gamma = j.gamma_off >= 0 ? wsrc + j.gamma_off : nullptr;
   if (j.mode == 2) {
-    for (long e = (long)blockIdx.x * 256 + threadIdx.x; e < j.total; e += (long)gridDim.x * 256)
+    for (long e = (long)lb * 256 + threadIdx.x; e < j.total; e += (long)nb * 256)
       dst[e] = gamma ? src[e] * (gamma[e] * bn_c) + wsrc[j.beta_off + e] : src[e];
     return;
   }
   if (j.mode == 9 || j.mode == 10) {
     const int rv = (int)(j.beta_off / 3), cv = (int)(j.beta_off % 3);
-    for (long e = (long)blockIdx.x * 256 + threadIdx.x; e < j.total; e += (long)gridDim.x * 256) {
+    for (long e = (long)lb * 256 + threadIdx.x; e < j.total; e += (long)nb * 256) {
       const int n = (int)(e % j.ldw), k = (int)(e / j.ldw);
       int ks = k;
       if (k >= j.k_split) ks = (k < j.k_split + j.k_gap) ? -1 : k - j.k_gap;
@@ -181,10 +182,10 @@
     return;
   }
   if (j.mode == 7 || j.mode == 8) {
-    for (long e = (long)blockIdx.x * 256 + threadIdx.x; e < j.total; e += (long)gridDim.x * 256) wino_pack_item(j, src, gamma, bn_c, dst, e);
+    for (long e = (long)lb * 256 + threadIdx.x; e < j.total; e += (long)nb * 256) wino_pack_item(j, src, gamma, bn_c, dst, e);
     return;
   }
-  for (long e = (long)blockIdx.x * 256 + threadIdx.x; e < j.total; e += (long)gridDim.x * 256) {
+  for (long e = (long)lb * 256 + threadIdx.x; e < j.total; e += (long)nb * 256) {
     const int n = (int)(e % j.ldw);
     const int k = (int)((e / j.ldw) % j.Kc);
     int t = (int)(e / ((long)j.ldw * j.Kc));
@@ -218,9 +219,11 @@
     dst[e] = v;
   }
 }
-int launch_pack_jobs(const PackJob* jobs_dev, int njobs, const float* wsrc, float* ws, float bn_c, hipStream_t stream) {
+int launch_pack_jobs(const PackJob* jobs_dev, int njobs, const int* blkmap_dev, int nblocks, const float* wsrc, float* ws, float bn_c,
+                     hipStream_t stream) {
   if (njobs < 1) return UDET_OK;
-  UDET_LAUNCH(pack_jobs_kernel, dim3(48, njobs), dim3(256), 0, stream, jobs_dev, wsrc, ws, bn_c);
+  if (blkmap_dev && nblocks > 0) UDET_LAUNCH(pack_jobs_kernel, dim3(nblocks), dim3(256), 0, stream, jobs_dev, blkmap_dev, wsrc, ws, bn_c);
+  else UDET_LAUNCH(pack_jobs_kernel, dim3(48, njobs), dim3(256), 0, stream, jobs_dev, (const int*)nullptr, wsrc, ws, bn_c);
   UDET_HIP(hipGetLastError());
   return UDET_OK;
 }
diff --git a/unsupervised_detection_amd/csrc/conv_wgrad.hip b/unsupervised_detection_amd/csrc/conv_wgrad.hip
--- a/unsupervised_detection_amd/csrc/conv_wgrad.hip
+++ b/unsupervised_detection_amd/csrc/conv_wgrad.hip
@@ -495,44 +495,59 @@
     pd[(size_t)blockIdx.x * p.Cout + co] = d;
   }
 }
-__global__ __launch_bounds__(256) void wgrad_bn_finish2_kernel(const WgradParams p, int ldn, int nsplit, int nb, const float* __restrict__ pd) {
+__device__ __forceinline__ void wgrad_bn_finish2_body(const BnFinishJob& j, int blk) {
   __shared__ float red[256];
   __shared__ float redS[256];
-  const int t = threadIdx.x, cl = t & 31, rg = t >> 5, co = blockIdx.x * 32 + cl;
+  const float* __restrict__ pd = j.pd;
+  const float* __restrict__ pbias = j.pbias;
+  const int ldn = j.ldn, nsplit = j.nsplit, nb = j.nb, Cout = j.Cout;
+  const int t = threadIdx.x, cl = t & 31, rg = t >> 5, co = blk * 32 + cl;
   const int per = (nb + 7) / 8, b0 = rg * per, b1 = b0 + per < nb ? b0 + per : nb;
   const int pers = (nsplit + 7) / 8, k0 = rg * pers, k1 = k0 + pers < nsplit ? k0 + pers : nsplit;
   float d = 0.f, S = 0.f;
-  if (co < p.Cout) {
+  if (co < Cout) {
     int b = b0;
     for (; b + 11 < b1; b += 12) {
       float a[12];
 #pragma unroll
-      for (int u = 0; u < 12; ++u) a[u] = pd[(size_t)(b + u) * p.Cout + co];
+      for (int u = 0; u < 12; ++u) a[u] = pd[(size_t)(b + u) * Cout + co];
 #pragma unroll
       for (int u = 0; u < 12; ++u) d += a[u];
     }
-    for (; b < b1; ++b) d += pd[(size_t)b * p.Cout + co];
+    for (; b < b1; ++b) d += pd[(size_t)b * Cout + co];
     int k = k0;
     for (; k + 7 < k1; k += 8) {
       float a[8];
 #pragma unroll
-      for (int u = 0; u < 8; ++u) a[u] = p.pbias[(size_t)(k + u) * ldn + co];
+      for (int u = 0; u < 8; ++u) a[u] = pbias[(size_t)(k + u) * ldn + co];
 #pragma unroll
       for (int u = 0; u < 8; ++u) S += a[u];
     }
-    for (; k < k1; ++k) S += p.pbias[(size_t)k * ldn + co];
+    for (; k < k1; ++k) S += pbias[(size_t)k * ldn + co];
   }
   red[t] = d;
   redS[t] = S;
   __syncthreads();
-  if (rg == 0 && co < p.Cout) {
+  if (rg == 0 && co < Cout) {
     float dsum = red[cl], Ssum = redS[cl];
 #pragma unroll
     for (int g = 1; g < 8; ++g) { dsum += red[g * 32 + cl]; Ssum += redS[g * 32 + cl]; }
-    p.dgamma[co] = p.bn_c * (dsum + p.b[co] * Ssum);
-    p.dbeta[co] = Ssum;
-    p.db[co] = p.gamma[co] * p.bn_c * Ssum;
-  }
+    j.dgamma[co] = j.bn_c * (dsum + j.b[co] * Ssum);
+    j.dbeta[co] = Ssum;
+    j.db[co] = j.gamma[co] * j.bn_c * Ssum;
+  }
+}
+__global__ __launch_bounds__(256) void wgrad_bn_finish2_kernel(const BnFinishJob j) { wgrad_bn_finish2_body(j, blockIdx.x); }
+__global__ __launch_bounds__(256) void wgrad_bn_finish2_jobs_kernel(const BnFinishJobs t) {
+  int j = 0;
+  while (j + 1 < t.n && (int)blockIdx.x >= t.blk0[j + 1]) ++j;
+  wgrad_bn_finish2_body(t.j[j], (int)blockIdx.x - t.blk0[j]);
+}
+int launch_bn_finish_jobs(const BnFinishJobs& t, hipStream_t stream) {
+  if (t.n < 1) return UDET_OK;
+  UDET_LAUNCH(wgrad_bn_finish2_jobs_kernel, dim3(t.blk0[t.n]), dim3(256), 0, stream, t);
+  UDET_HIP(hipGetLastError());
+  return UDET_OK;
 }
 __global__ __launch_bounds__(256) void bn_dot_kernel(const float* __restrict__ w, const float* __restrict__ g, int R, int C,
                                                      float* __restrict__ pd) {
@@ -628,7 +643,8 @@
   else UDET_LAUNCH((conv_wgrad_kernel<BM, BN, WM_, WN_>), grid, dim3(256), 0, stream, p, co_tiles, nsplit);
 }
 
-int launch_wgrad_T(WgradParams& p, int T, hipStream_t stream) {
+int launch_wgrad_T(WgradParams& p, int T, hipStream_t stream, WgradBnDefer* defer) {
+  bool final_run = false;
   if (conv_debug_f16_on()) p.f16 = 1;
   if (p.f16 && !(p.f16_yscale > 0.f)) p.f16_yscale = 1.f;
   if (p.f16 && g_wtuning) p.f16_yscale = 1.f;
@@ -705,13 +721,15 @@
     if (dma != 3 && !dma_ok) dma = 0;
     if (dma == 3) ns = wgrad_wino_slices(g, ns > (int)maxs ? (int)maxs : ns);
     WgradParams q = g;
-    q.pbias = base;
+    auto deferred = [&](int n) { return final_run && fused_bn && defer && defer->table->n < UDET_BN_JOBS && (size_t)n * ldn <= defer->pbias_floats; };
+    q.pbias = deferred(ns) ? defer->pbias : base;
     q.partial = base + (size_t)ns * bgroups * ldn;
     if (dma == 3 && launch_wgrad_wino(q, ns, ldn, stream) != UDET_OK) {
       dma = dma_ok ? 1 : 0;
       ns = nsplit & 0xfffff;
       if (ns > cap) ns = cap;
       if (ns < 1) ns = 1;
+      q.pbias = deferred(ns) ? defer->pbias : base;
       q.partial = base + (size_t)ns * bgroups * ldn;
     }
     if (dma == 3) {}
@@ -727,13 +745,25 @@
       int rb = rg / sl;
       while ((Mreal + rb - 1) / rb > BNR_MAXBLK) rb *= 2;
       const int nb = (Mreal + rb - 1) / rb;
-#define UDET_RBN(CW_, SL_) UDET_LAUNCH((wgrad_reduce_bn_kernel<CW_, SL_>), dim3(nb), dim3(256), 0, stream, q, ldn, ns, rb, pd)
+      const bool dfr = deferred(ns);
+      float* pdl = dfr ? defer->pd : pd;
+#define UDET_RBN(CW_, SL_) UDET_LAUNCH((wgrad_reduce_bn_kernel<CW_, SL_>), dim3(nb), dim3(256), 0, stream, q, ldn, ns, rb, pdl)
       if (cw == 128) { if (sl == 2) UDET_RBN(128, 2); else UDET_RBN(128, 1); }
       else if (cw == 64) { if (sl == 4) UDET_RBN(64, 4); else if (sl == 2) UDET_RBN(64, 2); else UDET_RBN(64, 1); }
       else if (cw == 32) { if (sl == 8) UDET_RBN(32, 8); else if (sl == 4) UDET_RBN(32, 4); else if (sl == 2) UDET_RBN(32, 2); else UDET_RBN(32, 1); }
       else { if (sl == 8) UDET_RBN(16, 8); else if (sl == 4) UDET_RBN(16, 4); else if (sl == 2) UDET_RBN(16, 2); else UDET_RBN(16, 1); }
 #undef UDET_RBN
-      UDET_LAUNCH(wgrad_bn_finish2_kernel, dim3((g.Cout + 31) / 32), dim3(256), 0, stream, q, ldn, ns, nb, pd);
+      BnFinishJob fj;
+      fj.pd = pdl; fj.pbias = q.pbias; fj.b = q.b; fj.gamma = q.gamma; fj.dgamma = q.dgamma; fj.dbeta = q.dbeta; fj.db = q.db;
+      fj.bn_c = q.bn_c; fj.Cout = q.Cout; fj.ldn = ldn; fj.nsplit = ns; fj.nb = nb;
+      if (dfr) {
+        BnFinishJobs& t = *defer->table;
+        t.j[t.n] = fj;
+        t.blk0[t.n + 1] = t.blk0[t.n] + (g.Cout + 31) / 32;
+        ++t.n;
+        return UDET_OK;
+      }
+      UDET_LAUNCH(wgrad_bn_finish2_kernel, dim3((g.Cout + 31) / 32), dim3(256), 0, stream, fj);
       return UDET_OK;
     }
     const int sl = (ns >= 64 && total * 64 <= 262144) ? 64 : ((ns >= 8 && total * 8 <= 262144) ? 8 : 1);
@@ -841,6 +871,7 @@
   if ((nsplit >> 20) == 3 && !wino_ok) nsplit = (nsplit & 0xfffff) | ((dma_ok ? 1 : 0) << 20);
   if ((nsplit >> 20) == 3) nsplit = wgrad_wino_slices(g, (nsplit & 0xfffff) > (int)maxs ? (int)maxs : (nsplit & 0xfffff)) | (3 << 20);
   g_wlast = nsplit;
+  final_run = true;
   UDET_TRY(run(nsplit));
   UDET_HIP(hipGetLastError());
   int nbw = (int)((wsz + 255) / 256);
diff --git a/unsupervised_detection_amd/csrc/devel/api_debug.hip b/unsupervised_detection_amd/csrc/devel/api_debug.hip
--- a/unsupervised_detection_amd/csrc/devel/api_debug.hip
+++ b/unsupervised_detection_amd/csrc/devel/api_debug.hip
@@ -13,6 +13,11 @@
 void udet_debug_force_wgrad(int nsplit, int dma) { wgrad_force(nsplit, dma); }
 int udet_debug_last_wgrad(void) { return wgrad_last_config(); }
 void udet_debug_upb_min_pixels(long v) { plan_debug_upb_min_pixels(v); }
+void udet_debug_chain_old_mask(unsigned mask) { plan_debug_chain_old_mask(mask); }
+int udet_debug_grad_absmean(const float* g, const long* seg_off, const long* seg_len, int nvars, float* vpart, float thresh, float* out2,
+                            void* stream) {
+  return launch_grad_absmean(g, seg_off, seg_len, nvars, vpart, thresh, out2, (hipStream_t)stream);
+}
 void udet_debug_force_pair(int on) { conv_force_pair(on); }
 int udet_debug_last_pair(void) { return conv_last_pair(); }
 int udet_debug_conv2d_pair(const float* xa, const float* xb, const float* wa, const float* wb, const float* ba, const float* bb, float* ya, float* yb,
diff --git a/unsupervised_detection_amd/csrc/elementwise.h b/unsupervised_detection_amd/csrc/elementwise.h
--- a/unsupervised_detection_amd/csrc/elementwise.h
+++ b/unsupervised_detection_amd/csrc/elementwise.h
@@ -9,11 +9,23 @@
 int launch_upb_ring_fold(const float* dxh, int ld, int N, int H, int W, float* dx, hipStream_t s);
 int launch_share_samples(float* buf, long P, int ld, int coff, int C, int copies, hipStream_t s);
 int launch_fold_samples(float* buf, long P, int ld, int coff, int C, int copies, hipStream_t s);
+#define UDET_SHARE_JOBS 8
+struct ShareJobs {
+  int n = 0;
+  int blk0[UDET_SHARE_JOBS + 1] = {0};
+  long off[UDET_SHARE_JOBS], P[UDET_SHARE_JOBS];
+  int ld[UDET_SHARE_JOBS], coff[UDET_SHARE_JOBS], C[UDET_SHARE_JOBS];
+};
+bool share_jobs_add(ShareJobs& t, size_t off, long P, int ld, int coff, int C);
+int launch_share_fold_jobs(float* ws, const ShareJobs& t, int copies, bool fold, hipStream_t s);
 int launch_emit_du(const float* d, const float* a, float* u, long P, int ld, int coff, int C, int act, float alpha, hipStream_t s);
 int launch_pool2x2_sum(const float* du, float* dx, int N, int H, int W, int C, hipStream_t s);
 int launch_pack_pwc_input(const float* i1, const float* i2, float* x8, long P, hipStream_t s);
 int launch_gen_input(const float* img, const float* f, double* part, float* gin, int B, long HW, hipStream_t s);
 size_t flow_stats_doubles(int B);
+int launch_flow_stats(const float* f, double* part, int B, long HW, hipStream_t s);
+int launch_consume_prefetch(const float* img, const float* f, const double* part, float* io, float* fo, float* gin, float* imgin, int B,
+                            long HW, hipStream_t s);
 int launch_mask_rec_inputs(const float* logits, const float* f, float* mask, float* fin, long P, int ncalls, hipStream_t s);
 int launch_pack_imgin(const float* img, float* imgin, long P, int ncalls, hipStream_t s);
 int launch_losses(const float* f, const float* mask, const float* pred, long HW, int B, float cbn, float eps,
diff --git a/unsupervised_detection_amd/csrc/elementwise.hip b/unsupervised_detection_amd/csrc/elementwise.hip
--- a/unsupervised_detection_amd/csrc/elementwise.hip
+++ b/unsupervised_detection_amd/csrc/elementwise.hip
@@ -370,6 +370,44 @@
   UDET_HIP(hipGetLastError());
   return UDET_OK;
 }
+template <bool FOLD>
+__global__ __launch_bounds__(256) void share_fold_jobs_kernel(float* __restrict__ ws, const ShareJobs t, int copies) {
+  int j = 0;
+  while (j + 1 < t.n && (int)blockIdx.x >= t.blk0[j + 1]) ++j;
+  float* buf = ws + t.off[j];
+  const long P = t.P[j];
+  const int ld = t.ld[j], coff = t.coff[j], CV = t.C[j] / 4;
+  const long total = P * CV, stride = (long)(t.blk0[j + 1] - t.blk0[j]) * 256;
+  for (long e = (long)((int)blockIdx.x - t.blk0[j]) * 256 + threadIdx.x; e < total; e += stride) {
+    const long pix = e / CV;
+    const long o = pix * ld + coff + (e - pix * CV) * 4;
+    float4 v = *reinterpret_cast<const float4*>(buf + o);
+    for (int k = 1; k < copies; ++k) {
+      float4* q = reinterpret_cast<float4*>(buf + o + (long)k * P * ld);
+      if (FOLD) {
+        const float4 w = *q;
+        v.x += w.x; v.y += w.y; v.z += w.z; v.w += w.w;
+      } else {
+        *q = v;
+      }
+    }
+    if (FOLD) *reinterpret_cast<float4*>(buf + o) = v;
+  }
+}
+bool share_jobs_add(ShareJobs& t, size_t off, long P, int ld, int coff, int C) {
+  if (t.n >= UDET_SHARE_JOBS || C < 4 || (ld % 4) || (coff % 4) || (C % 4) || (off % 4)) return false;
+  const int j = t.n++;
+  t.off[j] = (long)off; t.P[j] = P; t.ld[j] = ld; t.coff[j] = coff; t.C[j] = C;
+  t.blk0[j + 1] = t.blk0[j] + grid_for(P * (C / 4));
+  return true;
+}
+int launch_share_fold_jobs(float* ws, const ShareJobs& t, int copies, bool fold, hipStream_t s) {
+  if (copies < 2 || t.n < 1) return UDET_OK;
+  if (fold) hipLaunchKernelGGL(share_fold_jobs_kernel<true>, dim3(t.blk0[t.n]), dim3(256), 0, s, ws, t, copies);
+  else hipLaunchKernelGGL(share_fold_jobs_kernel<false>, dim3(t.blk0[t.n]), dim3(256), 0, s, ws, t, copies);
+  UDET_HIP(hipGetLastError());
+  return UDET_OK;
+}
 int launch_share_samples(float* buf, long P, int ld, int coff, int C, int copies, hipStream_t s) {
   return launch_share_fold(buf, P, ld, coff, C, copies, false, s);
 }
@@ -438,6 +476,46 @@
   return UDET_OK;
 }
 size_t flow_stats_doubles(int B) { return (size_t)B * FS_BLOCKS * 4; }
+int launch_flow_stats(const float* f, double* part, int B, long HW, hipStream_t s) {
+  hipLaunchKernelGGL(flow_stats_kernel, dim3(FS_BLOCKS, B), dim3(256), 0, s, f, HW, part);
+  UDET_HIP(hipGetLastError());
+  return UDET_OK;
+}
+__global__ __launch_bounds__(256) void consume_prefetch_kernel(const float* __restrict__ img, const float* __restrict__ f,
+                                                               const double* __restrict__ part, float* __restrict__ io,
+                                                               float* __restrict__ fo, float* __restrict__ gin,
+                                                               float* __restrict__ imgin, long HW) {
+  __shared__ float st[4];
+  const int n = blockIdx.y;
+  if (threadIdx.x < 2) {
+    double s = 0, q = 0;
+    for (int b = 0; b < FS_BLOCKS; ++b) {
+      s += part[((long)n * FS_BLOCKS + b) * 4 + threadIdx.x];
+      q += part[((long)n * FS_BLOCKS + b) * 4 + 2 + threadIdx.x];
+    }
+    const double mean = s / (double)HW, var = q / (double)HW - mean * mean;
+    st[threadIdx.x] = (float)mean;
+    st[2 + threadIdx.x] = sqrtf((float)var);
+  }
+  __syncthreads();
+  const float m0 = st[0], m1 = st[1], d0 = st[2], d1 = st[3];
+  for (long p = (long)blockIdx.x * 256 + threadIdx.x; p < HW; p += (long)gridDim.x * 256) {
+    const long q = (long)n * HW + p;
+    const float2 v = *reinterpret_cast<const float2*>(f + q * 2);
+    const float i0 = img[q * 3], i1 = img[q * 3 + 1], i2 = img[q * 3 + 2];
+    *reinterpret_cast<float2*>(fo + q * 2) = v;
+    io[q * 3] = i0; io[q * 3 + 1] = i1; io[q * 3 + 2] = i2;
+    *reinterpret_cast<float4*>(gin + q * 8) = make_float4(i0, i1, i2, (v.x - m0) / d0);
+    *reinterpret_cast<float4*>(gin + q * 8 + 4) = make_float4((v.y - m1) / d1, 0.f, 0.f, 0.f);
+    *reinterpret_cast<float4*>(imgin + q * 4) = make_float4(i0, i1, i2, 0.f);
+  }
+}
+int launch_consume_prefetch(const float* img, const float* f, const double* part, float* io, float* fo, float* gin, float* imgin, int B,
+                            long HW, hipStream_t s) {
+  hipLaunchKernelGGL(consume_prefetch_kernel, dim3(grid_for(HW, 256), B), dim3(256), 0, s, img, f, part, io, fo, gin, imgin, HW);
+  UDET_HIP(hipGetLastError());
+  return UDET_OK;
+}
 __global__ __launch_bounds__(256) void flow_normalize_kernel(const float* __restrict__ f, const double* __restrict__ part,
                                                              float* __restrict__ out, long HW) {
   __shared__ float st[4];
@@ -541,14 +619,27 @@
     o[0] = R; o[1] = Rc; o[2] = Pp; o[3] = Dr; o[4] = Dc;
   }
 }
-__global__ void loss_finish_kernel(const float* __restrict__ part, int B, float eps, float num_pixels,
-                                   float* __restrict__ losses, float* __restrict__ coef, float* __restrict__ sums) {
-  if (threadIdx.x != 0 || blockIdx.x != 0) return;
+__global__ __launch_bounds__(256) void loss_finish_kernel(const float* __restrict__ part, int B, float eps, float num_pixels,
+                                                          float* __restrict__ losses, float* __restrict__ coef, float* sums) {
+  for (int e = threadIdx.x; e < B * 5; e += blockDim.x) {
+    const int b = e / 5, j = e - b * 5;
+    const float* p = part + (long)b * LS_BLOCKS * 5 + j;
+    float a = 0.f;
+    for (int k = 0; k < LS_BLOCKS; k += 8) {
+      float t[8];
+#pragma unroll
+      for (int u = 0; u < 8; ++u) t[u] = p[(k + u) * 5];
+#pragma unroll
+      for (int u = 0; u < 8; ++u) a += t[u];
+    }
+    sums[e] = a;
+  }
+  __syncthreads();
+  if (threadIdx.x != 0) return;
   float red = 0.f, redc = 0.f, rs = 0.f;
   for (int b = 0; b < B; ++b) {
-    float v[5] = {0, 0, 0, 0, 0};
-    for (int k = 0; k < LS_BLOCKS; ++k)
-      for (int j = 0; j < 5; ++j) v[j] += part[((long)b * LS_BLOCKS + k) * 5 + j];
+    float v[5];
+    for (int j = 0; j < 5; ++j) v[j] = sums[b * 5 + j];
     const float D = v[3] + eps, Dc = v[4] + eps;
     red += 1.f - v[0] / D;
     redc += 1.f - v[1] / Dc;
@@ -557,7 +648,6 @@
     coef[b * 4 + 1] = v[0] / (B * D * D);
     coef[b * 4 + 2] = -1.f / (B * Dc);
     coef[b * 4 + 3] = v[1] / (B * Dc * Dc);
-    for (int j = 0; j < 5; ++j) sums[b * 5 + j] = v[j];
     if (b == 0) { losses[4] = v[0]; losses[5] = v[1]; losses[6] = D; losses[7] = Dc; }
   }
   red /= B; redc /= B;
@@ -569,7 +659,7 @@
 int launch_losses(const float* f, const float* mask, const float* pred, long HW, int B, float cbn, float eps,
                   float num_pixels, float* part, float* losses, float* coef, float* sums, hipStream_t s) {
   hipLaunchKernelGGL(loss_sums_kernel, dim3(LS_BLOCKS, B), dim3(256), 0, s, f, mask, pred, HW, B, cbn, part);
-  hipLaunchKernelGGL(loss_finish_kernel, dim3(1), dim3(64), 0, s, part, B, eps, num_pixels, losses, coef, sums);
+  hipLaunchKernelGGL(loss_finish_kernel, dim3(1), dim3(B * 5 <= 64 ? 64 : 256), 0, s, part, B, eps, num_pixels, losses, coef, sums);
   UDET_HIP(hipGetLastError());
   return UDET_OK;
 }
@@ -697,15 +787,26 @@
   const float s = block_sum((s0 + s1) + (s2 + s3), sm);
   if (threadIdx.x == 0) vpart[blockIdx.x * GA_SPLIT + blockIdx.y] = s;
 }
-__global__ void grad_flag_kernel(const float* __restrict__ vpart, const long* __restrict__ seg_len, int nvars, float thresh,
-                                 float* __restrict__ out ) {
-  if (threadIdx.x == 0 && blockIdx.x == 0) {
-    float s = 0.f;
-    for (int i = 0; i < nvars; ++i) {
+__global__ __launch_bounds__(256) void grad_flag_kernel(const float* __restrict__ vpart, const long* __restrict__ seg_len, int nvars,
+                                                        float thresh, float* __restrict__ out ) {
+  __shared__ float q[256];
+  float s = 0.f;
+  for (int i0 = 0; i0 < nvars; i0 += 256) {
+    const int i = i0 + threadIdx.x;
+    if (i < nvars) {
       float v = 0.f;
+#pragma unroll
       for (int j = 0; j < GA_SPLIT; ++j) v += vpart[i * GA_SPLIT + j];
-      s += v / (float)seg_len[i];
-    }
+      q[threadIdx.x] = v / (float)seg_len[i];
+    }
+    __syncthreads();
+    if (threadIdx.x == 0) {
+      const int n = min(256, nvars - i0);
+      for (int k = 0; k < n; ++k) s += q[k];
+    }
+    __syncthreads();
+  }
+  if (threadIdx.x == 0) {
     s /= (float)nvars;
     out[0] = s;
     out[1] = s < thresh ? 1.f : 0.f;
@@ -714,7 +815,7 @@
 int launch_grad_absmean(const float* g, const long* seg_off, const long* seg_len, int nvars, float* vmean, float thresh,
                         float* out, hipStream_t s) {
   hipLaunchKernelGGL(grad_absmean_kernel, dim3(nvars, GA_SPLIT), dim3(256), 0, s, g, seg_off, seg_len, vmean);
-  hipLaunchKernelGGL(grad_flag_kernel, dim3(1), dim3(64), 0, s, vmean, seg_len, nvars, thresh, out);
+  hipLaunchKernelGGL(grad_flag_kernel, dim3(1), dim3(256), 0, s, vmean, seg_len, nvars, thresh, out);
   UDET_HIP(hipGetLastError());
   return UDET_OK;
 }
diff --git a/unsupervised_detection_amd/csrc/plan.h b/unsupervised_detection_amd/csrc/plan.h
--- a/unsupervised_detection_amd/csrc/plan.h
+++ b/unsupervised_detection_amd/csrc/plan.h
@@ -4,6 +4,7 @@
 #include <vector>
 
 #include "common.h"
+#include "elementwise.h"
 
 namespace udet {
 
@@ -43,6 +44,7 @@
   int KcT = 0, ldwT = 0;
   size_t wpT_off = 0;
   size_t bias_f_off = 0, scale_off = 0;
+  size_t bn_fin_off = 0;
   size_t wu_off = 0, wuT_off = 0;
   size_t wino_off = 0, winoT_off = 0;
   int wino_np = 0, winoT_np = 0;
@@ -94,11 +96,15 @@
   hipEvent_t prefetch_ev = nullptr;
   hipEvent_t grad_ev[3] = {nullptr, nullptr, nullptr};
   bool prefetch_pending = false;
+  bool prefetch_has_stats = false;
+  bool inputs_packed = false;
   std::vector<hipEvent_t> ev_pool, ev_pool_prefetch;
   size_t ev_next = 0, ev_next_prefetch = 0;
   bool in_prefetch = false;
   bool concurrent = true;
   bool enc_a_shared = false;
+  ShareJobs enc_a_share;
+  int enc_a_share_state = 0;
   size_t scratch_off[NLANE] = {}, scratch_floats = 0;
   size_t wgrad_off[NLANE] = {}, wgrad_floats = 0;
   ~Plan();
@@ -107,6 +113,8 @@
   size_t seg_off[3] = {0, 0, 0};
   size_t jobs_off[3] = {0, 0, 0};
   int njobs[3] = {0, 0, 0};
+  size_t jobmap_off[3] = {0, 0, 0};
+  int njobblk[3] = {0, 0, 0};
   struct ProfRec {
     int cat; double flops, bytes; hipEvent_t a, b; std::string name;
     double mfma_scale = 1.0;
@@ -129,11 +137,16 @@
 };
 
 #define UDET_PACKJOB_CAP(layers) (8 * (layers) + 32)
+#define UDET_PACKJOB_MAXBLK 16384
 #define UDET_SMALL_NOISE 256
 #define UDET_SMALL_OVF 300
 #define UDET_SMALL_SUMS 1024
 Plan* plan_build(const Config& cfg);
 void plan_debug_upb_min_pixels(long v);
+enum { UDET_CHAIN_PREFETCH = 1, UDET_CHAIN_SHARE = 2, UDET_CHAIN_BNFIN = 4, UDET_CHAIN_PACK = 8 };
+#define UDET_BN_PBIAS_FLOATS ((size_t)1024 * 128)
+void plan_debug_chain_old_mask(unsigned mask);
+bool plan_chain_old(unsigned bit);
 enum { UDET_KNOB_ENC_A_LANE = 0, UDET_KNOB_REC_DEC_WGRAD_LANE = 1, UDET_KNOB_REC_ENC_WGRAD_LANE = 2, UDET_KNOB_GEN_WGRAD_LATE = 3, UDET_KNOB_NO_WGRAD_WINO = 6, UDET_KNOB_SKIP = 7, UDET_KNOB_NO_PAIRS = 8, UDET_KNOB_COUNT = 12 };
 #ifdef UDET_EXPERIMENT
 void plan_debug_knob(int id, long v);
@@ -146,7 +159,8 @@
 int plan_pack_pwc(Plan* P, const float* w_pwc, float* ws, hipStream_t s);
 int plan_pack_trainable(Plan* P, const float* w_gen, const float* w_rec, float* ws, hipStream_t s);
 int plan_pwc_forward(Plan* P, const float* img1, const float* img2, float* ws, hipStream_t s);
-int plan_forward(Plan* P, const float* img1, const float* img2, int ncalls, float* ws, hipStream_t s, bool prefetched = false);
+int plan_forward(Plan* P, const float* img1, const float* img2, int ncalls, float* ws, hipStream_t s, bool prefetched = false,
+                 bool consumed = false);
 int plan_prefetch(Plan* P, const float* img1, const float* img2, float* ws, hipStream_t s);
 int plan_prefetch_consume(Plan* P, float* ws, hipStream_t s);
 int plan_generator_forward(Plan* P, float* ws, hipStream_t s);
diff --git a/unsupervised_detection_amd/csrc/plan_build.hip b/unsupervised_detection_amd/csrc/plan_build.hip
--- a/unsupervised_detection_amd/csrc/plan_build.hip
+++ b/unsupervised_detection_amd/csrc/plan_build.hip
@@ -177,6 +177,9 @@
 
 static long g_upb_bwd_min = 8192;
 void plan_debug_upb_min_pixels(long v) { g_upb_bwd_min = v < 0 ? 8192 : v; }
+static unsigned g_chain_old = 0;
+void plan_debug_chain_old_mask(unsigned mask) { g_chain_old = mask; }
+bool plan_chain_old(unsigned bit) { return (g_chain_old & bit) != 0; }
 #ifdef UDET_EXPERIMENT
 static long g_knob[UDET_KNOB_COUNT] = {};
 void plan_debug_knob(int id, long v) { if (id >= 0 && id < UDET_KNOB_COUNT) g_knob[id] = v; }
@@ -555,6 +558,11 @@
     P->wgrad_off[l] = off;
     if (l < 4) off = align64(off + P->wgrad_floats);
   }
+  for (auto& L : P->gen)
+    if (L.g_idx >= 0) {
+      L.bn_fin_off = off;
+      off = align64(off + (size_t)1024 * L.cout + UDET_BN_PBIAS_FLOATS);
+    }
   P->small_off = off;
   off = align64(off + 65536);
   P->ticket_off = off;
@@ -567,6 +575,8 @@
     const size_t nl = net == NET_GEN ? P->gen.size() : P->rec.size();
     P->jobs_off[net] = off;
     off = align64(off + UDET_PACKJOB_CAP(nl) * (sizeof(PackJob) / sizeof(float)) + 64);
+    P->jobmap_off[net] = off;
+    off = align64(off + UDET_PACKJOB_MAXBLK);
   }
   P->arena_floats = off;
   if (const char* e = getenv("UDET_SERIAL")) P->concurrent = atoi(e) == 0;
diff --git a/unsupervised_detection_amd/csrc/plan_exec.hip b/unsupervised_detection_amd/csrc/plan_exec.hip
--- a/unsupervised_detection_amd/csrc/plan_exec.hip
+++ b/unsupervised_detection_amd/csrc/plan_exec.hip
@@ -370,7 +370,8 @@
   return UDET_OK;
 }
 
-static int run_wgrad(Plan* P, const Layer& L, int N, int dy, bool dy_is_du, const float* w_flat, float* g_flat, float* ws, const Lane& ln) {
+static int run_wgrad(Plan* P, const Layer& L, int N, int dy, bool dy_is_du, const float* w_flat, float* g_flat, float* ws, const Lane& ln,
+                     BnFinishJobs* fin = nullptr) {
   hipStream_t s = ln.s;
   if (skip_launch(2, L.net)) return UDET_OK;
   const NetParams& np = net_params(L.net);
@@ -431,7 +432,14 @@
     return rc;
   }
   prof_begin(P, PROF_CONV_WGRAD, layer_flops(L, N), layer_bytes(L, N), s, L.name.c_str());
-  const int rc = launch_wgrad_T(q, L.kh * L.kw, s);
+  WgradBnDefer defer;
+  if (fin && L.bn_fin_off) {
+    defer.pd = ws + L.bn_fin_off;
+    defer.pbias = defer.pd + (size_t)1024 * L.cout;
+    defer.pbias_floats = UDET_BN_PBIAS_FLOATS;
+    defer.table = fin;
+  }
+  const int rc = launch_wgrad_T(q, L.kh * L.kw, s, fin && L.bn_fin_off ? &defer : nullptr);
   if (P->profiling && (wgrad_last_config() >> 20) == 3) P->prof.back()->mfma_scale = 4.0 / 9.0;
   prof_end(P, s);
   return rc;
@@ -581,8 +589,23 @@
                 (size_t)UDET_PACKJOB_CAP(layers.size()));
       return UDET_ERR_ARG;
     }
+    std::vector<int> blkmap;
+    for (int shrink = 1; ; shrink *= 2) {
+      blkmap.clear();
+      for (size_t i = 0; i < jobs.size(); ++i) {
+        PackJob& j = jobs[i];
+        const long weight = (j.mode == 9 || j.mode == 10) ? 16 : ((j.mode == 7 || j.mode == 8) ? 8 : 1);
+        long nb = (j.total * weight + 2047) / 2048 / shrink;
+        j.nblk = (int)(nb < 1 ? 1 : (nb > 1024 ? 1024 : nb));
+        j.blk0 = (int)blkmap.size();
+        blkmap.insert(blkmap.end(), (size_t)j.nblk, (int)i);
+      }
+      if (blkmap.size() <= UDET_PACKJOB_MAXBLK) break;
+    }
     P->njobs[net] = (int)jobs.size();
+    P->njobblk[net] = (int)blkmap.size();
     UDET_HIP(hipMemcpyAsync(ws + P->jobs_off[net], jobs.data(), jobs.size() * sizeof(PackJob), hipMemcpyHostToDevice, s));
+    UDET_HIP(hipMemcpyAsync(ws + P->jobmap_off[net], blkmap.data(), blkmap.size() * sizeof(int), hipMemcpyHostToDevice, s));
     UDET_HIP(hipStreamSynchronize(s));
   }
   for (const auto& L : P->rec)
@@ -623,10 +646,13 @@
 }
 
 int plan_pack_trainable(Plan* P, const float* w_gen, const float* w_rec, float* ws, hipStream_t s) {
-  if (w_gen)
-    UDET_TRY(launch_pack_jobs(reinterpret_cast<const PackJob*>(ws + P->jobs_off[NET_GEN]), P->njobs[NET_GEN], w_gen, ws, BN_C, s));
-  if (w_rec)
-    UDET_TRY(launch_pack_jobs(reinterpret_cast<const PackJob*>(ws + P->jobs_off[NET_REC]), P->njobs[NET_REC], w_rec, ws, BN_C, s));
+  const bool flat = !plan_chain_old(UDET_CHAIN_PACK);
+  for (int net = NET_GEN; net <= NET_REC; ++net) {
+    const float* w = net == NET_GEN ? w_gen : w_rec;
+    if (!w) continue;
+    UDET_TRY(launch_pack_jobs(reinterpret_cast<const PackJob*>(ws + P->jobs_off[net]), P->njobs[net],
+                              flat ? reinterpret_cast<const int*>(ws + P->jobmap_off[net]) : nullptr, flat ? P->njobblk[net] : 0, w, ws, BN_C, s));
+  }
   return UDET_OK;
 }
 
@@ -691,6 +717,10 @@
                                     c.img_w, 2, 1.f, c.flow_normalizer, s);
 }
 
+static double* prefetch_stats(Plan* P, float* ws) { return reinterpret_cast<double*>(ws + P->small_off + 32768); }
+static bool prefetch_stats_fit(Plan* P) {
+  return 8192 + loss_part_floats(P->cfg.batch) <= 32768 && 32768 + 2 * flow_stats_doubles(P->cfg.batch) <= 60000;
+}
 int plan_prefetch(Plan* P, const float* img1, const float* img2, float* ws, hipStream_t s) {
   const Lane L0 = lane_of(P, s, 0), LC = lane_of(P, s, 4), LH = lane_of(P, s, 5);
   P->in_prefetch = true;
@@ -701,6 +731,9 @@
   UDET_TRY(rc);
   UDET_TRY(plan_prepare_flow(P, "flow.next", ws, LC.s));
   UDET_TRY(plan_prepare_image(P, img1, "image.next", ws, LC.s));
+  P->prefetch_has_stats = !plan_chain_old(UDET_CHAIN_PREFETCH) && prefetch_stats_fit(P);
+  if (P->prefetch_has_stats)
+    UDET_TRY(launch_flow_stats(ws + P->buf(P->bid("flow.next")).off, prefetch_stats(P, ws), P->cfg.batch, (long)P->cfg.img_h * P->cfg.img_w, LC.s));
   if (!P->prefetch_ev) (void)hipEventCreateWithFlags(&P->prefetch_ev, hipEventDisableTiming);
   (void)hipEventRecord(P->prefetch_ev, LC.s);
   P->prefetch_pending = true;
@@ -730,22 +763,43 @@
 
 static const char* ENC_NAMES[9] = {"conv1", "conv2", "conv3", "conv31", "conv4", "conv41", "conv5", "conv51", "conv6"};
 
+static bool enc_a_output_is_shared(Plan* P, const Layer& L) {
+  const Buf& y = P->buf(L.y);
+  return y.name.find("concat") != std::string::npos || y.name == "rec.conv6";
+}
 static int share_enc_a_output(Plan* P, const Layer& L, int ncalls, float* ws, hipStream_t s) {
   const Buf& y = P->buf(L.y);
-  if (ncalls > 1 && (y.name.find("concat") != std::string::npos || y.name == "rec.conv6"))
+  if (ncalls > 1 && enc_a_output_is_shared(P, L))
     return launch_share_samples(ws + y.off, (long)P->cfg.batch * y.h * y.w, y.ld, L.y_coff, L.cout, ncalls, s);
   return UDET_OK;
 }
-static int plan_rec_image_branch(Plan* P, int ncalls, float* ws, const Lane& ln, bool with_layers = true) {
+static bool enc_a_share_jobs(Plan* P) {
+  if (P->enc_a_share_state == 0) {
+    P->enc_a_share_state = 1;
+    for (int i = 0; i < 9; ++i) {
+      const Layer& L = *find_layer(P->rec, std::string("a") + ENC_NAMES[i]);
+      if (!enc_a_output_is_shared(P, L)) continue;
+      const Buf& y = P->buf(L.y);
+      if (!share_jobs_add(P->enc_a_share, y.off, (long)P->cfg.batch * y.h * y.w, y.ld, L.y_coff, L.cout)) P->enc_a_share_state = -1;
+    }
+  }
+  return P->enc_a_share_state > 0;
+}
+static int share_enc_a_level(Plan* P, int i, int ncalls, float* ws, hipStream_t s) {
+  if (plan_chain_old(UDET_CHAIN_SHARE) || !enc_a_share_jobs(P))
+    return share_enc_a_output(P, *find_layer(P->rec, std::string("a") + ENC_NAMES[i]), ncalls, ws, s);
+  return i == 8 ? launch_share_fold_jobs(ws, P->enc_a_share, ncalls, false, s) : UDET_OK;
+}
+static int plan_rec_image_branch(Plan* P, int ncalls, float* ws, const Lane& ln, bool with_layers = true, bool imgin_packed = false) {
   const Config& c = P->cfg;
   if (ncalls < 1) return UDET_OK;
   const long Ppix = (long)c.batch * c.img_h * c.img_w;
-  UDET_TRY(launch_pack_imgin(ws + P->buf(P->bid("image")).off, ws + P->buf(P->bid("rec.imgin")).off, Ppix, 1, ln.s));
+  if (!imgin_packed) UDET_TRY(launch_pack_imgin(ws + P->buf(P->bid("image")).off, ws + P->buf(P->bid("rec.imgin")).off, Ppix, 1, ln.s));
   if (!with_layers) return UDET_OK;
   for (int i = 0; i < 9; ++i) {
     const Layer& L = *find_layer(P->rec, std::string("a") + ENC_NAMES[i]);
     UDET_TRY(run_fwd(P, L, c.batch, ws, ln));
-    UDET_TRY(share_enc_a_output(P, L, ncalls, ws, ln.s));
+    UDET_TRY(share_enc_a_level(P, i, ncalls, ws, ln.s));
   }
   P->enc_a_shared = true;
   return UDET_OK;
@@ -765,7 +819,7 @@
     for (int i = 0; i < 9; ++i) {
       const Layer& La = *find_layer(P->rec, std::string("a") + ENC_NAMES[i]);
       UDET_TRY(run_fwd_pair(P, La, inputs_prepacked ? N : B, *find_layer(P->rec, std::string("b") + ENC_NAMES[i]), N, ws, L0));
-      if (!inputs_prepacked) UDET_TRY(share_enc_a_output(P, La, ncalls, ws, s));
+      if (!inputs_prepacked) UDET_TRY(share_enc_a_level(P, i, ncalls, ws, s));
     }
     P->enc_a_shared = !inputs_prepacked;
   } else {
@@ -810,16 +864,29 @@
   (void)hipStreamWaitEvent(s, P->prefetch_ev, 0);
   P->prefetch_pending = false;
   const Buf &fn = P->buf(P->bid("flow.next")), &in = P->buf(P->bid("image.next"));
+  P->inputs_packed = false;
+  if (P->prefetch_has_stats && !plan_chain_old(UDET_CHAIN_PREFETCH)) {
+    const Config& c = P->cfg;
+    UDET_TRY(launch_consume_prefetch(ws + in.off, ws + fn.off, prefetch_stats(P, ws), ws + P->buf(P->bid("image")).off,
+                                     ws + P->buf(P->bid("flow")).off, ws + P->buf(P->bid("gen.in")).off,
+                                     ws + P->buf(P->bid("rec.imgin")).off, c.batch, (long)c.img_h * c.img_w, s));
+    P->inputs_packed = true;
+    return UDET_OK;
+  }
   UDET_HIP(hipMemcpyAsync(ws + P->buf(P->bid("flow")).off, ws + fn.off, fn.floats() * sizeof(float), hipMemcpyDeviceToDevice, s));
   UDET_HIP(hipMemcpyAsync(ws + P->buf(P->bid("image")).off, ws + in.off, in.floats() * sizeof(float), hipMemcpyDeviceToDevice, s));
   return UDET_OK;
 }
 
-int plan_forward(Plan* P, const float* img1, const float* img2, int ncalls, float* ws, hipStream_t s, bool prefetched) {
+int plan_forward(Plan* P, const float* img1, const float* img2, int ncalls, float* ws, hipStream_t s, bool prefetched, bool consumed) {
   P->ev_next = 0;
   const Lane L0 = lane_of(P, s, 0), LI = lane_of(P, s, 1);
+  bool packed = consumed && !img1 && P->inputs_packed;
+  P->inputs_packed = false;
   if (prefetched) {
     UDET_TRY(plan_prefetch_consume(P, ws, s));
+    packed = P->inputs_packed;
+    P->inputs_packed = false;
     img1 = img2 = nullptr;
   } else if (img1 && P->prefetch_pending) {
     (void)hipStreamWaitEvent(s, P->prefetch_ev, 0);
@@ -832,13 +899,14 @@
     (void)hipEventRecord(e_img, LI.s);
   }
   const bool paired = pairs_on(P);
-  UDET_TRY(plan_rec_image_branch(P, ncalls, ws, LI, !paired));
+  UDET_TRY(plan_rec_image_branch(P, ncalls, ws, LI, !paired, packed));
   if (img1) {
     UDET_TRY(pwc_forward_on(P, img1, img2, ws, L0, lane_of(P, s, 2)));
     UDET_TRY(plan_prepare_flow(P, "flow", ws, s));
   }
   if (e_img) (void)hipStreamWaitEvent(s, e_img, 0);
-  UDET_TRY(plan_generator_forward(P, ws, s));
+  if (packed) UDET_TRY(plan_generator_layers(P, ws, s));
+  else UDET_TRY(plan_generator_forward(P, ws, s));
   order_after(P, LI, L0);
   UDET_TRY(plan_recover_forward(P, ncalls, ws, s, false, !paired, paired));
   if (ncalls == 3) UDET_TRY(plan_losses(P, ws, s));
@@ -912,6 +980,24 @@
   }
   if (a_own_lane) order_after(P, LD, LA);
   const bool pair_enc = pairs_on(P, 1) && with_wgrad && !a_own_lane;
+  bool folded = false;
+  if (with_wgrad && a_shared && !plan_chain_old(UDET_CHAIN_SHARE)) {
+    ShareJobs t;
+    folded = true;
+    for (int i = 8; i >= 1 && folded; --i) {
+      const Layer* L = Lr(std::string("a") + ENC_NAMES[i]);
+      if (i == 8) {
+        const Buf& u = P->buf(U_(P->buf(L->y).name.substr(4)));
+        folded = share_jobs_add(t, u.off, (long)c.batch * u.h * u.w, u.ld, L->y_coff, L->cout);
+      }
+      const std::string xname = P->buf(L->x).name;
+      if (folded && xname.find("concat") != std::string::npos) {
+        const Buf& d = P->buf(D_(xname.substr(4)));
+        folded = share_jobs_add(t, d.off, (long)c.batch * d.h * d.w, d.ld, L->x_coff, L->cin);
+      }
+    }
+    if (folded) UDET_TRY(launch_share_fold_jobs(ws, t, ncopies, true, LA.s));
+  }
   for (int i = 8; i >= 0; --i) {
     DgradJob job[2];
     int njob = 0;
@@ -924,7 +1010,7 @@
       const bool own = e[0] == 'a' && a_own_lane;
       const Lane& LE = own ? LA : LD;
       hipStream_t se = LE.s;
-      if (shared && i == 8) {
+      if (shared && i == 8 && !folded) {
         const Buf& u = P->buf(du);
         UDET_TRY(launch_fold_samples(ws + u.off, (long)c.batch * u.h * u.w, u.ld, L->y_coff, L->cout, ncopies, se));
       }
@@ -941,7 +1027,7 @@
       const bool slab_in = xname.find("concat") != std::string::npos;
       Emit em;
       em.ubuf = U_(xname.substr(4)); em.abuf = L->x; em.c0 = 0; em.c1 = L->cin; em.act = ACT_LEAKY; em.alpha = LEAK;
-      if (shared && slab_in) {
+      if (shared && slab_in && !folded) {
         const Buf& d = P->buf(dx);
         UDET_TRY(launch_fold_samples(ws + d.off, (long)c.batch * d.h * d.w, d.ld, L->x_coff, L->cin, ncopies, se));
       }
@@ -983,13 +1069,17 @@
   UDET_TRY(rec_backward(P, 2 * B, "e", false, true, nullptr, nullptr, ws, LD, LD));
   UDET_TRY(launch_mask_bwd(ws + P->buf(B_("d.mask")).off, ws + P->buf(B_("rec.e.fin")).off, ws + P->buf(B_("flow")).off,
                            ws + P->buf(B_("mask")).off, ws + P->buf(B_("gen.d17")).off, B * HW, s));
+  BnFinishJobs fin[2];
+  const bool defer_fin = !plan_chain_old(UDET_CHAIN_BNFIN) && !P->profiling;
   for (int i = 16; i >= 0; --i) {
     const Layer& L = P->gen[i];
     const bool has_act = L.act != ACT_NONE;
     const int dy = has_act ? B_(S("gen.u%d", i + 1)) : B_(S("gen.d%d", i + 1));
-    const Lane& LWi = (LWlate && i < nlate) ? *LWlate : LW;
+    const bool late = LWlate && i < nlate;
+    const Lane& LWi = late ? *LWlate : LW;
     order_after(P, LD, LWi);
-    UDET_TRY(run_wgrad(P, L, B, dy, has_act, w_gen, g_gen, ws, LWi));
+    UDET_TRY(run_wgrad(P, L, B, dy, has_act, w_gen, g_gen, ws, LWi, defer_fin ? &fin[late ? 1 : 0] : nullptr));
+    if (defer_fin && (i == 0 || (!late && LWlate && i == nlate))) UDET_TRY(launch_bn_finish_jobs(fin[late ? 1 : 0], LWi.s));
     if (i == 0) break;
     int res = -1;
     if (i == 6) res = B_("gen.d11");
diff --git a/unsupervised_detection_amd/engine.py b/unsupervised_detection_amd/engine.py
--- a/unsupervised_detection_amd/engine.py
+++ b/unsupervised_detection_amd/engine.py
@@ -50,6 +50,10 @@
                ("udet_train_step", [c_p, c_i] + [c_p] * 12)):
     getattr(lib, _n).restype = c_i
     getattr(lib, _n).argtypes = _a
+_HAVE_CONSUMED = hasattr(lib, "udet_forward_consumed")
+if _HAVE_CONSUMED:
+    lib.udet_forward_consumed.restype = c_i
+    lib.udet_forward_consumed.argtypes = [c_p, c_i, c_p, c_p]
 
 lib.udet_autotune.restype = c_i
 lib.udet_autotune.argtypes = [c_p] * 7
@@ -164,8 +168,9 @@
         check(lib.udet_prefetch_consume(self._h, self.ws.data_ptr(), self._stream()))
         self._prefetch_keep = None
 
-    def forward_in_place(self, ncalls=3):
-        check(lib.udet_forward_from_flow(self._h, ncalls, self.ws.data_ptr(), self._stream()))
+    def forward_in_place(self, ncalls=3, consumed=False):
+        fn = lib.udet_forward_consumed if consumed and _HAVE_CONSUMED else lib.udet_forward_from_flow
+        check(fn(self._h, ncalls, self.ws.data_ptr(), self._stream()))
 
     def forward_prefetched(self, ncalls=3):
         check(lib.udet_forward_prefetched(self._h, ncalls, self.ws.data_ptr(), self._stream()))
diff --git a/unsupervised_detection_amd/trainer.py b/unsupervised_detection_amd/trainer.py
--- a/unsupervised_detection_amd/trainer.py
+++ b/unsupervised_detection_amd/trainer.py
@@ -144,7 +144,7 @@
         if next_pair is not None:
             e.prefetch_flow(next_pair[0], next_pair[1])
             st._prefetched = (next_pair[0], next_pair[1])
-        call(e.forward_in_place, 3)
+        call(e.forward_in_place, 3, True)
     else:
         call(e.forward, img1, img2, 3)
         if next_pair is not None:
```
